# f4exb/sdrdaemon

Measured on AMD Instinct MI355X. Metric: IQ Msamples/s through decim+FEC-encode pipe; bit-exact vs CPU ref, higher is better.
Workload: dtype int32

## Files before the change

### sdrdaemon_amd/csrc/decim_body.h

```cpp
#pragma once
#include "sdrhip_internal.h"

namespace sdrhip {
namespace {

constexpr int NT = 256;
constexpr int P0 = DECIM_PASS;
constexpr int FULL = 512;
constexpr int HE = 32;

typedef short short2_t __attribute__((ext_vector_type(2)));
typedef int int2_t __attribute__((ext_vector_type(2)));
typedef int int4_t __attribute__((ext_vector_type(4)));
typedef unsigned uint4_t __attribute__((ext_vector_type(4)));

constexpr int C64[16] = {-7, 11, -20, 32, -49, 71, -101, 140, -190, 256, -345, 469, -656, 978, -1698, 5201};
__host__ __device__ constexpr int H32(int i) { return i < 16 ? C64[i] : C64[31 - i]; }
__host__ __device__ constexpr unsigned pack_taps(int lo, int hi) { return ((unsigned)lo & 0xffffu) | ((unsigned)hi << 16); }

constexpr int PK0_DW = 16 + 512 + 16;
constexpr int I0_DW = 32 + 1024;
constexpr int SN_DW = 32 + FULL;

template <int NS_, bool PK_> struct Geo {
    static constexpr int NS = NS_;
    static constexpr bool PK = PK_;
    static constexpr int stride(int s) { return s == 0 ? (PK ? PK0_DW : I0_DW) : SN_DW; }
    static constexpr int base(int s) { return s == 0 ? 0 : base(s - 1) + 4 * stride(s - 1); }
    static constexpr int ldsDw = base(NS);
    static constexpr int plane(int s, int parity, int comp) { return base(s) + (parity * 2 + comp) * stride(s); }
};

__device__ __forceinline__ int dot2(unsigned a, unsigned taps, int acc)
{
    return __builtin_amdgcn_sdot2(__builtin_bit_cast(short2_t, a), __builtin_bit_cast(short2_t, taps), acc, false);
}

__device__ __forceinline__ int dot2_link(unsigned a, unsigned taps, int acc) { return dot2(a, taps, acc); }

__device__ __forceinline__ int dot2_init(unsigned a, unsigned taps, int c)
{
    int d;
    asm("v_dot2_i32_i16 %0, %1, %2, %3" : "=v"(d) : "v"(a), "s"(taps), "v"(c));
    return d;
}

__device__ __forceinline__ int mad24(int a, int tap, int acc)
{
    int d;
    asm("v_mad_i32_i24 %0, %1, %2, %3" : "=v"(d) : "v"(a), "s"(tap), "v"(acc));
    return d;
}

struct OutCtx {
    unsigned *out;
    size_t out_pos;
    bool store;
    int norm, trunk;
    int frame_mode, frame_blocks;
    uint64_t frame_sample_base;
};

__device__ __forceinline__ unsigned final_pack(int i, int q, int norm, int trunk)
{
    int a = (int)((unsigned)i << norm) >> trunk;
    int b = (int)((unsigned)q << norm) >> trunk;
    return ((unsigned)a & 0xffffu) | ((unsigned)b << 16);
}

__device__ __forceinline__ void store_one(const OutCtx &oc, size_t k, unsigned v)
{
    if (!oc.frame_mode) {
        oc.out[k] = v;
    } else {
        uint64_t g = oc.frame_sample_base + k;
        uint64_t f = g / 16129u;
        unsigned w = (unsigned)(g - f * 16129u);
        unsigned b = w / 127u, i = w - b * 127u;
        oc.out[((size_t)f * oc.frame_blocks + 1 + b) * 128u + 1 + i] = v;
    }
}

template <class G, int S> __device__ __forceinline__ void run_stage(int *lds, int tid, int valid, int fill_next, int bias, const OutCtx &oc)
{
    constexpr bool PK = G::PK && S == 0;
    constexpr bool LAST = (S == G::NS - 1);
    constexpr int R = (S == 0) ? 8 : 4;
    const int j = tid >> 1, comp = tid & 1;
    const int k0 = j * R;
    if (k0 >= valid) return;
    const int *pe = lds + G::plane(S, 0, 0) + comp * G::stride(S);
    const int *po = lds + G::plane(S, 1, 0) + comp * G::stride(S);
    int res[R];
    if constexpr (PK) {
        constexpr int WO = (R + 32) / 2, WE = R / 2 + 4;
        unsigned wo[WO], we[WE];
#pragma unroll
        for (int d = 0; d < WO; d += 4) {
            uint4_t v = *reinterpret_cast<const uint4_t *>(po + k0 / 2 + d);
            wo[d] = v.x; wo[d + 1] = v.y; wo[d + 2] = v.z; wo[d + 3] = v.w;
        }
#pragma unroll
        for (int d = 0; d < WE; d += 4) {
            uint4_t v = *reinterpret_cast<const uint4_t *>(pe + k0 / 2 + 8 + d);
            we[d] = v.x; we[d + 1] = v.y; we[d + 2] = v.z; we[d + 3] = v.w;
        }
        const int bias13 = bias << 13;
        int acc[R];
#pragma unroll
        for (int r = 0; r < R; ++r)
            acc[r] = (r & 1) ? dot2_init(we[(r + 1) / 2], pack_taps(8192, 0), bias13) : dot2_init(we[r / 2], pack_taps(0, 8192), bias13);
#pragma unroll
        for (int t = 0; t < 17; ++t) {
#pragma unroll
            for (int r = 0; r < R; ++r) {
                if (r & 1) {
                    if (t < 16) acc[r] = dot2_link(wo[(r + 1) / 2 + t], pack_taps(H32(31 - 2 * t), H32(30 - 2 * t)), acc[r]);
                } else {
                    const unsigned taps = t == 0 ? pack_taps(0, H32(31)) : (t == 16 ? pack_taps(H32(0), 0) : pack_taps(H32(32 - 2 * t), H32(31 - 2 * t)));
                    acc[r] = dot2_link(wo[r / 2 + t], taps, acc[r]);
                }
            }
        }
#pragma unroll
        for (int r = 0; r < R; ++r) res[r] = acc[r] >> 13;
    } else {
        int wo[R + 32], we[R + 4];
#pragma unroll
        for (int x = 0; x < R + 32; x += 4) {
            int4_t v = *reinterpret_cast<const int4_t *>(po + k0 + x);
            wo[x] = v.x; wo[x + 1] = v.y; wo[x + 2] = v.z; wo[x + 3] = v.w;
        }
#pragma unroll
        for (int x = 0; x < R + 4; x += 4) {
            int4_t v = *reinterpret_cast<const int4_t *>(pe + k0 + 16 + x);
            we[x] = v.x; we[x + 1] = v.y; we[x + 2] = v.z; we[x + 3] = v.w;
        }
        int acc[R];
#pragma unroll
        for (int r = 0; r < R; ++r) acc[r] = (int)((unsigned)(we[r + 1] + bias) << 13);
#pragma unroll
        for (int i = 0; i < 16; ++i) {
#pragma unroll
            for (int r = 0; r < R; ++r) acc[r] = mad24(wo[r + 32 - i] + wo[r + 1 + i], C64[i], acc[r]);
        }
#pragma unroll
        for (int r = 0; r < R; ++r) res[r] = acc[r] >> 13;
    }

    if constexpr (LAST) {
        unsigned o[R];
#pragma unroll
        for (int r = 0; r < R; ++r) {
            int other = __builtin_amdgcn_update_dpp(0, res[r], 0xB1 , 0xf, 0xf, true);
            o[r] = final_pack(res[r], other, oc.norm, oc.trunk);
        }
        if (comp != 0 || !oc.store) return;
        const size_t k = oc.out_pos + k0;
        if (!oc.frame_mode && k0 + R <= valid) {
#pragma unroll
            for (int r = 0; r < R; r += 4) *reinterpret_cast<uint4_t *>(oc.out + k + r) = (uint4_t){o[r], o[r + 1], o[r + 2], o[r + 3]};
        } else if (!oc.frame_mode) {
#pragma unroll
            for (int r = 0; r < R; ++r)
                if (k0 + r < valid) oc.out[k + r] = o[r];
        } else {
            const uint64_t g = oc.frame_sample_base + k;
            const uint64_t f = g / 16129u;
            const unsigned w = (unsigned)(g - f * 16129u);
            unsigned b = w / 127u, i = w - b * 127u;
            size_t dw = ((size_t)f * oc.frame_blocks + 1 + b) * 128u + 1 + i;
#pragma unroll
            for (int r = 0; r < R; ++r) {
                if (k0 + r < valid) oc.out[dw] = o[r];
                ++i; ++dw;
                if (i == 127u) {
                    i = 0; ++b; dw += 1;
                    if (b == 127u) { b = 0; dw += ((size_t)oc.frame_blocks - 127u) * 128u; }
                }
            }
        }
    } else {
        int *ne = lds + G::plane(S + 1, 0, 0) + comp * G::stride(S + 1) + HE + fill_next + k0 / 2;
        int *no = lds + G::plane(S + 1, 1, 0) + comp * G::stride(S + 1) + HE + fill_next + k0 / 2;
        if constexpr (R == 8) {
            *reinterpret_cast<int4_t *>(ne) = (int4_t){res[0], res[2], res[4], res[6]};
            *reinterpret_cast<int4_t *>(no) = (int4_t){res[1], res[3], res[5], res[7]};
        } else {
            *reinterpret_cast<int2_t *>(ne) = (int2_t){res[0], res[2]};
            *reinterpret_cast<int2_t *>(no) = (int2_t){res[1], res[3]};
        }
    }
}

template <class G, int S> __device__ __forceinline__ void slide(int *lds, int tid, int consumed)
{
    if (tid >= 128) return;
    const int p = tid >> 5, e = tid & 31;
    int *pl = lds + G::base(S) + p * G::stride(S);
    if constexpr (G::PK && S == 0) {
        short *ps = reinterpret_cast<short *>(pl);
        const short v = ps[e + consumed];
        ps[e] = v;
    } else {
        const int v = pl[e + consumed];
        pl[e] = v;
    }
}

template <class G, int S> __device__ __forceinline__ void hist_put(int *lds, int p, int e, int v)
{
    int *pl = lds + G::base(S) + p * G::stride(S);
    if constexpr (G::PK && S == 0) reinterpret_cast<short *>(pl)[e] = (short)v;
    else pl[e] = v;
}
template <class G, int S> __device__ __forceinline__ int hist_get(const int *lds, int p, int e)
{
    const int *pl = lds + G::base(S) + p * G::stride(S);
    if constexpr (G::PK && S == 0) return reinterpret_cast<const short *>(pl)[e];
    else return pl[e];
}

template <class G, int S = 0> __device__ __forceinline__ void state_load(int *lds, int tid, const int32_t *st, bool zero)
{
    if (tid < 128) {
        const int sp = tid >> 5, e = tid & 31;
        const int kp = (sp & 1) * 2 + (sp >> 1);
        hist_put<G, S>(lds, kp, e, zero ? 0 : st[S * 4 * DEC_HIST + sp * DEC_HIST + e]);
    }
    if constexpr (S + 1 < G::NS) state_load<G, S + 1>(lds, tid, st, zero);
}
template <class G, int S = 0> __device__ __forceinline__ void state_store(const int *lds, int tid, int32_t *st)
{
    if (tid < 128) {
        const int sp = tid >> 5, e = tid & 31;
        const int kp = (sp & 1) * 2 + (sp >> 1);
        st[S * 4 * DEC_HIST + sp * DEC_HIST + e] = hist_get<G, S>(lds, kp, e);
    }
    if constexpr (S + 1 < G::NS) state_store<G, S + 1>(lds, tid, st);
}

template <class G, int S> __device__ __forceinline__ void later_stages(int *lds, int tid, int (&fill)[6], int consumed_prev, bool flush, int bias, OutCtx &oc)
{
    if constexpr (S < G::NS) {
        slide<G, S - 1>(lds, tid, consumed_prev);
        fill[S] += consumed_prev / 2;
        const int have = fill[S];
        const bool run = have > 0 && (have >= FULL || flush);
        if (run) {
            run_stage<G, S>(lds, tid, have, fill[S + 1 < 6 ? S + 1 : 5], bias, oc);
            if (S == G::NS - 1 && oc.store) oc.out_pos += have;
            fill[S] = 0;
        }
        __syncthreads();
        if (run) later_stages<G, S + 1>(lds, tid, fill, have, flush, bias, oc);
    } else {
        slide<G, G::NS - 1>(lds, tid, consumed_prev);
        __syncthreads();
    }
}

template <int L, int FC, bool PACK16, bool TAB = true>
__device__ __forceinline__ void decim_piece(const DecimArgs &a, int *lds, int stream, size_t seg_start, size_t seg_end, bool from_state,
                                            bool store_state, int meta_id, int meta_n)
{
    constexpr bool CEN = (FC == 2);
    constexpr int NS = CEN ? L : L - 2;
    constexpr int RAWSH = CEN ? 0 : 2;
    constexpr int PRAW = P0 << RAWSH;
    constexpr int NLD = PRAW / 4 / NT;
    constexpr int WRAW = 64 << L;
    using G = Geo<NS, PACK16>;
    const int tid = threadIdx.x;
    const unsigned *in = reinterpret_cast<const unsigned *>(a.in) + (size_t)stream * a.in_stride;

    const int32_t *stc = a.state_cur + (size_t)stream * DEC_STATE_WORDS;
    state_load<G>(lds, tid, stc, !from_state);

    OutCtx oc;
    oc.norm = a.norm; oc.trunk = a.trunk;
    oc.frame_mode = a.frame_mode; oc.frame_blocks = a.frame_blocks; oc.frame_sample_base = a.frame_sample_base;
    oc.out = reinterpret_cast<unsigned *>(a.out) + (size_t)stream * a.out_stride;
    oc.out_pos = seg_start >> L;

    if (a.frame_mode) {
        unsigned base[6], rate;
        stream_meta_base(a.meta_w, a.meta_rate, TAB ? a.meta_tab : nullptr, stream, base, rate);
        for (int fi = meta_id + tid * meta_n; fi < a.meta_count; fi += NT * meta_n) {
            unsigned w[6];
            frame_meta_words_thread(base, a.meta_idx0, rate, fi, w);
            unsigned *fr = oc.out + (size_t)(a.meta_first + fi) * a.frame_blocks * 128u;
            fr[0] = (a.meta_frame_count0 + (unsigned)fi) & 0xffffu;
#pragma unroll
            for (int k = 0; k < 6; ++k) fr[1 + k] = w[k];
        }
        if (tid < 128) {
            for (int fi = meta_id; fi < a.meta_count; fi += meta_n) {
                unsigned *fr = oc.out + (size_t)(a.meta_first + fi) * a.frame_blocks * 128u;
                const unsigned fidx = (a.meta_frame_count0 + (unsigned)fi) & 0xffffu;
                if (tid >= 7) fr[tid] = 0u;
                if (tid >= 1) fr[(size_t)tid * 128] = fidx | ((unsigned)tid << 16);
            }
        }
    }

    int fill[6] = {0, 0, 0, 0, 0, 0};
    bool warm = !from_state;
    size_t pos = warm ? seg_start - WRAW : 0;
    size_t region_end = warm ? seg_start : seg_end;

    uint4_t ld[NLD];
    auto issue = [&](size_t p, size_t rend) {
        const unsigned *src = in + p;
        const size_t left = rend - p;
        if (left >= (size_t)PRAW) {
#pragma unroll
            for (int n = 0; n < NLD; ++n) ld[n] = SDRHIP_STREAM_LOAD(reinterpret_cast<const uint4_t *>(src + 4 * (tid + n * NT)));
            return;
        }
        const unsigned rem = (unsigned)left;
#pragma unroll
        for (int n = 0; n < NLD; ++n) {
            const unsigned q = (unsigned)(tid + n * NT);
            uint4_t v = (uint4_t){0u, 0u, 0u, 0u};
            if (4 * q + 3 < rem) {
                v = SDRHIP_STREAM_LOAD(reinterpret_cast<const uint4_t *>(src + 4 * q));
            } else if (4 * q < rem) {
                v.x = src[4 * q];
                if (4 * q + 1 < rem) v.y = src[4 * q + 1];
                if (4 * q + 2 < rem) v.z = src[4 * q + 2];
            }
            ld[n] = v;
        }
    };
    issue(pos, region_end);
    __syncthreads();

    while (true) {
        const size_t left = region_end - pos;
        const int cnt_raw = left < (size_t)PRAW ? (int)left : PRAW;
        const int cnt0 = cnt_raw >> RAWSH;
#pragma unroll
        for (int n = 0; n < NLD; ++n) {
            const int q = tid + n * NT;
            const uint4_t v = ld[n];
            if constexpr (CEN && PACK16) {
                lds[G::plane(0, 0, 0) + 16 + q] = (int)__builtin_amdgcn_perm(v.z, v.x, 0x05040100u);
                lds[G::plane(0, 0, 1) + 16 + q] = (int)__builtin_amdgcn_perm(v.z, v.x, 0x07060302u);
                lds[G::plane(0, 1, 0) + 16 + q] = (int)__builtin_amdgcn_perm(v.w, v.y, 0x05040100u);
                lds[G::plane(0, 1, 1) + 16 + q] = (int)__builtin_amdgcn_perm(v.w, v.y, 0x07060302u);
            } else if constexpr (CEN) {
                *reinterpret_cast<int2_t *>(&lds[G::plane(0, 0, 0) + HE + 2 * q]) = (int2_t){(int)(short)(v.x & 0xffff), (int)(short)(v.z & 0xffff)};
                *reinterpret_cast<int2_t *>(&lds[G::plane(0, 0, 1) + HE + 2 * q]) = (int2_t){(int)v.x >> 16, (int)v.z >> 16};
                *reinterpret_cast<int2_t *>(&lds[G::plane(0, 1, 0) + HE + 2 * q]) = (int2_t){(int)(short)(v.y & 0xffff), (int)(short)(v.w & 0xffff)};
                *reinterpret_cast<int2_t *>(&lds[G::plane(0, 1, 1) + HE + 2 * q]) = (int2_t){(int)v.y >> 16, (int)v.w >> 16};
            } else {
                const int I0 = (short)(v.x & 0xffff), Q0 = (int)v.x >> 16, I1 = (short)(v.y & 0xffff), Q1 = (int)v.y >> 16;
                const int I2 = (short)(v.z & 0xffff), Q2 = (int)v.z >> 16, I3 = (short)(v.w & 0xffff), Q3 = (int)v.w >> 16;
                int x, y;
                if constexpr (FC == 0) {
                    x = I0 - Q1 + Q3 - I2; y = Q0 - Q2 + I1 - I3;
                } else {
                    x = Q0 - I1 - Q2 + I3; y = -I0 - Q1 + I2 + Q3;
                }
                lds[G::plane(0, q & 1, 0) + HE + (q >> 1)] = x;
                lds[G::plane(0, q & 1, 1) + HE + (q >> 1)] = y;
            }
        }
        const size_t next_pos = pos + cnt_raw;
        const bool flush = next_pos >= region_end;
        bool more = !flush;
        size_t n_pos = next_pos, n_end = region_end;
        if (flush && warm && seg_start < seg_end) { more = true; n_pos = seg_start; n_end = seg_end; }
        if (more) issue(n_pos, n_end);
        __syncthreads();

        oc.store = !warm;
        const int valid0 = cnt0 >> 1;
        run_stage<G, 0>(lds, tid, valid0, fill[1], a.bias, oc);
        if (NS == 1 && oc.store) oc.out_pos += valid0;
        __syncthreads();
        later_stages<G, 1>(lds, tid, fill, valid0, flush, a.bias, oc);

        if (!more) break;
        if (flush) { warm = false; region_end = seg_end; }
        pos = n_pos;
    }

    if (store_state) {
        int32_t *stn = a.state_next + (size_t)stream * DEC_STATE_WORDS;
        state_store<G>(lds, tid, stn);
        for (int i = NS * 4 * DEC_HIST + tid; i < DEC_STAGES * 4 * DEC_HIST; i += NT) stn[i] = stc[i];
    }
}


template <int L, int FC, bool PACK16> struct DecimLds {
    static constexpr int NS = (FC == 2) ? L : L - 2;
    static constexpr int dwords = Geo<NS, PACK16>::ldsDw;
    static_assert(dwords * 4 <= 64 * 1024, "LDS budget");
};

__device__ __forceinline__ void decim_simple_row(int log2decim, int fcpos, const int16_t *in, size_t in_stride, int16_t *out,
                                                 size_t out_stride, size_t n_in, int norm, int trunk, int stream)
{
    const unsigned *src = reinterpret_cast<const unsigned *>(in) + (size_t)stream * in_stride;
    unsigned *dst = reinterpret_cast<unsigned *>(out) + (size_t)stream * out_stride;
    const size_t g = (size_t)blockIdx.x * blockDim.x + threadIdx.x;
    if (log2decim == 0) {
        for (size_t i = g; i < n_in; i += (size_t)gridDim.x * blockDim.x) {
            unsigned v = SDRHIP_STREAM_LOAD(src + i);
            int a = (short)(v & 0xffff), b = (int)v >> 16;
            dst[i] = (((unsigned)a << norm) & 0xffffu) | (((unsigned)b << norm) << 16);
        }
        return;
    }
    const size_t n_resize = n_in >> log2decim;
    const size_t ngroups = n_in / 4;
    for (size_t q = g; q < (n_in + 3) / 4; q += (size_t)gridDim.x * blockDim.x) {
        if (q >= ngroups) {
            if (log2decim == 1 && 2 * q < n_resize) dst[2 * q] = 0;
            continue;
        }
        const unsigned v0 = SDRHIP_STREAM_LOAD(src + 4 * q), v1 = SDRHIP_STREAM_LOAD(src + 4 * q + 1), v2 = SDRHIP_STREAM_LOAD(src + 4 * q + 2), v3 = SDRHIP_STREAM_LOAD(src + 4 * q + 3);
        const int I0 = (short)(v0 & 0xffff), Q0 = (int)v0 >> 16, I1 = (short)(v1 & 0xffff), Q1 = (int)v1 >> 16;
        const int I2 = (short)(v2 & 0xffff), Q2 = (int)v2 >> 16, I3 = (short)(v3 & 0xffff), Q3 = (int)v3 >> 16;
        if (log2decim == 1) {
            int xa, ya, xb, yb;
            if (fcpos == 0) { xa = I0 - Q1; ya = Q0 + I1; xb = Q3 - I2; yb = -Q2 - I3; }
            else { xa = Q0 - I1; ya = -I0 - Q1; xb = I3 - Q2; yb = I2 + Q3; }
            dst[2 * q] = final_pack(xa, ya, norm, trunk);
            dst[2 * q + 1] = final_pack(xb, yb, norm, trunk);
        } else {
            int x, y;
            if (fcpos == 0) { x = I0 - Q1 + Q3 - I2; y = Q0 - Q2 + I1 - I3; }
            else { x = Q0 - I1 - Q2 + I3; y = -I0 - Q1 + I2 + Q3; }
            dst[q] = final_pack(x, y, norm, trunk);
        }
    }
}

}
}
```

### sdrdaemon_amd/csrc/decim_mfma.hip

```cpp
#include "decim_body.h"

#include <type_traits>
#include <utility>

#ifndef MF_WAVES
#define MF_WAVES 2
#endif
#ifndef MF_DMA_BURST
#define MF_DMA_BURST 1
#endif

namespace sdrhip {
namespace {

__host__ __device__ constexpr int mf_entry(int kq, int t) { return 8 * (t >> 1) + 2 * kq + (t & 1); }

struct MfATab {
    unsigned w[2][4][64][4];
};

constexpr MfATab mf_make_atab()
{
    MfATab T{};
    for (int m = 0; m < 2; ++m)
        for (int ph = 0; ph < 4; ++ph)
            for (int lane = 0; lane < 64; ++lane) {
                const int r = lane & 15, kq = lane >> 4;
                for (int j = 0; j < 4; ++j) {
                    const int beta = (ph - j) & 3;
                    unsigned word = 0;
                    for (int t = 0; t < 4; ++t) {
                        const int d = r - mf_entry(kq, t) + 16 * beta;
                        int v = 0;
                        if (beta == 3) {
                            const int e = mf_entry(kq, t);
                            const bool hit = (kq == 0 && t == 0) ? r == 15 : e == r + 1;
                            v = (m == 1 && hit) ? 32 : 0;
                        } else if (d >= 0 && d <= 31) {
                            const int h = H32(d);
                            const int h1 = (h + 128) >> 8, h0 = h - 256 * h1;
                            v = m == 0 ? h0 : h1;
                        }
                        word |= (unsigned)(v & 0xff) << (8 * t);
                    }
                    T.w[m][ph][lane][j] = word;
                }
            }
    return T;
}

__device__ const MfATab mf_atab = mf_make_atab();

constexpr int mf_tap_sum()
{
    int s = 0;
    for (int i = 0; i < 32; ++i) s += H32(i);
    return s;
}

template <class F, int... Is> __device__ __forceinline__ void mf_static_for_impl(F &&f, std::integer_sequence<int, Is...>)
{
    (f(std::integral_constant<int, Is>{}), ...);
}
template <int N, class F> __device__ __forceinline__ void mf_static_for(F &&f)
{
    mf_static_for_impl(f, std::make_integer_sequence<int, N>{});
}

__device__ __forceinline__ int4_t mfma(int4_t a, int4_t b, int4_t c)
{
    return __builtin_amdgcn_mfma_i32_16x16x64_i8(a, b, c, 0, 0, 0);
}
__device__ __forceinline__ unsigned perm(unsigned hi, unsigned lo, unsigned sel) { return __builtin_amdgcn_perm(hi, lo, sel); }

template <int NS> struct MfState {
    int4_t O[NS][3];
    unsigned pend[NS][2];
    unsigned evp[NS][2];
};

constexpr int MF_LIMB_BIAS = 128 + 32768 - 262144;

struct MfConst {
    int4_t A[2][4];
    int4_t c0;
    int cinN;
    unsigned selA;
    unsigned selB;
};

template <bool FR> struct MfOut {
    unsigned *p;
    unsigned *dump;
    int store;
    int norm, trunk;
    unsigned sel_pack;
    __amdgpu_buffer_rsrc_t rsrc;
    unsigned off, c, b, t0, t1;
    unsigned gap;
};

typedef unsigned uint2_t __attribute__((ext_vector_type(2)));
__device__ __forceinline__ int sbfe16(unsigned v, int off) { return (int)__builtin_amdgcn_sbfe((int)v, (unsigned)off, 16u); }

__device__ __forceinline__ unsigned lshl_add(unsigned a, int sh, unsigned b) { return (a << sh) + b; }
__device__ __forceinline__ unsigned opaque(unsigned v)
{
    asm("" : "+v"(v));
    return v;
}

__host__ __device__ constexpr int mf_nfixed(int ns) { return ns > 4 ? ns - 4 : 0; }
__host__ __device__ constexpr bool mf_fixed(int ns, int s) { return s >= ns - mf_nfixed(ns); }
template <int NS> constexpr int mf_period() { return 4 << (NS - 1 - mf_nfixed(NS)); }

template <int NS, int S, int I, class OC> __device__ __forceinline__ void mf_stage(MfState<NS> &st, const MfConst &k, OC &oc, int comp)
{
    constexpr int PH = mf_fixed(NS, S) ? 0 : (I & 3);
    const int4_t Ah0 = k.A[0][PH], Ah1 = k.A[1][PH];
    const int4_t z = {0, 0, 0, 0};
    unsigned acc[4];
    if constexpr (S == 0) {
        int4_t g0 = mfma(Ah0, st.O[0][0], k.c0);
        int4_t g1 = mfma(Ah0, st.O[0][1], z);
        int4_t g2 = mfma(Ah1, st.O[0][1], z);
        g1 = mfma(Ah1, st.O[0][0], g1);
#pragma unroll
        for (int r = 0; r < 4; ++r) acc[r] = lshl_add(opaque(lshl_add((unsigned)g2[r], 8, (unsigned)g1[r])), 8, (unsigned)g0[r]);
    } else {
        const int4_t cN = {k.cinN, k.cinN, k.cinN, k.cinN};
        int4_t g0 = mfma(Ah0, st.O[S][0], cN);
        int4_t g1 = mfma(Ah0, st.O[S][1], z);
        int4_t g2 = mfma(Ah0, st.O[S][2], z);
        int4_t g3 = mfma(Ah1, st.O[S][2], z);
        g1 = mfma(Ah1, st.O[S][0], g1);
        g2 = mfma(Ah1, st.O[S][1], g2);
#pragma unroll
        for (int r = 0; r < 4; ++r)
            acc[r] = lshl_add(opaque(lshl_add(opaque(lshl_add((unsigned)g3[r], 8, (unsigned)g2[r])), 8, (unsigned)g1[r])), 8, (unsigned)g0[r]);
    }

    if constexpr (S < NS - 1) {
        constexpr int SIG = I & 1, J = I >> 1;
        const unsigned X = 0x80808080u, X2 = 0x04040404u;
        const unsigned u0 = acc[0] >> 13, u1 = acc[1] >> 13, u2 = acc[2] >> 13, u3 = acc[3] >> 13;
        const unsigned po = perm(u3, u1, 0x05010400u), po2 = perm(u3, u1, 0x0c0c0602u);
        const unsigned pe = perm(u2, u0, 0x05010400u), pe2 = perm(u2, u0, 0x0c0c0602u);
        if constexpr (SIG == 0) {
            st.pend[S + 1][0] = po; st.pend[S + 1][1] = po2;
            constexpr int DJ = mf_fixed(NS, S + 1) ? 1 : ((J + 1) & 3);
            st.O[S + 1][0][DJ] = (int)(perm(pe, (unsigned)st.O[S + 1][0][DJ], k.selA) ^ X);
            st.O[S + 1][1][DJ] = (int)(perm(pe, (unsigned)st.O[S + 1][1][DJ], k.selB) ^ X);
            st.O[S + 1][2][DJ] = (int)(perm(pe2, (unsigned)st.O[S + 1][2][DJ], k.selA) ^ X2);
            st.evp[S + 1][0] = pe; st.evp[S + 1][1] = pe2;
        } else {
            constexpr bool FIX = mf_fixed(NS, S + 1);
            constexpr int NJ = FIX ? 0 : (J & 3), DN = FIX ? 1 : ((J + 2) & 3);
            if constexpr (FIX) {
#pragma unroll
                for (int l = 0; l < 3; ++l) { st.O[S + 1][l][2] = st.O[S + 1][l][3]; st.O[S + 1][l][3] = st.O[S + 1][l][0]; }
            }
            st.O[S + 1][0][NJ] = (int)(perm(po, st.pend[S + 1][0], 0x05040100u) ^ X);
            st.O[S + 1][1][NJ] = (int)(perm(po, st.pend[S + 1][0], 0x07060302u) ^ X);
            st.O[S + 1][2][NJ] = (int)(perm(po2, st.pend[S + 1][1], 0x05040100u) ^ X2);
            const unsigned e0 = perm(pe, st.evp[S + 1][0], 0x05040100u), e1 = perm(pe, st.evp[S + 1][0], 0x07060302u),
                           e2 = perm(pe2, st.evp[S + 1][1], 0x05040100u);
            mf_stage<NS, S + 1, J>(st, k, oc, comp);
            st.O[S + 1][0][DN] = (int)e0; st.O[S + 1][1][DN] = (int)e1; st.O[S + 1][2][DN] = (int)e2;
        }
    } else {
        const int o0 = (int)acc[0] >> 13, o1 = (int)acc[1] >> 13, o2 = (int)acc[2] >> 13, o3 = (int)acc[3] >> 13;
        const int g0 = comp ? o0 : o2, g1 = comp ? o1 : o3;
        const int m0 = comp ? o2 : o0, m1 = comp ? o3 : o1;
        const int r0 = __builtin_amdgcn_update_dpp(0, g0, 0xB1 , 0xf, 0xf, true);
        const int r1 = __builtin_amdgcn_update_dpp(0, g1, 0xB1, 0xf, 0xf, true);
        const unsigned pk0 = perm((unsigned)((int)((unsigned)r0 << oc.norm) >> oc.trunk), (unsigned)((int)((unsigned)m0 << oc.norm) >> oc.trunk), oc.sel_pack);
        const unsigned pk1 = perm((unsigned)((int)((unsigned)r1 << oc.norm) >> oc.trunk), (unsigned)((int)((unsigned)m1 << oc.norm) >> oc.trunk), oc.sel_pack);
        if constexpr (std::is_same<OC, MfOut<true>>::value) {
            const unsigned extra = oc.b == 126u ? oc.gap : 4u;
            const unsigned bias = oc.store ? 0u : 0x80000000u;
            const unsigned a0 = oc.off + (oc.c >= oc.t0 ? extra : 0u) + bias;
            const unsigned hi = a0 ^ 0x40000000u;
            const bool split = oc.c == oc.t1;
            const unsigned a8 = split ? hi : a0, a4 = split ? a0 : hi;
            __builtin_amdgcn_raw_buffer_store_b64((uint2_t){pk0, pk1}, oc.rsrc, a8, 0, 0);
            __builtin_amdgcn_raw_buffer_store_b32(pk0, oc.rsrc, a4, 0, 0);
            __builtin_amdgcn_raw_buffer_store_b32(pk1, oc.rsrc, a4 + extra, 4, 0);
            const unsigned inc = oc.store ? 16u : 0u;
            oc.c += inc;
            const bool wrap = oc.c >= 127u;
            oc.off += 4u * inc + (wrap ? extra : 0u);
            oc.c -= wrap ? 127u : 0u;
            oc.b += wrap ? 1u : 0u;
            oc.b = oc.b >= 127u ? 0u : oc.b;
        } else {
            unsigned *dst = oc.store ? oc.p : oc.dump;
            *reinterpret_cast<uint2_t *>(dst) = (uint2_t){pk0, pk1};
            oc.p += oc.store ? 16 : 0;
        }
    }
}

struct MfFront {
    unsigned sel_own, sel_oth, sel_lo, sel_hi;
    unsigned ev_lo, ev_hi;
};
template <int NS, int I> __device__ __forceinline__ void mf_front(MfState<NS> &st, const MfConst &k, MfFront &f, const uint4_t r)
{
    constexpr int i = I;
    const unsigned ao = perm(r.w, r.y, f.sel_own), ae = perm(r.z, r.x, f.sel_own);
    const unsigned xo = perm(r.w, r.y, f.sel_oth), xe = perm(r.z, r.x, f.sel_oth);
    const unsigned yo = (unsigned)__builtin_amdgcn_update_dpp(0, (int)xo, 0xB1 , 0xf, 0xf, true);
    const unsigned ye = (unsigned)__builtin_amdgcn_update_dpp(0, (int)xe, 0xB1, 0xf, 0xf, true);
    st.O[0][0][i & 3] = (int)(perm(ao, yo, f.sel_lo) ^ 0x80808080u);
    st.O[0][1][i & 3] = (int)perm(ao, yo, f.sel_hi);
    const unsigned cur_lo = perm(ae, ye, f.sel_lo) ^ 0x80808080u, cur_hi = perm(ae, ye, f.sel_hi);
    st.O[0][0][(i + 1) & 3] = (int)perm(cur_lo, f.ev_lo, k.selA);
    st.O[0][1][(i + 1) & 3] = (int)perm(cur_hi, f.ev_hi, k.selA);
    f.ev_lo = cur_lo; f.ev_hi = cur_hi;
}

template <int NS, int I> __device__ __forceinline__ void mf_front2(MfState<NS> &st, const MfConst &k, MfFront &f, const uint4_t rA, const uint4_t rB)
{
    constexpr int i = I;
    const unsigned aoA = perm(rA.w, rA.y, f.sel_own), aoB = perm(rB.w, rB.y, f.sel_own);
    const unsigned aeA = perm(rA.z, rA.x, f.sel_own), aeB = perm(rB.z, rB.x, f.sel_own);
    st.O[0][0][i & 3] = (int)(perm(aoA, aoB, 0x01000504u) ^ 0x80808080u);
    st.O[0][1][i & 3] = (int)perm(aoA, aoB, 0x03020706u);
    const unsigned cur_lo = perm(aeA, aeB, 0x01000504u) ^ 0x80808080u, cur_hi = perm(aeA, aeB, 0x03020706u);
    st.O[0][0][(i + 1) & 3] = (int)perm(cur_lo, f.ev_lo, k.selA);
    st.O[0][1][(i + 1) & 3] = (int)perm(cur_hi, f.ev_hi, k.selA);
    f.ev_lo = cur_lo; f.ev_hi = cur_hi;
}

constexpr int MF_GROUP_BYTES = 9216;
constexpr int mf_wave_ring(int ng) { return ng * MF_GROUP_BYTES; }
static_assert(MF_HEAD_MIN % P0 == 0 && MF_TAIL_SEG % P0 == 0, "K1m's head and tail pieces are whole passes of the VALU code");
__host__ __device__ constexpr int mf_block_units(int p) { return 72 * p + 2 * (p >> 2); }

template <int D> __device__ __forceinline__ void mf_dma_issue(unsigned slot, unsigned voff, unsigned long long span_base)
{
    constexpr int off = 16 * mf_block_units(D);
    asm volatile("s_add_u32 m0, %1, %2\n\ts_nop 0\n\tglobal_load_lds_dwordx4 %0, %3 nt" ::"v"(voff), "s"(slot), "n"(off), "s"(span_base) : "memory", "scc");
}
template <int N> __device__ __forceinline__ void mf_wait_vm()
{
    static_assert(N == 0 || N == 7 || N == 8 || N == 15 || N == 16, "vmcnt immediates of the ring");
    if constexpr (N == 0) asm volatile("s_waitcnt vmcnt(0)" ::: "memory");
    if constexpr (N == 7) asm volatile("s_waitcnt vmcnt(7)" ::: "memory");
    if constexpr (N == 8) asm volatile("s_waitcnt vmcnt(8)" ::: "memory");
    if constexpr (N == 15) asm volatile("s_waitcnt vmcnt(15)" ::: "memory");
    if constexpr (N == 16) asm volatile("s_waitcnt vmcnt(16)" ::: "memory");
}

#ifdef MF_STAMPS
__device__ unsigned long long g_mf_stamps[4096 * 10];
__device__ __forceinline__ void mf_stamp(int gw, int k)
{
    if ((threadIdx.x & 63) == 0 && gw < 4096) {
        unsigned long long t;
        asm volatile("s_memrealtime %0\n\ts_waitcnt lgkmcnt(0)" : "=s"(t)::"memory");
        g_mf_stamps[gw * 10 + k] = t;
        if (k == 0) {
            unsigned hw, xcc;
            asm volatile("s_getreg_b32 %0, hwreg(HW_REG_HW_ID)" : "=s"(hw));
            asm volatile("s_getreg_b32 %0, hwreg(HW_REG_XCC_ID)" : "=s"(xcc));
            g_mf_stamps[gw * 10 + 8] = ((unsigned long long)(xcc & 0xfu) << 32) | hw;
        }
    }
}
#define MF_STAMP(gw, k) mf_stamp(gw, k)
#else
#define MF_STAMP(gw, k) do { } while (0)
#endif

template <int NS, int NG, class OC>
__device__ __forceinline__ void mf_loop_dma(const DecimArgs &a, MfState<NS> &st, const MfConst &k, OC &oc, MfFront &fr, unsigned lds_addr,
                                            const char *wbase, size_t S, int nper, int WP, int lane, int p, int comp, int q, int gw)
{
    constexpr int P = mf_period<NS>();
    static_assert(P == 32, "four groups of 8 steps per period");
    static_assert(NG == 2 || NG == 3 || NG == 4, "ring depth");
    constexpr int LA = NG - 1;
    const int wv = __builtin_amdgcn_readfirstlane((int)(threadIdx.x >> 6));
    const unsigned ring = (unsigned)__builtin_amdgcn_readfirstlane((int)(lds_addr + (unsigned)wv * (unsigned)mf_wave_ring(NG)));
    unsigned long long sb[8];
#pragma unroll
    for (int d = 0; d < 8; ++d) {
        const unsigned long long v = (unsigned long long)(wbase + (size_t)d * S * 4);
        sb[d] = ((unsigned long long)(unsigned)__builtin_amdgcn_readfirstlane((int)(v >> 32)) << 32) | (unsigned)__builtin_amdgcn_readfirstlane((int)v);
    }
    unsigned rs[NG];
    const __attribute__((address_space(3))) char *lr[NG];
#pragma unroll
    for (int j = 0; j < NG; ++j) {
        rs[j] = ring + (unsigned)(j * MF_GROUP_BYTES);
        lr[j] = (const __attribute__((address_space(3))) char *)(size_t)(rs[j] + 16u * (unsigned)(mf_block_units(0) + 72 * p + 2 * (p >> 2) + 4 * comp + q));
    }
    unsigned voff[4];
    const unsigned vmax = 16u * (unsigned)lane + 1024u * (unsigned)(4 * nper - 1);
#pragma unroll
    for (int g = 0; g < 4; ++g) voff[g] = min(16u * (unsigned)lane + 1024u * (unsigned)(g + LA), vmax);
    {
        unsigned v0 = 16u * (unsigned)lane;
        mf_static_for<8 * LA>([&](auto ic) {
            constexpr int i = decltype(ic)::value;
            mf_dma_issue<i % 8>(rs[i / 8], v0 + 1024u * (unsigned)(i / 8), sb[i % 8]);
        });
    }
    MF_STAMP(gw, 1);
    mf_wait_vm<8 * (LA - 1)>();
    uint4_t r = *reinterpret_cast<const __attribute__((address_space(3))) uint4_t *>(lr[0]);
    MF_STAMP(gw, 2);
    for (int per = 0; per < nper; ++per) {
#ifdef MF_STAMPS
        if (per == 1) MF_STAMP(gw, 3);
        if (per == nper / 4) MF_STAMP(gw, 4);
        if (per == nper / 2) MF_STAMP(gw, 5);
        if (per == 3 * nper / 4) MF_STAMP(gw, 6);
#endif
        oc.store = per >= WP;
        mf_static_for<P>([&](auto ic) {
            constexpr int i = decltype(ic)::value;
            constexpr int i1 = i + 1;
            constexpr int B = NG == 2 ? 8 : MF_DMA_BURST;
            if constexpr (i1 % 8 == 0) mf_wait_vm<(B == 1 ? 8 * (LA - 2) + 7 : 8 * (LA - 1))>();
            const uint4_t rn = *reinterpret_cast<const __attribute__((address_space(3))) uint4_t *>(lr[(i1 / 8) % NG] + 128 * (i1 % 8));
            constexpr int g = i / 8, d = i % 8;
            if constexpr (d < 8 / B) {
                mf_static_for<B>([&](auto bc) {
                    constexpr int sp = B * d + decltype(bc)::value;
                    mf_dma_issue<sp>(rs[(g + LA) % NG], voff[g], sb[sp]);
                });
                if constexpr (d == 8 / B - 1) voff[g] = min(voff[g] + 4096u, vmax);
            }
            mf_front<NS, i>(st, k, fr, r);
            mf_stage<NS, 0, i>(st, k, oc, comp);
            r = rn;
        });
        if constexpr (4 % NG != 0) {
            const unsigned t = rs[0];
            const __attribute__((address_space(3))) char *u = lr[0];
#pragma unroll
            for (int j = 0; j + 1 < NG; ++j) { rs[j] = rs[j + 1]; lr[j] = lr[j + 1]; }
            rs[NG - 1] = t; lr[NG - 1] = u;
        }
    }
    mf_wait_vm<0>();
}

template <int NS, int NG = 0, bool FR = false> __device__ __forceinline__ void mf_wave(const DecimArgs &a, int gw, unsigned lds_addr)
{
    if (a.mf_prio) __builtin_amdgcn_s_setprio(3);
    constexpr int L = NS;
    constexpr int P = mf_period<NS>();
#ifndef MF_DEPTH
#define MF_DEPTH 8
#endif
#ifndef MF_BURST
#define MF_BURST 1
#endif
    constexpr int D = MF_DEPTH < P ? MF_DEPTH : P / 2;
    constexpr size_t W = (size_t)64 << L;
    constexpr int WP = (int)(W / (32 * (size_t)P));
    static_assert(P % D == 0, "prefetch ring");
    static_assert((size_t)D * 32 <= MF_READ_AHEAD, "the planner leaves the register ring's read-ahead behind a wave's last span (decim_plan.h)");
    const int lane = threadIdx.x & 63;
    const int n = lane & 15, q = lane >> 4, comp = n & 1, p = n >> 1;
    const int stream = gw / a.mf_wps, ws = gw - stream * a.mf_wps;
    const size_t S = a.mf_span;
    const size_t wave_start = a.mf_head + (size_t)ws * 8 * S;
    const char *wbase = reinterpret_cast<const char *>(a.in) + ((size_t)stream * a.in_stride + wave_start - W) * 4;
    const unsigned loff = (unsigned)((size_t)p * S * 4) + 16u * (unsigned)q + 64u * (unsigned)comp;
    const int T = (int)((W + S) / 32);
    const int nper = T / P;

    MfConst k;
#pragma unroll
    for (int m = 0; m < 2; ++m)
#pragma unroll
        for (int ph = 0; ph < 4; ++ph) k.A[m][ph] = *reinterpret_cast<const int4_t *>(&mf_atab.w[m][ph][lane][0]);
    const unsigned b13 = (unsigned)a.bias << 13;
    const unsigned gain = (unsigned)mf_tap_sum() + 8192u;
    {
        const int c = (int)(128u * gain + b13);
        k.c0 = (int4_t){c, c, c, c};
    }
    k.cinN = (int)((unsigned)MF_LIMB_BIAS * gain + b13);
    k.selA = q == 0 ? 0x03020104u : 0x03020100u;
    k.selB = q == 0 ? 0x03020106u : 0x03020100u;

    MfOut<FR> oc;
    oc.store = 0;
    oc.dump = a.mf_dump + 4 * lane;
    oc.norm = a.norm; oc.trunk = a.trunk;
    oc.sel_pack = comp ? 0x01000504u : 0x05040100u;
    {
        const size_t first = ((wave_start + (size_t)p * S) >> L) + 4u * (unsigned)q;
        if constexpr (FR) {
            unsigned *obase = reinterpret_cast<unsigned *>(a.out) + (size_t)stream * a.out_stride;
            oc.rsrc = __builtin_amdgcn_make_buffer_rsrc(obase, 0, 0x3fffffff, 0x00020000);
            const unsigned long long g = a.frame_sample_base + first;
            const unsigned long long f = g / 16129u;
            const unsigned w = (unsigned)(g - f * 16129u);
            oc.b = w / 127u; oc.c = w - oc.b * 127u;
            oc.off = 4u * (unsigned)(((size_t)f * (size_t)a.frame_blocks + 1u + oc.b) * 128u + 1u + oc.c + 2u * (unsigned)comp);
            oc.t0 = 127u - 2u * (unsigned)comp; oc.t1 = 126u - 2u * (unsigned)comp;
            oc.gap = 4u * ((unsigned)a.frame_blocks * 128u - 16255u);
            oc.p = nullptr;
        } else {
            unsigned *obase = reinterpret_cast<unsigned *>(a.out) + (size_t)stream * a.out_stride;
            oc.p = obase + first + 2 * comp;
            oc.off = oc.c = oc.b = oc.t0 = oc.t1 = oc.gap = 0u;
        }
    }

    MfState<NS> st;
#pragma unroll
    for (int s = 0; s < NS; ++s) {
#pragma unroll
        for (int b = 0; b < 3; ++b) st.O[s][b] = (int4_t){0, 0, 0, 0};
        st.pend[s][0] = st.pend[s][1] = 0u;
        st.evp[s][0] = st.evp[s][1] = 0u;
    }

    MfFront fr;
    fr.sel_own = comp ? 0x07030602u : 0x05010400u;
    fr.sel_oth = comp ? 0x05010400u : 0x07030602u;
    fr.sel_lo = comp ? 0x05040100u : 0x01000504u; fr.sel_hi = comp ? 0x07060302u : 0x03020706u;
    fr.ev_lo = 0u; fr.ev_hi = 0u;
    if constexpr (NG != 0 && mf_dma_applies(NS)) {
        mf_loop_dma<NS, NG>(a, st, k, oc, fr, lds_addr, wbase, S, nper, WP, lane, p, comp, q, gw);
        return;
    }
    uint4_t ld[D];
    const char *src = wbase + loff;
#define MF_LDSTRIDE 128
#pragma unroll
    for (int d = 0; d < D; ++d) ld[d] = SDRHIP_STREAM_LOAD(reinterpret_cast<const uint4_t *>(src + MF_LDSTRIDE * d));

    for (int per = 0; per < nper; ++per) {
        oc.store = per >= WP;
        mf_static_for<P>([&](auto ic) {
            constexpr int i = decltype(ic)::value;
            constexpr int slot = i % D;
            const uint4_t r = ld[slot];
            ld[slot] = SDRHIP_STREAM_LOAD(reinterpret_cast<const uint4_t *>(src + MF_LDSTRIDE * (i + D)));
            mf_front<NS, i>(st, k, fr, r);
            mf_stage<NS, 0, i>(st, k, oc, comp);
        });
        src += MF_LDSTRIDE * P;
    }
}

__host__ __device__ constexpr int mf_block_threads(int) { return NT; }

template <int L, bool PACK16, int NG, bool FR> __global__ __launch_bounds__(mf_block_threads(L), mf_dma_applies(L) && NG != 2 ? 1 : MF_WAVES) void decim_mfma_kernel(DecimArgs a)
{
    constexpr int LDSDW = mf_dma_applies(L) && mf_wave_ring(NG) > DecimLds<L, 2, PACK16>::dwords ? mf_wave_ring(NG) : DecimLds<L, 2, PACK16>::dwords;
    __shared__ __attribute__((aligned(16))) int lds[LDSDW];
    const int nmf = (a.nstreams * a.mf_wps + 3) / 4;
    const int bx = blockIdx.x;
    if (bx >= nmf) {
        const int nitems = a.nstreams * a.mf_npieces, j = bx - nmf, nearly = a.mf_piece_early * a.mf_piece_share;
        const int nmine = j < a.mf_piece_early ? a.mf_piece_share : 1;
        for (int k = 0; k < nmine; ++k) {
            const int lx = j < a.mf_piece_early ? j + k * a.mf_piece_early : nearly + (j - a.mf_piece_early);
            if (lx >= nitems || (j < a.mf_piece_early && lx >= nearly)) break;
            const int stream = lx / a.mf_npieces, piece = lx - stream * a.mf_npieces;
            if (piece == 0) {
                decim_piece<L, 2, PACK16>(a, lds, stream, 0, a.mf_head, true, false, piece, a.mf_npieces);
            } else {
                const size_t s0 = a.mf_tail_start + (size_t)(piece - 1) * a.mf_tail_seg;
                size_t s1 = s0 + a.mf_tail_seg;
                if (s1 > a.n_used || piece == a.mf_npieces - 1) s1 = a.n_used;
                decim_piece<L, 2, PACK16>(a, lds, stream, s0, s1, false, piece == a.mf_npieces - 1, piece, a.mf_npieces);
            }
            __syncthreads();
        }
        return;
    }
    const int gw = __builtin_amdgcn_readfirstlane(bx * 4 + (int)(threadIdx.x >> 6));
    if (gw >= a.nstreams * a.mf_wps) return;
    MF_STAMP(gw, 0);
    mf_wave<L, NG, FR>(a, gw, (unsigned)(size_t)(__attribute__((address_space(3))) char *)lds);
    MF_STAMP(gw, 7);
}
__device__ __forceinline__ int mf_ragged_find(const RaggedRow *rows, int nstreams, int x, bool waves)
{
    int lo = 0, hi = nstreams - 1;
    while (lo < hi) {
        const int mid = (lo + hi + 1) >> 1;
        if ((waves ? rows[mid].mf_w0 : rows[mid].mf_p0) <= x) lo = mid;
        else hi = mid - 1;
    }
    return __builtin_amdgcn_readfirstlane(lo);
}
__device__ __forceinline__ DecimArgs mf_ragged_args(const DecimArgs &a, const RaggedRow &r)
{
    DecimArgs b = a;
    b.n_used = (size_t)r.n_used;
    b.mf_wps = r.mf_wps;
    const unsigned sh = (unsigned)__builtin_amdgcn_readfirstlane((int)r.shifts);
    b.norm = (int)(sh & 0xffu); b.trunk = (int)(sh >> 8);
    if (a.frame_mode) {
        b.out = reinterpret_cast<int16_t *>(reinterpret_cast<unsigned *>(a.out) + r.out_off);
        b.frame_sample_base = r.frame_sample_base;
        b.meta_first = r.meta_first; b.meta_count = r.meta_count; b.meta_frame_count0 = r.frame_count0;
        b.meta_w[3] = r.tv_sec; b.meta_w[4] = r.tv_usec;
        b.meta_idx0 = r.meta_idx0;
    }
    return b;
}

template <int L, bool PACK16, int NG, bool FR> __global__ __launch_bounds__(mf_block_threads(L), mf_dma_applies(L) && NG != 2 ? 1 : MF_WAVES) void decim_mfma_ragged_kernel(DecimArgs a, const RaggedRow *rows)
{
    constexpr int LDSDW = mf_dma_applies(L) && mf_wave_ring(NG) > DecimLds<L, 2, PACK16>::dwords ? mf_wave_ring(NG) : DecimLds<L, 2, PACK16>::dwords;
    __shared__ __attribute__((aligned(16))) int lds[LDSDW];
    const int nmf = (a.mf_wps + 3) / 4;
    const int bx = blockIdx.x;
    if (bx >= nmf) {
        const int nitems = a.mf_npieces, j = bx - nmf, nearly = a.mf_piece_early * a.mf_piece_share;
        const int nmine = j < a.mf_piece_early ? a.mf_piece_share : 1;
        for (int k = 0; k < nmine; ++k) {
            const int lx = j < a.mf_piece_early ? j + k * a.mf_piece_early : nearly + (j - a.mf_piece_early);
            if (lx >= nitems || (j < a.mf_piece_early && lx >= nearly)) break;
            const int stream = mf_ragged_find(rows, a.nstreams, lx, false);
            const RaggedRow &r = rows[stream];
            const DecimArgs b = mf_ragged_args(a, r);
            const int piece = lx - r.mf_p0;
            const size_t n_used = (size_t)r.n_used;
            if (piece == 0) {
                decim_piece<L, 2, PACK16, false>(b, lds, stream, 0, (size_t)r.mf_head, true, r.mf_np == 1, piece, r.mf_np);
            } else {
                const size_t s0 = (size_t)r.mf_tail_start + (size_t)(piece - 1) * a.mf_tail_seg;
                size_t s1 = s0 + a.mf_tail_seg;
                if (s1 > n_used || piece == r.mf_np - 1) s1 = n_used;
                decim_piece<L, 2, PACK16, false>(b, lds, stream, s0, s1, false, piece == r.mf_np - 1, piece, r.mf_np);
            }
            __syncthreads();
        }
        return;
    }
    const int gw = __builtin_amdgcn_readfirstlane(bx * 4 + (int)(threadIdx.x >> 6));
    if (gw >= a.mf_wps) return;
    const int stream = mf_ragged_find(rows, a.nstreams, gw, true);
    const RaggedRow &r = rows[stream];
    const DecimArgs b = mf_ragged_args(a, r);
    mf_wave<L, NG, FR>(b, stream * r.mf_wps + (gw - r.mf_w0), (unsigned)(size_t)(__attribute__((address_space(3))) char *)lds);
}

#ifdef MF_STAMPS
}
extern "C" int sdrhip_debug_mf_stamps(unsigned long long *dst) { return (int)hipMemcpyFromSymbol(dst, HIP_SYMBOL(g_mf_stamps), sizeof(g_mf_stamps)); }
namespace {
#endif

#include "gf_encode128_body.h"
#ifndef MF_FUSED_WPE
#define MF_FUSED_WPE 3
#endif
struct FusedRoles {
    unsigned *tab;
    unsigned tag;
};

template <int L, bool PACK16> __global__ __launch_bounds__(NT, MF_FUSED_WPE) void rx_fused_kernel(DecimArgs a, Enc128Args e, FusedRoles fr)
{
    constexpr int LDSDW = ENC128_LDS_BYTES / 4 > DecimLds<L, 2, PACK16>::dwords ? ENC128_LDS_BYTES / 4 : DecimLds<L, 2, PACK16>::dwords;
    __shared__ __attribute__((aligned(16))) int lds[LDSDW];
    __shared__ int s_unit;
    const int nmf = (a.nstreams * a.mf_wps + 3) / 4;
    const int npiece = a.nstreams * a.mf_npieces;
    const int nenc = 2 * e.nlist;
    if (threadIdx.x == 0) {
        unsigned hw, xcc;
        asm volatile("s_getreg_b32 %0, hwreg(HW_REG_HW_ID)" : "=s"(hw));
        asm volatile("s_getreg_b32 %0, hwreg(HW_REG_XCC_ID)" : "=s"(xcc));
        const unsigned key = ((xcc & 0xfu) << 8) | ((hw >> 8) & 0xffu);
        unsigned *cnt = fr.tab + 4096 + 4 * (fr.tag & 1u);
        if (blockIdx.x == 0) { unsigned *nxt = fr.tab + 4096 + 4 * ((fr.tag + 1u) & 1u); nxt[0] = 0u; nxt[1] = 0u; nxt[2] = 0u; }
        const bool first = atomicMax(fr.tab + key, fr.tag) < fr.tag;
        int unit = -1;
        if (first) { const unsigned u = atomicAdd(cnt + 0, 1u); if (u < (unsigned)nmf) unit = (int)u; }
        if (unit < 0) { const unsigned u = atomicAdd(cnt + 1, 1u); if (u < (unsigned)npiece) unit = nmf + (int)u; }
        if (unit < 0) { const unsigned u = atomicAdd(cnt + 2, 1u); if (u < (unsigned)nenc) unit = nmf + npiece + (int)u; }
        if (unit < 0) { const unsigned u = atomicAdd(cnt + 0, 1u); if (u < (unsigned)nmf) unit = (int)u; }
        s_unit = unit;
    }
    __syncthreads();
    const int bx = s_unit;
    if (bx < 0) return;
    const int ndec = nmf + npiece;
    if (bx >= ndec) {
        gf_encode128_wg(e, bx - ndec, reinterpret_cast<unsigned char *>(lds));
        return;
    }
    if (bx >= nmf) {
        const int lx = bx - nmf;
        const int stream = lx / a.mf_npieces, piece = lx - stream * a.mf_npieces;
        if (piece == 0) {
            decim_piece<L, 2, PACK16>(a, lds, stream, 0, a.mf_head, true, false, piece, a.mf_npieces);
        } else {
            const size_t s0 = a.mf_tail_start + (size_t)(piece - 1) * a.mf_tail_seg;
            size_t s1 = s0 + a.mf_tail_seg;
            if (s1 > a.n_used || piece == a.mf_npieces - 1) s1 = a.n_used;
            decim_piece<L, 2, PACK16>(a, lds, stream, s0, s1, false, piece == a.mf_npieces - 1, piece, a.mf_npieces);
        }
        return;
    }
    const int gw = __builtin_amdgcn_readfirstlane(bx * 4 + (int)(threadIdx.x >> 6));
    if (gw >= a.nstreams * a.mf_wps) return;
    mf_wave<L, 0>(a, gw, 0u);
}

template <int L> hipError_t launch_fused(bool pack16, const DecimArgs &a, const Enc128Args &e, unsigned *roles, unsigned tag, hipStream_t stream)
{
    const int ndec = (a.nstreams * a.mf_wps + 3) / 4 + a.nstreams * a.mf_npieces;
    const dim3 grid(ndec + 2 * e.nlist), block(NT);
    FusedRoles fr;
    fr.tab = roles; fr.tag = tag;
    if (pack16) hipLaunchKernelGGL((rx_fused_kernel<L, true>), grid, block, 0, stream, a, e, fr);
    else hipLaunchKernelGGL((rx_fused_kernel<L, false>), grid, block, 0, stream, a, e, fr);
    return hipGetLastError();
}

template <int L, int NG, bool FR> void launch_mf2(bool pack16, const DecimArgs &a, dim3 grid, dim3 block, hipStream_t stream)
{
    if (pack16) hipLaunchKernelGGL((decim_mfma_kernel<L, true, NG, FR>), grid, block, 0, stream, a);
    else hipLaunchKernelGGL((decim_mfma_kernel<L, false, NG, FR>), grid, block, 0, stream, a);
}

template <int L> hipError_t launch_mf(bool pack16, const DecimArgs &a, hipStream_t stream)
{
    const int nleg = a.mf_piece_wgs > 0 ? a.mf_piece_wgs : a.nstreams * a.mf_npieces;
    const int nmf = (a.nstreams * a.mf_wps + 3) / 4;
    const dim3 grid(nleg + nmf), block(mf_block_threads(L));
    if constexpr (mf_dma_applies(L)) {
// ... 76 lines not shown
```

### sdrdaemon_amd/csrc/rx_frame_area.h

```cpp
#pragma once
#include <cstddef>
#include <cstdint>
#include <vector>

namespace sdrhip {
constexpr uint64_t RX_FRAME_SAMPLES = 127 * 127;
constexpr size_t RX_NO_LATE = ~(size_t)0;

struct RxAdvance {
    size_t done;
    uint64_t rest;
    int first_new;
    int started;
    uint64_t idx0;
    unsigned frame_count0;
};

struct RxAreaPlan {
    size_t new_cap = 0;
    bool keep_old = false;
    std::vector<uint8_t> to_slot0;
    bool moves() const
    {
        for (size_t s = 0; s < to_slot0.size(); ++s)
            if (to_slot0[s]) return true;
        return false;
    }
};

class RxFrameArea {
public:
    void init(size_t nstreams)
    {
        cap_ = 0;
        base_.assign(nstreams, 0); pending_.assign(nstreams, 0); open_.assign(nstreams, 0); count_.assign(nstreams, 0);
    }
    size_t streams() const { return base_.size(); }
    size_t cap() const { return cap_; }
    size_t slot(size_t s) const { return base_[s]; }
    const size_t *slots() const { return base_.data(); }
    uint64_t pending(size_t s) const { return pending_[s]; }
    bool open(size_t s) const { return open_[s] != 0; }
    uint16_t count(size_t s) const { return count_[s]; }
    size_t index(size_t s, size_t f = 0) const { return s * cap_ + base_[s] + f; }

    bool aligned() const
    {
        for (size_t s = 1; s < base_.size(); ++s)
            if (base_[s] != base_[0] || pending_[s] != pending_[0] || open_[s] != open_[0] || count_[s] != count_[0]) return false;
        return true;
    }

    RxAdvance advance(size_t s, size_t n_dec) const
    {
        RxAdvance a;
        const uint64_t total = pending_[s] + n_dec;
        a.done = (size_t)(total / RX_FRAME_SAMPLES);
        a.rest = total - (uint64_t)a.done * RX_FRAME_SAMPLES;
        a.first_new = open_[s] ? 1 : 0;
        a.started = (int)(a.done + (a.rest > 0 ? 1 : 0)) - a.first_new;
        a.idx0 = a.first_new ? RX_FRAME_SAMPLES - pending_[s] : 0;
        a.frame_count0 = (unsigned)count_[s] + (unsigned)a.first_new;
        return a;
    }

    RxAreaPlan plan(const size_t *done, size_t late_slot0, size_t window_multiple) const
    {
        RxAreaPlan p;
        const size_t S = base_.size();
        size_t need_max = 0;
        for (size_t s = 0; s < S; ++s) need_max = done[s] + 1 > need_max ? done[s] + 1 : need_max;
        bool hits_late = false;
        p.to_slot0.assign(S, 0);
        if (need_max > cap_) p.new_cap = window_multiple * need_max;
        else
            for (size_t s = 0; s < S; ++s) {
                if (base_[s] + done[s] + 1 <= cap_) continue;
                p.to_slot0[s] = 1;
                hits_late = hits_late || (late_slot0 != RX_NO_LATE && done[s] + 1 > late_slot0);
            }
        if (hits_late) p.new_cap = cap_;
        if (p.new_cap) {
            p.to_slot0.assign(S, 1);
            p.keep_old = late_slot0 != RX_NO_LATE;
        }
        return p;
    }
    RxAreaPlan replan() const
    {
        RxAreaPlan p;
        p.new_cap = cap_;
        p.to_slot0.assign(base_.size(), cap_ ? 1 : 0);
        return p;
    }
    void moved(const RxAreaPlan &p)
    {
        if (p.new_cap) cap_ = p.new_cap;
        for (size_t s = 0; s < base_.size(); ++s)
            if (p.to_slot0[s]) base_[s] = 0;
    }
    void commit(const size_t *done, const uint64_t *rest)
    {
        for (size_t s = 0; s < base_.size(); ++s) {
            base_[s] += done[s];
            pending_[s] = rest[s];
            open_[s] = rest[s] > 0 ? 1 : 0;
            count_[s] = (uint16_t)(count_[s] + done[s]);
        }
    }

    void reset(const uint8_t *mask)
    {
        for (size_t s = 0; s < base_.size(); ++s) {
            if (mask && !mask[s]) continue;
            pending_[s] = 0; open_[s] = 0; count_[s] = 0;
            if (!mask) base_[s] = 0;
        }
    }
    static bool importable(uint64_t pending, uint32_t open, uint32_t count)
    {
        return open <= 1 && pending < RX_FRAME_SAMPLES && (open || !pending) && count <= 0xffffu;
    }
    void import_stream(size_t s, uint64_t pending, uint32_t open, uint32_t count)
    {
        pending_[s] = pending; open_[s] = (uint8_t)open; count_[s] = (uint16_t)count;
    }

private:
    size_t cap_ = 0;
    std::vector<size_t> base_;
    std::vector<uint64_t> pending_;
    std::vector<uint8_t> open_;
    std::vector<uint16_t> count_;
};

class RxView {
public:
    const uint8_t *base() const { return base_; }
    size_t stride() const { return stride_; }
    size_t first(size_t s) const { return first_[s]; }
    size_t frames(size_t s) const { return frames_[s]; }
    void init(size_t nstreams) { set(nullptr, 0, nstreams, 0, 0); }
    void clear() { base_ = nullptr; stride_ = 0; first_.assign(first_.size(), 0); frames_.assign(frames_.size(), 0); }
    bool uniform() const
    {
        for (size_t s = 1; s < first_.size(); ++s)
            if (first_[s] != first_[0] || frames_[s] != frames_[0]) return false;
        return true;
    }
    void set(const uint8_t *area, size_t stream_stride, size_t nstreams, size_t first_slot, size_t n)
    {
        base_ = area; stride_ = stream_stride; first_.assign(nstreams, first_slot); frames_.assign(nstreams, n);
    }
    void set_each(const uint8_t *area, size_t stream_stride, size_t nstreams, const size_t *first_slot, const size_t *n)
    {
        base_ = area; stride_ = stream_stride; first_.assign(first_slot, first_slot + nstreams); frames_.assign(n, n + nstreams);
    }
    size_t offset(size_t s, size_t frame_bytes) const { return s * stride_ + first_[s] * frame_bytes; }
    const uint8_t *window(size_t s, size_t frame_bytes) const { return base_ ? base_ + offset(s, frame_bytes) : nullptr; }

private:
    const uint8_t *base_ = nullptr;
    size_t stride_ = 0;
    std::vector<size_t> first_, frames_;
};
}
```

### sdrdaemon_amd/csrc/sdrhip.cpp

```cpp
#include "sdrhip_host.h"
#include "gf256.h"

#include <cstdarg>
#include <cstdio>
#include <cstdlib>
#include <cstring>
#include <new>
#include <string>
#include <vector>

using namespace sdrhip;

namespace {
thread_local std::string g_err;
}

namespace sdrhip {

int fail(int code, const char *fmt, ...)
{
    char buf[512];
    va_list ap;
    va_start(ap, fmt);
    vsnprintf(buf, sizeof(buf), fmt, ap);
    va_end(ap);
    g_err = buf;
    return code;
}

}

extern "C" const char *sdrhip_last_error(void) { return g_err.c_str(); }

extern "C" int sdrhip_device_count(void)
{
    int n = 0;
    if (hipGetDeviceCount(&n) != hipSuccess) return 0;
    return n;
}

namespace sdrhip {
static void ctx_free(sdrhip_ctx *c);
static void drop_kernel_events(sdrhip_ctx *c)
{
    (void)hipStreamSynchronize(c->stream);
    if (c->stream2) (void)hipStreamSynchronize(c->stream2);
    for (int k = 0; k < SDRHIP_KCLASSES; ++k) {
        for (auto &pr : c->kev[k]) { (void)hipEventDestroy(pr.first); (void)hipEventDestroy(pr.second); }
        c->kev[k].clear();
    }
}
}

extern "C" int sdrhip_ctx_create(int device, void *hip_stream, sdrhip_ctx **out)
{
    if (!out) return fail(SDRHIP_EINVAL, "ctx_create: out is NULL");
    *out = nullptr;
    int n = sdrhip_device_count();
    if (n <= 0) return fail(SDRHIP_EDEVICE, "no HIP device available (this library has no CPU fallback)");
    if (device < 0 || device >= n) return fail(SDRHIP_EINVAL, "device %d out of range (have %d)", device, n);
    HIP_TRY(hipSetDevice(device));
    sdrhip_ctx *c = new (std::nothrow) sdrhip_ctx();
    if (!c) return fail(SDRHIP_ENOMEM, "out of host memory");
    c->device = device;
    c->stream = static_cast<hipStream_t>(hip_stream);
    {
        hipDeviceProp_t prop;
        if (hipGetDeviceProperties(&prop, device) == hipSuccess && prop.multiProcessorCount > 0) c->n_cu = prop.multiProcessorCount;
        static const char *const keys[][2] = {{"SDRHIP_DECIM_PATH", "decim_path"}, {"SDRHIP_MFMA_SPAN", "mfma_span"}, {"SDRHIP_MFMA_MIN", "mfma_min"},
                                              {"SDRHIP_INTERP_PATH", "interp_path"}, {"SDRHIP_INTERP_SPAN", "interp_span"}, {"SDRHIP_RX_FUSED", "rx_fused"}, {"SDRHIP_RX_DIRECT", "rx_direct"},
                                              {"SDRHIP_DEC_PATH", "dec_path"}, {"SDRHIP_ENC_PATH", "enc_path"}, {"SDRHIP_ENC_MIN_ROWS", "enc_min_rows"}, {"SDRHIP_MFMA_RING", "mfma_ring"}, {"SDRHIP_TX_OVERLAP", "tx_overlap"}, {"SDRHIP_RX_WINDOW", "rx_window"}, {"SDRHIP_FEC_STAGGER", "fec_stagger"}, {"SDRHIP_FEC_STAGGER_MOD", "fec_stagger_mod"}, {"SDRHIP_DEC_PLAN", "dec_plan"}, {"SDRHIP_TX_GATHER", "tx_gather"}, {"SDRHIP_ENC_UNITS", "enc_units"}, {"SDRHIP_ENC_FORM", "enc_form"}};
        for (size_t i = 0; i < sizeof(keys) / sizeof(keys[0]); ++i)
            if (const char *v = getenv(keys[i][0])) (void)sdrhip_ctx_set_option(c, keys[i][1], v);
    }
    std::vector<uint8_t> tab(256 * 32);
    gf_build_tables(tab.data());
    if (hipMalloc(reinterpret_cast<void **>(&c->gf_tab), tab.size()) != hipSuccess) { c->gf_tab = nullptr; ctx_free(c); return fail(SDRHIP_ENOMEM, "hipMalloc gf tables"); }
    if (hipMemcpy(c->gf_tab, tab.data(), tab.size(), hipMemcpyHostToDevice) != hipSuccess) { ctx_free(c); return fail(SDRHIP_EDEVICE, "upload gf tables"); }
    std::vector<uint8_t> em(128 * 128);
    cm256_encode_matrix(128, 128, em.data());
    if (hipMalloc(reinterpret_cast<void **>(&c->enc_matrix), em.size()) != hipSuccess ||
        hipMemcpy(c->enc_matrix, em.data(), em.size(), hipMemcpyHostToDevice) != hipSuccess) { ctx_free(c); return fail(SDRHIP_ENOMEM, "upload encode matrix"); }
    std::vector<uint8_t> kl(8 * 81 * 32);
    cm256_karatsuba_leaf_tables(kl.data());
    if (hipMalloc(reinterpret_cast<void **>(&c->enc_leaves), kl.size()) != hipSuccess ||
        hipMemcpy(c->enc_leaves, kl.data(), kl.size(), hipMemcpyHostToDevice) != hipSuccess) { ctx_free(c); return fail(SDRHIP_ENOMEM, "upload encoder constants"); }
    {
        std::vector<uint8_t> ft((size_t)CM256_FFT_TABLES * 32);
        cm256_fft_tables(ft.data());
        if (hipMalloc(reinterpret_cast<void **>(&c->enc_fft), ft.size()) != hipSuccess ||
            hipMemcpy(c->enc_fft, ft.data(), ft.size(), hipMemcpyHostToDevice) != hipSuccess) { ctx_free(c); return fail(SDRHIP_ENOMEM, "upload encoder FFT constants"); }
    }
    {
        const GF256 &g = gf();
        uint8_t el[1024];
        memcpy(el, g.exp, 512);
        memcpy(el + 512, g.log, 512);
        if (hipMalloc(reinterpret_cast<void **>(&c->gf_explog), sizeof(el)) != hipSuccess ||
            hipMemcpy(c->gf_explog, el, sizeof(el), hipMemcpyHostToDevice) != hipSuccess) { ctx_free(c); return fail(SDRHIP_ENOMEM, "upload GF(256) exp/log tables"); }
    }
    if (hipMalloc(reinterpret_cast<void **>(&c->dec_stats), 64) != hipSuccess ||
        hipMemset(c->dec_stats, 0, 64) != hipSuccess) { ctx_free(c); return fail(SDRHIP_ENOMEM, "hipMalloc decoder counters"); }
    if (hipMalloc(reinterpret_cast<void **>(&c->decim_dump), 4096) != hipSuccess) { c->decim_dump = nullptr; ctx_free(c); return fail(SDRHIP_ENOMEM, "hipMalloc decimator scratch"); }
    if (hipMalloc(reinterpret_cast<void **>(&c->fused_roles), SDRHIP_FUSED_ROLE_WORDS * 4) != hipSuccess ||
        hipMemset(c->fused_roles, 0, SDRHIP_FUSED_ROLE_WORDS * 4) != hipSuccess) { ctx_free(c); return fail(SDRHIP_ENOMEM, "hipMalloc role table"); }
    if (hipEventCreate(&c->ev0) != hipSuccess || hipEventCreate(&c->ev1) != hipSuccess) { ctx_free(c); return fail(SDRHIP_EDEVICE, "hipEventCreate"); }
    *out = c;
    return SDRHIP_OK;
}

namespace sdrhip {
int ctx_stream2(sdrhip_ctx *c, hipStream_t *out)
{
    if (!c->stream2) {
        int lo = 0, hi = 0;
        if (hipDeviceGetStreamPriorityRange(&lo, &hi) != hipSuccess) lo = 0;
        if (hipStreamCreateWithPriority(&c->stream2, hipStreamNonBlocking, lo) != hipSuccess) {
            c->stream2 = nullptr;
            return fail(SDRHIP_EDEVICE, "hipStreamCreate (second stream)");
        }
    }
    *out = c->stream2;
    return SDRHIP_OK;
}
void ctx_retain(sdrhip_ctx *c) { c->refs.fetch_add(1); }
void ctx_release(sdrhip_ctx *c)
{
    if (c->refs.fetch_sub(1) == 1 && c->dying) ctx_free(c);
}
}

extern "C" void sdrhip_ctx_destroy(sdrhip_ctx *c)
{
    if (!c || c->dying.exchange(true)) return;
    if (c->refs.load() == 0) ctx_free(c);
}

extern "C" int sdrhip_ctx_set_option(sdrhip_ctx *c, const char *key, const char *value)
{
    if (!c || !key || !value) return fail(SDRHIP_EINVAL, "ctx_set_option: NULL argument");
    sdrhip::CtxLock lock_(c);
    const std::string k(key), v(value);
    char *end = nullptr;
    const unsigned long long num = strtoull(value, &end, 10);
    const bool isnum = *value && end && !*end;
    if (k == "decim_path") {
        if (v == "auto") c->opt.decim_path = DECIM_PATH_AUTO;
        else if (v == "valu") c->opt.decim_path = DECIM_PATH_VALU;
        else if (v == "mfma") c->opt.decim_path = DECIM_PATH_MFMA;
        else return fail(SDRHIP_EINVAL, "ctx_set_option: decim_path must be auto, valu or mfma");
    } else if (k == "interp_path") {
        if (v == "auto") c->opt.interp_wave = CtxOptions().interp_wave;
        else if (v == "valu") c->opt.interp_wave = 0;
        else if (v == "wave") c->opt.interp_wave = 1;
        else return fail(SDRHIP_EINVAL, "ctx_set_option: interp_path must be auto, valu or wave");
    } else if (k == "mfma_span" && isnum) c->opt.mfma_span = (size_t)num;
    else if (k == "mfma_min" && isnum) c->opt.mfma_min = (size_t)num;
    else if (k == "interp_span" && isnum) c->opt.interp_span = (size_t)num;
    else if (k == "rx_fused" && isnum && num <= 3) c->opt.rx_fused = (int)num;
    else if (k == "rx_fused" && v == "overlap") c->opt.rx_fused = 3;
    else if (k == "rx_direct" && isnum && num <= 1) c->opt.rx_direct = (int)num;
    else if (k == "rx_window" && isnum && num <= 8) c->opt.rx_window = (int)num;
    else if (k == "mfma_ring" && isnum && num >= 2 && num <= 4) c->opt.mfma_ring = (int)num;
    else if (k == "tx_overlap" && isnum && num <= 1) c->opt.tx_overlap = (int)num;
    else if (k == "fec_stagger" && isnum && num <= 64) c->opt.fec_stagger = (int)num;
    else if (k == "fec_stagger_mod" && isnum && num <= 116) c->opt.fec_stagger_mod = (int)num;
    else if (k == "tx_gather" && isnum && num <= 1) c->opt.tx_gather = (int)num;
    else if (k == "dec_plan") {
        if (v == "fused") c->opt.dec_fused_plan = 1;
        else if (v == "kernel") c->opt.dec_fused_plan = 0;
        else return fail(SDRHIP_EINVAL, "ctx_set_option: dec_plan must be fused or kernel");
    }
    else if (k == "enc_min_rows" && isnum && num >= 1 && num <= 32) c->opt.enc_min_rows = (int)num;
    else if (k == "enc_units" && (v == "frame" || v == "half")) c->opt.enc_half = v == "half";
    else if (k == "enc_form" && (v == "bitslice" || v == "table")) c->opt.enc_bitslice = v == "bitslice";
    else if (k == "enc_path") {
        if (v == "fft") c->opt.enc_fft = 1;
        else if (v == "karatsuba") c->opt.enc_fft = 0;
        else return fail(SDRHIP_EINVAL, "ctx_set_option: enc_path must be fft or karatsuba");
    } else if (k == "dec_path") {
        if (v == "syndrome") c->opt.dec_syndrome = 1;
        else if (v == "dense") c->opt.dec_syndrome = 0;
        else return fail(SDRHIP_EINVAL, "ctx_set_option: dec_path must be syndrome or dense");
    } else if (k == "dec_max_rows" && isnum && num >= 1 && num <= 128) { c->opt.dec_max_rows = (int)num; c->opt.dec_auto = 0; }
    else if (k == "dec_max_rows" && v == "auto") { c->opt.dec_max_rows = 128; c->opt.dec_auto = 1; }
    else if (k == "dec_strict" && isnum && num <= 1) c->opt.dec_strict = (int)num;
    else if (k == "ktime_stride" && isnum && num >= 1 && num <= 1024) { c->ktime_stride = (int)num; for (int i = 0; i < SDRHIP_KCLASSES; ++i) c->ktime_stride_cls[i] = 0; }
    else if (k == "ktime_stride_class") {
        int cls = -1, st = 0;
        if (sscanf(value, "%d:%d", &cls, &st) != 2 || cls < 0 || cls >= SDRHIP_KCLASSES || st < 1 || st > 1024) return fail(SDRHIP_EINVAL, "ctx_set_option: ktime_stride_class takes <class 0..4>:<stride 1..1024>");
        c->ktime_stride_cls[cls] = st;
    }
    else return fail(SDRHIP_EINVAL, "ctx_set_option: unknown key or malformed value: %s=%s", key, value);
    return SDRHIP_OK;
}

extern "C" int sdrhip_ctx_get_counter(sdrhip_ctx *c, const char *key, uint64_t *value)
{
    if (!c || !key || !value) return fail(SDRHIP_EINVAL, "ctx_get_counter: NULL argument");
    sdrhip::CtxLock lock_(c);
    if (std::string(key) == "h2d_bytes") { *value = c->h2d_bytes; return SDRHIP_OK; }
    if (std::string(key) == "d2h_bytes") { *value = c->d2h_bytes; return SDRHIP_OK; }
    const bool shadow = std::string(key) == "fecbuf_shadow_mismatch";
    const bool deferred = std::string(key) == "dec_deferred";
    if (std::string(key) != "dec_rows_exceeded" && !shadow && !deferred) return fail(SDRHIP_EINVAL, "ctx_get_counter: unknown key: %s", key);
    HIP_TRY(hipSetDevice(c->device));
    unsigned v = 0;
    HIP_TRY(link_copy(c, &v, c->dec_stats + (shadow ? DEC_STATS_SHADOW_MISMATCH : deferred ? DEC_STATS_DEFERRED : 0), sizeof(v), hipMemcpyDeviceToHost, c->stream));
    HIP_TRY(hipStreamSynchronize(c->stream));
    *value = v;
    return SDRHIP_OK;
}

int sdrhip::enc128_min_rows(const sdrhip_ctx *c) { return c->opt.enc_fft ? c->opt.enc_min_rows : ENC128_MIN_ROWS; }

static void sdrhip::ctx_free(sdrhip_ctx *c)
{
    (void)hipSetDevice(c->device);
    (void)hipStreamSynchronize(c->stream);
    drop_kernel_events(c);
    c->in.release(); c->out.release(); c->aux.release(); c->aux3.release();
    if (c->gf_tab) (void)hipFree(c->gf_tab);
    if (c->enc_matrix) (void)hipFree(c->enc_matrix);
    if (c->enc_leaves) (void)hipFree(c->enc_leaves);
    if (c->enc_fft) (void)hipFree(c->enc_fft);
    if (c->decim_dump) (void)hipFree(c->decim_dump);
    if (c->fused_roles) (void)hipFree(c->fused_roles);
    if (c->gf_explog) (void)hipFree(c->gf_explog);
    if (c->dec_stats) (void)hipFree(c->dec_stats);
    c->dec_plan.release();
    c->pin.release();
    c->zin.release(); c->zout.release();
    if (c->stream2) { (void)hipStreamSynchronize(c->stream2); (void)hipStreamDestroy(c->stream2); }
    if (c->ev0) (void)hipEventDestroy(c->ev0);
    if (c->ev1) (void)hipEventDestroy(c->ev1);
    delete c;
}

extern "C" int sdrhip_ctx_synchronize(sdrhip_ctx *c)
{
    if (!c) return fail(SDRHIP_EINVAL, "ctx is NULL");
    sdrhip::CtxLock lock_(c);
    HIP_TRY(hipStreamSynchronize(c->stream));
    if (c->stream2) HIP_TRY(hipStreamSynchronize(c->stream2));
    return SDRHIP_OK;
}

extern "C" int sdrhip_ctx_timing_begin(sdrhip_ctx *c)
{
    if (!c) return fail(SDRHIP_EINVAL, "ctx is NULL");
    HIP_TRY(hipEventRecord(c->ev0, c->stream));
    return SDRHIP_OK;
}

extern "C" int sdrhip_ctx_timing_end(sdrhip_ctx *c, float *ms)
{
    if (!c || !ms) return fail(SDRHIP_EINVAL, "ctx/ms is NULL");
    HIP_TRY(hipEventRecord(c->ev1, c->stream));
    HIP_TRY(hipEventSynchronize(c->ev1));
    HIP_TRY(hipEventElapsedTime(ms, c->ev0, c->ev1));
    return SDRHIP_OK;
}

extern "C" int sdrhip_ctx_kernel_timing(sdrhip_ctx *c, int enable)
{
    if (!c) return fail(SDRHIP_EINVAL, "ctx is NULL");
    sdrhip::CtxLock lock_(c);
    c->ktime_on = enable != 0;
    for (int i = 0; i < SDRHIP_KCLASSES; ++i) c->ktime_seen[i] = 0;
    if (!enable) drop_kernel_events(c);
    return SDRHIP_OK;
}

extern "C" int sdrhip_ctx_kernel_timing_read(sdrhip_ctx *c, int cls, double *total_ms, unsigned *launches)
{
    if (!c || cls < 0 || cls >= SDRHIP_KCLASSES || !total_ms || !launches) return fail(SDRHIP_EINVAL, "kernel_timing_read: bad argument");
    sdrhip::CtxLock lock_(c);
    HIP_TRY(hipStreamSynchronize(c->stream));
    if (c->stream2) HIP_TRY(hipStreamSynchronize(c->stream2));
    double sum = 0;
    unsigned n = 0;
    for (auto &pr : c->kev[cls]) {
        float ms = 0;
        if (hipEventElapsedTime(&ms, pr.first, pr.second) == hipSuccess) { sum += ms; ++n; }
        (void)hipEventDestroy(pr.first);
        (void)hipEventDestroy(pr.second);
    }
    c->kev[cls].clear();
    *total_ms = sum;
    *launches = n;
    return SDRHIP_OK;
}

namespace {
struct HostRange { const char *p; size_t n; };
std::mutex g_host_mtx;
std::vector<HostRange> g_host_ranges;
}
namespace sdrhip {
bool host_is_pinned(const void *p, size_t n)
{
    std::lock_guard<std::mutex> g(g_host_mtx);
    const char *c = static_cast<const char *>(p);
    for (const HostRange &r : g_host_ranges)
        if (c >= r.p && c + n <= r.p + r.n) return true;
    return false;
}
}

extern "C" void *sdrhip_host_alloc(sdrhip_ctx *c, size_t bytes)
{
    if (!c || bytes == 0) return nullptr;
    if (hipSetDevice(c->device) != hipSuccess) return nullptr;
    void *p = nullptr;
    if (hipHostMalloc(&p, bytes, hipHostMallocDefault) != hipSuccess) { (void)fail(SDRHIP_ENOMEM, "hipHostMalloc(%zu) failed", bytes); return nullptr; }
    std::lock_guard<std::mutex> g(g_host_mtx);
    g_host_ranges.push_back(HostRange{static_cast<const char *>(p), bytes});
    return p;
}

extern "C" void sdrhip_host_free(sdrhip_ctx *c, void *p)
{
    if (!p) return;
    (void)c;
    {
        std::lock_guard<std::mutex> g(g_host_mtx);
        for (size_t i = 0; i < g_host_ranges.size(); ++i)
            if (g_host_ranges[i].p == p) { g_host_ranges.erase(g_host_ranges.begin() + (long)i); break; }
    }
    (void)hipHostFree(p);
}
```

### sdrdaemon_amd/csrc/sdrhip_decim.cpp

```cpp
#include "sdrhip_host.h"

#include <cstring>
#include <new>
#include <vector>

using namespace sdrhip;

struct sdrhip_decimators {
    sdrhip::CtxRef ctx;
    int nstreams;
    int bias;
    sdrhip::DevBuf state[2];
    int cur;
    bool stage0_int16;
    sdrhip::DecimPlanInfo last;
    sdrhip::PinnedBuf rows_pin, stage_pin, out_pin;
    sdrhip::DevBuf rows_dev;
    sdrhip::StreamMask reset_mask;
    explicit sdrhip_decimators(sdrhip_ctx *c) : ctx(c) {}
};

extern "C" int sdrhip_decimators_last_plan(const sdrhip_decimators *d, sdrhip_decim_plan *out)
{
    if (!d || !out) return fail(SDRHIP_EINVAL, "decimators_last_plan: NULL argument");
    sdrhip::CtxLock lock_(d->ctx);
    out->path = d->last.path; out->wps = d->last.wps; out->npieces = d->last.npieces; out->nseg = d->last.nseg;
    out->span = d->last.span; out->head = d->last.head; out->tail_start = d->last.tail_start;
    return SDRHIP_OK;
}

extern "C" int sdrhip_decimators_create(sdrhip_ctx *ctx, int nstreams, int hb_variant, sdrhip_decimators **out)
{
    if (!ctx || !out || nstreams <= 0 || nstreams > 65535) return fail(SDRHIP_EINVAL, "decimators_create: bad argument");
    if (hb_variant != SDRHIP_HB_EO1 && hb_variant != SDRHIP_HB_DB) return fail(SDRHIP_EINVAL, "hb_variant must be SDRHIP_HB_EO1 or SDRHIP_HB_DB");
    HIP_TRY(hipSetDevice(ctx->device));
    sdrhip_decimators *d = new (std::nothrow) sdrhip_decimators(ctx);
    if (!d) return fail(SDRHIP_ENOMEM, "out of host memory");
    d->nstreams = nstreams; d->bias = hb_variant; d->cur = 0; d->stage0_int16 = true;
    size_t bytes = (size_t)nstreams * DEC_STATE_WORDS * sizeof(int32_t);
    if (d->state[0].alloc_exact(bytes) || d->state[1].alloc_exact(bytes)) {
        delete d;
        return fail(SDRHIP_ENOMEM, "hipMalloc decimator state");
    }
    *out = d;
    return sdrhip_decimators_reset(d);
}

extern "C" void sdrhip_decimators_destroy(sdrhip_decimators *d)
{
    if (!d) return;
    (void)hipSetDevice(d->ctx->device);
    (void)hipStreamSynchronize(d->ctx->stream);
    delete d;
}

extern "C" int sdrhip_decimators_reset(sdrhip_decimators *d)
{
    if (!d) return fail(SDRHIP_EINVAL, "decimators is NULL");
    sdrhip::CtxLock lock_(d->ctx);
    size_t bytes = (size_t)d->nstreams * DEC_STATE_WORDS * sizeof(int32_t);
    HIP_TRY(hipMemsetAsync(d->state[0].p, 0, bytes, d->ctx->stream));
    HIP_TRY(hipMemsetAsync(d->state[1].p, 0, bytes, d->ctx->stream));
    d->cur = 0;
    d->stage0_int16 = true;
    return SDRHIP_OK;
}

namespace sdrhip {
void decimators_reset_part(sdrhip_decimators *d, StreamResetArgs *a)
{
    a->rows[0] = d->state[0].as<int32_t>(); a->rows[1] = d->state[1].as<int32_t>();
    a->row_words = DEC_STATE_WORDS;
}
void decimators_reset_done(sdrhip_decimators *d, bool all)
{
    if (all) d->stage0_int16 = true;
}
int32_t *decimators_row(sdrhip_decimators *d, int s, int half) { return d->state[d->cur ^ (half & 1)].as<int32_t>() + (size_t)s * DEC_STATE_WORDS; }
bool decimators_stage0_int16(const sdrhip_decimators *d) { return d->stage0_int16; }
void decimators_clear_stage0_int16(sdrhip_decimators *d) { d->stage0_int16 = false; }
}

extern "C" int sdrhip_decimators_reset_streams(sdrhip_decimators *d, const uint8_t *mask)
{
    if (!d) return fail(SDRHIP_EINVAL, "decimators is NULL");
    sdrhip::CtxLock lock_(d->ctx);
    return stream_reset_bank(d->ctx, d->reset_mask, mask, d->nstreams,
                             [d](StreamResetArgs *a) { decimators_reset_part(d, a); },
                             [d](const uint8_t *m) { decimators_reset_done(d, m == nullptr); });
}

namespace {
void set_mf_args(DecimArgs &a, const MfPlan &p)
{
    a.mf_head = p.head; a.mf_span = p.span; a.mf_tail_start = p.tail_start; a.mf_tail_seg = p.tail_seg;
    a.mf_wps = p.wps; a.mf_npieces = p.npieces;
    a.mf_piece_wgs = p.piece_wgs; a.mf_piece_early = p.piece_early; a.mf_piece_share = p.piece_share;
}

struct DecimCall {
    const int16_t *in;
    size_t in_stride;
    int16_t *out;
    size_t out_stride;
    int frame_mode, frame_blocks;
    size_t n_raw, n_dec;
    size_t min_used;
};

template <class Simple, class Plan, class Launch>
int decimate_core(sdrhip_decimators *d, unsigned L, int fcpos, const DecimCall &k, Simple simple, Plan plan, Launch launch)
{
    sdrhip_ctx *c = d->ctx;
    d->last = DecimPlanInfo();
    if ((L == 0 ? k.n_raw : k.n_dec) == 0) return SDRHIP_OK;
    const bool cen = fcpos == SDRHIP_FC_CEN;
    if (L == 0 || (!cen && L <= 2)) {
        if (k.frame_mode) return fail(SDRHIP_EINVAL, L == 0 ? "internal: frame mode needs log2decim >= 1" : "internal: frame mode unsupported for filter-less decimation");
        hipError_t e = simple();
        if (e != hipSuccess) return fail(SDRHIP_EDEVICE, "decimate%u launch: %s", 1u << L, hipGetErrorString(e));
        return SDRHIP_OK;
    }

    DecimArgs a;
    memset(&a, 0, sizeof(a));
    a.in = k.in; a.out = k.out; a.in_stride = k.in_stride; a.out_stride = k.out_stride;
    a.state_cur = d->state[d->cur].as<int32_t>(); a.state_next = d->state[d->cur ^ 1].as<int32_t>();
    a.nstreams = d->nstreams;
    a.bias = d->bias;
    a.frame_mode = k.frame_mode; a.frame_blocks = k.frame_blocks;
    a.mf_dump = c->decim_dump;
    bool mfma = false;
    if (int rc = plan(a, &mfma)) return rc;
    const bool pack16 = cen && d->stage0_int16;
    hipError_t e;
    {
        KTimer kt(c, SDRHIP_K_DECIMATE);
        e = launch(a, pack16, mfma);
    }
    if (e != hipSuccess) return fail(SDRHIP_EDEVICE, "decimate launch: %s", hipGetErrorString(e));
    d->last.path = mfma ? DECIM_PATH_MFMA : DECIM_PATH_VALU;
    if (mfma) {
        d->last.span = a.mf_span; d->last.head = a.mf_head; d->last.tail_start = a.mf_tail_start;
        d->last.wps = a.mf_wps; d->last.npieces = a.mf_npieces;
    } else {
        d->last.nseg = a.nseg;
    }
    d->cur ^= 1;
    d->stage0_int16 = cen && (d->stage0_int16 || k.min_used >= (size_t)2 * DEC_HIST);
    return SDRHIP_OK;
}
}

namespace sdrhip {
int decimate_device(sdrhip_decimators *d, int log2decim, int fcpos, unsigned *sampleSize, const int16_t *in, size_t n_in,
                    size_t in_stride, int16_t *out, size_t out_stride, size_t *n_out, int frame_mode, int frame_blocks,
                    uint64_t frame_sample_base, const RxMeta *meta, const Enc128Args *fuse, bool *fused, bool coresident)
{
    if (fused) *fused = false;
    sdrhip_ctx *c = d->ctx;
    const int S = d->nstreams;
    const unsigned L = (unsigned)log2decim;
    const DecimShifts sh = decimated_shifts(L, *sampleSize);
    const size_t n_dec = n_in >> L;
    const size_t n_used = n_dec << L;
    *sampleSize = decimated_sample_size(L, *sampleSize);
    if (n_out) *n_out = n_dec;
    const DecimCall k = {in, in_stride, out, out_stride, frame_mode, frame_blocks, n_in, n_dec, n_used};
    return decimate_core(
        d, L, fcpos, k,
        [&]() { return launch_decimate_simple(log2decim, fcpos, in, in_stride, out, out_stride, n_in, S, (int)sh.norm, (int)sh.trunk, c->stream); },
        [&](DecimArgs &a, bool *mfma) -> int {
            a.n_used = n_used;
            a.norm = (int)sh.norm; a.trunk = (int)sh.trunk;
            a.frame_sample_base = frame_sample_base;
            if (meta) set_meta_args(a, *meta);
            plan_decimate(log2decim, fcpos, n_used, S, &a.nsub_per_seg, &a.nseg);
            const CtxOptions &env = c->opt;
            const bool mfma_frames = env.rx_direct && out_stride * 4 < 0x3fffffffu;
            a.mf_ring = coresident ? 3 : env.mfma_ring;
            a.mf_prio = coresident ? 1 : 0;
            MfPlan p;
            *mfma = (!frame_mode || mfma_frames) && mfma_admitted(env.decim_path, env.mfma_min, log2decim, n_used * (size_t)S) &&
                    plan_decimate_mfma(log2decim, fcpos, n_used, S, env.mfma_span, c->n_cu, a.mf_ring, &p);
            if (*mfma) set_mf_args(a, p);
            return SDRHIP_OK;
        },
        [&](const DecimArgs &a, bool pack16, bool mfma) -> hipError_t {
            if (!(mfma && fuse && L <= 4))
                return mfma ? launch_decimate_mfma(log2decim, pack16, a, c->stream) : launch_decimate(log2decim, fcpos, pack16, a, c->stream);
            hipError_t e;
            if (++c->fused_tag == 0xffffffffu) {
                (void)hipMemsetAsync(c->fused_roles, 0, SDRHIP_FUSED_ROLE_WORDS * 4, c->stream);
                c->fused_tag = 1;
            }
            if (c->opt.rx_fused == 2) {
                Enc128Args none = *fuse;
                none.nlist = 0;
                e = launch_rx_fused(log2decim, pack16, a, none, c->fused_roles, c->fused_tag, c->stream);
                if (e == hipSuccess) e = launch_gf_encode128(*fuse, c->stream);
            } else
                e = launch_rx_fused(log2decim, pack16, a, *fuse, c->fused_roles, c->fused_tag, c->stream);
            if (e != hipSuccess) {
                (void)hipMemsetAsync(c->fused_roles, 0, SDRHIP_FUSED_ROLE_WORDS * 4, c->stream);
                c->fused_tag = 0;
            }
            if (fused) *fused = true;
            return e;
        });
}

bool decimate_mfma_applies(const sdrhip_decimators *d, int log2decim, int fcpos, size_t n_in)
{
    const CtxOptions &env = d->ctx->opt;
    const size_t n_used = (n_in >> log2decim) << log2decim;
    MfPlan p;
    return mfma_admitted(env.decim_path, env.mfma_min, log2decim, n_used * (size_t)d->nstreams) &&
           plan_decimate_mfma(log2decim, fcpos, n_used, d->nstreams, env.mfma_span, d->ctx->n_cu, env.mfma_ring, &p);
}
}

extern "C" int sdrhip_decimate(sdrhip_decimators *d, int log2decim, int fcpos, unsigned *sampleSize, const int16_t *iq_in,
                               size_t n_in, size_t in_stride, int16_t *iq_out, size_t out_stride, size_t *n_out, int mem)
{
    if (!d || !sampleSize) return fail(SDRHIP_EINVAL, "decimate: NULL handle or sampleSize");
    sdrhip::CtxLock lock_(d->ctx);
    if (log2decim < 0 || log2decim > 6) return fail(SDRHIP_EINVAL, "Invalid log2 decimation factor");
    if (fcpos < SDRHIP_FC_INF || fcpos > SDRHIP_FC_CEN) return fail(SDRHIP_EINVAL, "Invalid Fc position index");
    if (*sampleSize < 1 || *sampleSize > 16) return fail(SDRHIP_EINVAL, "sampleSize must be 1..16");
    if (n_in && (!iq_in || (!iq_out && (n_in >> log2decim)))) return fail(SDRHIP_EINVAL, "decimate: NULL buffer");
    sdrhip_ctx *c = d->ctx;
    HIP_TRY(hipSetDevice(c->device));
    const int S = d->nstreams;
    const size_t n_res = n_in >> log2decim;
    if (S == 1) { in_stride = n_in; out_stride = n_res; }
    if (S > 1 && (in_stride < n_in || out_stride < n_res)) return fail(SDRHIP_EINVAL, "decimate: stride smaller than the per-stream length");

    if (mem == SDRHIP_MEM_DEVICE) {
        if (n_in && (!aligned16(iq_in) || !aligned16(iq_out) || (S > 1 && ((in_stride & 3) || (out_stride & 3)))))
            return fail(SDRHIP_EALIGN, "decimate: device pointers must be 16-byte aligned and strides multiples of 4 samples");
        return decimate_device(d, log2decim, fcpos, sampleSize, iq_in, n_in, in_stride, iq_out, out_stride, n_out, 0, 0, 0);
    }
    if (int e = check_mem(mem)) return e;

    const size_t dis = (n_in + 3) & ~(size_t)3, dos = (n_res + 3) & ~(size_t)3;
    if (n_in == 0)
        return decimate_device(d, log2decim, fcpos, sampleSize, nullptr, 0, 0, nullptr, 0, n_out, 0, 0, 0);
    int rc;
    if ((size_t)S * dis * 4 <= SDRHIP_ZEROCOPY_MAX) {
        if ((rc = c->zin.reserve((size_t)S * dis * 4 + 16))) return rc;
        if ((rc = c->zout.reserve((size_t)S * dos * 4 + 16))) return rc;
        for (int s = 0; s < S; ++s) memcpy(c->zin.as<int16_t>() + (size_t)s * dis * 2, iq_in + (size_t)s * in_stride * 2, n_in * 4);
        link_bytes(c, hipMemcpyHostToDevice, (size_t)S * n_in * 4);
        link_bytes(c, hipMemcpyDeviceToHost, (size_t)S * n_res * 4);
        rc = decimate_device(d, log2decim, fcpos, sampleSize, c->zin.as<int16_t>(), n_in, dis, c->zout.as<int16_t>(), dos, n_out, 0, 0, 0);
        if (rc) return rc;
        HIP_TRY(hipStreamSynchronize(c->stream));
        for (int s = 0; s < S && n_res; ++s) memcpy(iq_out + (size_t)s * out_stride * 2, c->zout.as<int16_t>() + (size_t)s * dos * 2, n_res * 4);
        return SDRHIP_OK;
    }
    if ((rc = c->in.reserve((size_t)S * dis * 4 + 16))) return rc;
    if ((rc = c->out.reserve((size_t)S * dos * 4 + 16))) return rc;
    HIP_TRY(link_copy2d(c, c->in.p, dis * 4, iq_in, in_stride * 4, n_in * 4, S, hipMemcpyHostToDevice, c->stream));
    rc = decimate_device(d, log2decim, fcpos, sampleSize, static_cast<const int16_t *>(c->in.p), n_in, dis,
                         static_cast<int16_t *>(c->out.p), dos, n_out, 0, 0, 0);
    if (rc) return rc;
    if (n_res) HIP_TRY(link_copy2d(c, iq_out, out_stride * 4, c->out.p, dos * 4, n_res * 4, S, hipMemcpyDeviceToHost, c->stream));
    HIP_TRY(hipStreamSynchronize(c->stream));
    return SDRHIP_OK;
}

namespace sdrhip {
int ragged_prepare(sdrhip_decimators *d, int log2decim, int fcpos, const size_t *n_in, RaggedRow *rows, const RaggedRow **rows_dev,
                   RaggedPlan *plan, PinnedBuf *pin)
{
    sdrhip_ctx *c = d->ctx;
    const int S = d->nstreams;
    size_t total = 0;
    for (int s = 0; s < S; ++s) {
        rows[s].n_raw = n_in[s];
        rows[s].n_dec = n_in[s] >> log2decim;
        rows[s].n_used = (uint64_t)(n_in[s] >> log2decim) << log2decim;
        total += (size_t)rows[s].n_used;
    }
    if (!plan_decimate_ragged(log2decim, fcpos, rows, S, total, &plan->nsub, &plan->grid)) return fail(SDRHIP_EINVAL, "ragged call: too many segments");
    const CtxOptions &env = c->opt;
    plan->ring = env.mfma_ring == 3 ? 3 : 4;
    plan->mfma = mfma_admitted(env.decim_path, env.mfma_min, log2decim, total) &&
                 plan_decimate_mfma_ragged(log2decim, fcpos, rows, S, env.mfma_span, c->n_cu, plan->ring, &plan->mf);
    const size_t bytes = (size_t)S * sizeof(RaggedRow);
    int rc;
    PinnedBuf &tab = pin ? *pin : d->rows_pin;
    if ((rc = tab.reserve(bytes))) return rc;
    if ((rc = d->rows_dev.reserve(bytes))) return rc;
    memcpy(tab.p, rows, bytes);
    HIP_TRY(hipMemcpyAsync(d->rows_dev.p, tab.p, bytes, hipMemcpyHostToDevice, c->stream));
    tab.mark(c->stream);
    *rows_dev = d->rows_dev.as<RaggedRow>();
    return SDRHIP_OK;
}

int ragged_reserve(sdrhip_decimators *d, PinnedBuf *pin)
{
    const size_t bytes = (size_t)d->nstreams * sizeof(RaggedRow);
    if (int rc = (pin ? *pin : d->rows_pin).reserve(bytes)) return rc;
    return d->rows_dev.reserve(bytes);
}

int decimate_ragged_device(sdrhip_decimators *d, int log2decim, int fcpos, unsigned *sampleSize, const int16_t *in, size_t in_stride,
                           int16_t *out, size_t out_stride, const RaggedRow *rows, const RaggedRow *rows_dev, const RaggedPlan &plan,
                           int frame_mode, int frame_blocks, const unsigned *meta_w, unsigned meta_rate)
{
    sdrhip_ctx *c = d->ctx;
    const int S = d->nstreams;
    const unsigned L = (unsigned)log2decim;
    size_t max_raw = 0, max_dec = 0, min_used = SIZE_MAX;
    for (int s = 0; s < S; ++s) {
        if (rows[s].n_raw > max_raw) max_raw = (size_t)rows[s].n_raw;
        if (rows[s].n_dec > max_dec) max_dec = (size_t)rows[s].n_dec;
        if (rows[s].n_used < min_used) min_used = (size_t)rows[s].n_used;
    }
    for (int s = 0; s < S; ++s) sampleSize[s] = decimated_sample_size(L, sampleSize[s]);
    const DecimCall k = {in, in_stride, out, out_stride, frame_mode, frame_blocks, max_raw, max_dec, min_used};
    return decimate_core(
        d, L, fcpos, k,
        [&]() { return launch_decimate_simple_ragged(log2decim, fcpos, in, in_stride, out, out_stride, max_raw, S, 0, 0, rows_dev, c->stream); },
        [&](DecimArgs &a, bool *mfma) -> int {
            if (frame_mode && !plan.mfma) return fail(SDRHIP_EINVAL, "internal: ragged frame mode needs the matrix-core launch");
            a.nsub_per_seg = plan.nsub; a.nseg = plan.grid;
            a.meta_rate = meta_rate;
            if (meta_w) memcpy(a.meta_w, meta_w, sizeof(a.meta_w));
            if (plan.mfma) {
                set_mf_args(a, plan.mf);
                a.mf_ring = plan.ring;
            }
            *mfma = plan.mfma;
            return SDRHIP_OK;
        },
// ... 102 lines not shown
```

### sdrdaemon_amd/csrc/sdrhip_host.h

```cpp
#pragma once
#include "../../include/sdrhip.h"
#include "dev_buffers.h"
#include "rx_stream_settings.h"
#include "sdrhip_internal.h"

#include <cstdint>
#include <cstring>
#include <atomic>
#include <map>
#include <mutex>
#include <string>
#include <utility>
#include <vector>

namespace sdrhip {

#define HIP_TRY(expr)                                                                                           \
    do {                                                                                                        \
        hipError_t e_ = (expr);                                                                                 \
        if (e_ != hipSuccess) return ::sdrhip::fail(SDRHIP_EDEVICE, "%s: %s", #expr, hipGetErrorString(e_));    \
    } while (0)

constexpr size_t SDRHIP_ZEROCOPY_MAX = (size_t)384 << 10;

inline bool aligned16(const void *p) { return (reinterpret_cast<uintptr_t>(p) & 15u) == 0; }
inline int check_mem(int mem)
{
    return mem == SDRHIP_MEM_HOST || mem == SDRHIP_MEM_DEVICE ? SDRHIP_OK : fail(SDRHIP_EINVAL, "mem must be SDRHIP_MEM_HOST or SDRHIP_MEM_DEVICE");
}

struct RxMeta {
    int first, count;
    unsigned frame_count0;
    unsigned w[6];
    uint64_t idx0;
    unsigned rate;
    const unsigned *tab;
};

int decimate_device(sdrhip_decimators *d, int log2decim, int fcpos, unsigned *sampleSize, const int16_t *in, size_t n_in,
                    size_t in_stride, int16_t *out, size_t out_stride, size_t *n_out, int frame_mode, int frame_blocks,
                    uint64_t frame_sample_base, const RxMeta *meta = nullptr, const Enc128Args *fuse = nullptr, bool *fused = nullptr,
                    bool coresident = false);
int ragged_prepare(sdrhip_decimators *d, int log2decim, int fcpos, const size_t *n_in, RaggedRow *rows, const RaggedRow **rows_dev,
                   RaggedPlan *plan, PinnedBuf *pin = nullptr);
int ragged_reserve(sdrhip_decimators *d, PinnedBuf *pin);
int decimate_ragged_device(sdrhip_decimators *d, int log2decim, int fcpos, unsigned *sampleSize, const int16_t *in, size_t in_stride,
                           int16_t *out, size_t out_stride, const RaggedRow *rows, const RaggedRow *rows_dev, const RaggedPlan &plan,
                           int frame_mode = 0, int frame_blocks = 0, const unsigned *meta_w = nullptr, unsigned meta_rate = 0);
int ragged_stage_in(sdrhip_ctx *c, PinnedBuf &pin, DevBuf &dev, const void *src, size_t in_stride, const size_t *n_in, int S, size_t esz,
                    size_t dstride, const void **out);
int ctx_stream2(sdrhip_ctx *c, hipStream_t *out);
bool decimate_mfma_applies(const sdrhip_decimators *d, int log2decim, int fcpos, size_t n_in);
struct InterpGather {
    const unsigned *map;
    const uint8_t *rx, *restored;
    int frames;
};
bool interpolate_gather_ok(const sdrhip_ctx *c, int log2interp);
struct InterpCount {
    const int *count;
    int stride, unit;
};
int interpolate_device(sdrhip_interpolators *p, int log2interp, const int16_t *in, size_t n_in, size_t in_stride, int16_t *out,
                       size_t out_stride, size_t *n_out, const InterpGather *gather = nullptr, const InterpCount *count = nullptr,
                       int out_fmt = IQF_S16,
                       const int *fmt_dev = nullptr);
int fecbuf_check_dgrams(const sdrhip_fecbuf *b, const uint8_t *dgrams, const size_t *n_dgrams, size_t dgram_stride_bytes, int mem, const char *who);
struct FecBufJoin {
    const unsigned *row_off;
    int (*admit)(void *arg, const size_t *n_frames);
    void *arg;
};
int fecbuf_collect(sdrhip_fecbuf *b, const uint8_t *dgrams, const size_t *n_dgrams, size_t dgram_stride_bytes, int mem, uint8_t *data_out,
                   size_t data_stride_bytes, uint8_t *block0_out, size_t max_frames, sdrhip_fecbuf_frame *info_out, size_t *n_frames,
                   const int **counts, const FecBufJoin *join = nullptr, const uint8_t *staged = nullptr);
int fecbuf_join_carry(sdrhip_fecbuf *b, unsigned **dev, std::vector<size_t> **host);
const FecBufState *fecbuf_committed_state(const sdrhip_fecbuf *b);
struct FecBufShadow {
    int head, count, recov, maxrow, dup;
    unsigned pres[4];
};
int fecbuf_shadow(sdrhip_fecbuf *b, std::vector<FecBufShadow> *out);
void fecbuf_shadow_run(FecBufShadow &h, const uint8_t *dg, size_t n, int res[4]);
void fecbuf_shadow_step(FecBufShadow &h, uint32_t hd, int res[4]);
int fecbuf_packed(sdrhip_fecbuf *b, const uint8_t *dg, const size_t *n_dgrams, const int *res, const std::vector<FecBufShadow> &next,
                  PinnedBuf &tab, uint8_t *data_out, size_t data_stride, uint8_t *block0_out, size_t max_frames, unsigned *mismatch,
                  bool *committed, const int **counts, const FecBufPub **pub, const FecBufJoin *join = nullptr);
struct FecBufBatch {
    int S;
    const uint8_t *dgrams;
    const size_t *n_dgrams;
    size_t stride;
    bool packed, inplace;
    size_t sum, nmax, bytes_in;
    size_t dev_bytes;
    const uint16_t *tags = nullptr;
    size_t n_total = 0;
    std::vector<size_t> counts;
    uint32_t *dest = nullptr;
};
int fecbuf_batch_check(FecBufBatch *in, int S, const uint8_t *dgrams, const size_t *n_dgrams, size_t dgram_stride_bytes, const char *who);
int fecbuf_batch_check_tagged(FecBufBatch *in, int S, const uint8_t *dgrams, const uint16_t *stream_of, size_t n_total, const char *who);
int fecbuf_batch_stage(FecBufBatch *in, PinnedBuf &arena, PinnedBuf &tab, std::vector<FecBufShadow> &sh, int *res);
int fecbuf_batch_upload(sdrhip_ctx *c, const FecBufBatch &in, PinnedBuf &arena, uint8_t *pk);
int fecbuf_tag_counts(int S, const uint8_t *dgrams, const uint16_t *stream_of, size_t n_total, const char *who, size_t *counts, size_t *sum,
                      size_t *nmax);
int fecbuf_batch_lost(const char *who, int rc);
constexpr size_t DG_REC = sizeof(sdrhip_fecbuf_frame);
static_assert(sizeof(sdrhip_fecbuf_frame) == sizeof(FecBufPub), "public record layout");
inline int reserve_settled(sdrhip_ctx *c, DevBuf &b, size_t n);
constexpr int DEC_STATS_SHADOW_MISMATCH = 1;
void fecbuf_set_async_busy(sdrhip_fecbuf *b, bool busy);
struct EncodeLin {
    const unsigned *lin;
    size_t stride;
    int cap, first, pending;
};
int enc128_min_rows(const sdrhip_ctx *c);
inline bool fec_encode_fuses_framing(const sdrhip_ctx *c, int nb_fec) { return nb_fec >= enc128_min_rows(c); }
int fec_encode_device(sdrhip_ctx *ctx, const uint8_t *frames, size_t frame_bytes, size_t nframes, int nb_fec, uint8_t *rec,
                      size_t rec_frame_bytes, const int32_t *frame_list_dev = nullptr, int ngroups = 0, const EncodeLin *lin = nullptr);
int fec_encode128_launch(sdrhip_ctx *ctx, const Enc128Args &k, hipStream_t on = nullptr);
struct DecodeSide {
    hipStream_t stream;
    DevBuf *plan, *idx;
    PinnedBuf *pin;
};
struct DecodeGather {
    unsigned *srcmap;
    uint8_t *restored;
    int rows;
};
bool fec_decode_gather_ok(const sdrhip_ctx *c);
int fec_decode_device(sdrhip_ctx *ctx, const uint8_t *rx, size_t rx_frame_bytes, const uint8_t *indices, size_t nframes,
                      uint8_t *payload_out, size_t payload_frame_bytes, uint8_t *block0_out, const DecodeSide *side = nullptr,
                      const DecodeGather *gather = nullptr, int max_rows = 0);
bool host_is_pinned(const void *p, size_t n);

typedef TableVersions StreamMask;
int stream_mask_upload(sdrhip_ctx *c, StreamMask &m, const uint8_t *mask, int S, const uint8_t **dev, int *n_set);
void decimators_reset_part(sdrhip_decimators *d, StreamResetArgs *a);
void decimators_reset_done(sdrhip_decimators *d, bool all);
void interpolators_reset_part(sdrhip_interpolators *p, StreamResetArgs *a);
void fecbuf_reset_part(sdrhip_fecbuf *b, StreamResetArgs *a);
void fecbuf_reset_done(sdrhip_fecbuf *b, const uint8_t *mask);
void fecbuf_fresh_state(FecBufState *x);
int stream_reset_launch(sdrhip_ctx *c, const StreamResetArgs &a);
int32_t *decimators_row(sdrhip_decimators *d, int s, int half);
int32_t *interpolators_row(sdrhip_interpolators *p, int s, int half);
bool decimators_stage0_int16(const sdrhip_decimators *d);
void decimators_clear_stage0_int16(sdrhip_decimators *d);
struct FecBufStreamRef {
    FecBufState *st[2];
    uint8_t *carry;
    size_t carry_half;
};
void fecbuf_stream_ref(sdrhip_fecbuf *b, int s, FecBufStreamRef *out);
void fecbuf_import_host(sdrhip_fecbuf *b, int s, const FecBufState &st, size_t carry);

}

#define SDRHIP_KCLASSES 5
namespace sdrhip {
struct CtxOptions {
    int decim_path = DECIM_PATH_AUTO;
    size_t mfma_span = 0;
    size_t mfma_min = (size_t)1 << 22;
    int interp_wave = 1;
    size_t interp_span = 0;
    int mfma_ring = 4;
    int rx_fused = 1;
    int rx_direct = 1;
    int rx_window = 0;
    int tx_overlap = 1;
    int enc_fft = 1;
    int enc_half = 0;
    int enc_bitslice = 1;
    int enc_min_rows = 1;
    int fec_stagger_mod = 0;
    int fec_stagger = 0;
    int tx_gather = 0;
    int dec_fused_plan = 1;
    int dec_syndrome = 1;
    int dec_strict = 0;
    int dec_max_rows = 128;
    int dec_auto = 0;
};
struct DecimPlanInfo {
    int path = 0;
    size_t span = 0, head = 0, tail_start = 0;
    int wps = 0, npieces = 0, nseg = 0;
};
}

struct sdrhip_ctx {
    std::recursive_mutex mtx;
    int device = 0;
    int n_cu = 256;
    sdrhip::CtxOptions opt;
    hipStream_t stream = nullptr;
    hipStream_t stream2 = nullptr;
    std::atomic<int> refs{0};
    std::atomic<bool> dying{false};
    sdrhip::DevBuf in, out, aux, aux3;
    uint8_t *gf_tab = nullptr;
    uint8_t *enc_matrix = nullptr;
    uint8_t *enc_leaves = nullptr;
    uint8_t *enc_fft = nullptr;
    unsigned *decim_dump = nullptr;
    unsigned *fused_roles = nullptr;
    unsigned fused_tag = 0;
    hipEvent_t ev0 = nullptr, ev1 = nullptr;
    uint8_t *gf_explog = nullptr;
    sdrhip::DevBuf dec_plan;
    unsigned *dec_stats = nullptr;
    sdrhip::PinnedBuf pin;
    sdrhip::PinnedBuf zin, zout;
    bool ktime_on = false;
    int ktime_stride = 1;
    int ktime_stride_cls[SDRHIP_KCLASSES] = {0, 0, 0, 0, 0};
    unsigned ktime_seen[SDRHIP_KCLASSES] = {0, 0, 0, 0, 0};
    std::vector<std::pair<hipEvent_t, hipEvent_t>> kev[SDRHIP_KCLASSES];
    uint64_t h2d_bytes = 0, d2h_bytes = 0;
};

namespace sdrhip {
struct CtxLock {
    std::lock_guard<std::recursive_mutex> g;
    explicit CtxLock(sdrhip_ctx *c) : g(c->mtx) {}
};
struct KTimer {
    sdrhip_ctx *c;
    int cls;
    hipEvent_t e1 = nullptr;
    hipStream_t st;
    KTimer(sdrhip_ctx *ctx, int kernel_class, hipStream_t on = nullptr) : c(ctx), cls(kernel_class), st(on ? on : ctx->stream)
    {
        if (!c->ktime_on) return;
        if (cls >= 0 && cls < SDRHIP_KCLASSES) {
            const int stride = c->ktime_stride_cls[cls] > 0 ? c->ktime_stride_cls[cls] : c->ktime_stride;
            if (stride > 1 && (c->ktime_seen[cls]++ % (unsigned)stride) != 0) return;
        }
        hipEvent_t e0 = nullptr;
        if (hipEventCreate(&e0) != hipSuccess) return;
        if (hipEventCreate(&e1) != hipSuccess) { (void)hipEventDestroy(e0); e1 = nullptr; return; }
        (void)hipEventRecord(e0, st);
        c->kev[cls].push_back(std::make_pair(e0, e1));
    }
    ~KTimer()
    {
        if (e1) (void)hipEventRecord(e1, st);
    }
};
inline int reserve_settled(sdrhip_ctx *c, DevBuf &b, size_t n)
{
    if (n > b.cap && b.p && hipStreamSynchronize(c->stream) != hipSuccess) return fail(SDRHIP_EDEVICE, "hipStreamSynchronize");
    return b.reserve(n);
}
inline void link_bytes(sdrhip_ctx *c, hipMemcpyKind kind, size_t bytes)
{
    if (kind == hipMemcpyHostToDevice) c->h2d_bytes += bytes;
    else if (kind == hipMemcpyDeviceToHost) c->d2h_bytes += bytes;
}
inline hipError_t link_copy(sdrhip_ctx *c, void *dst, const void *src, size_t bytes, hipMemcpyKind kind, hipStream_t stream)
{
    const hipError_t e = hipMemcpyAsync(dst, src, bytes, kind, stream);
    if (e == hipSuccess) link_bytes(c, kind, bytes);
    return e;
}
inline hipError_t link_copy2d(sdrhip_ctx *c, void *dst, size_t dpitch, const void *src, size_t spitch, size_t width, size_t height,
                              hipMemcpyKind kind, hipStream_t stream)
{
    const hipError_t e = hipMemcpy2DAsync(dst, dpitch, src, spitch, width, height, kind, stream);
    if (e == hipSuccess) link_bytes(c, kind, width * height);
    return e;
}
template <class F, class D> int stream_reset_bank(sdrhip_ctx *c, StreamMask &m, const uint8_t *mask, int S, F fill, D done)
{
    HIP_TRY(hipSetDevice(c->device));
    StreamResetArgs a;
    memset(&a, 0, sizeof(a));
    int n_set = 0;
    if (int rc = stream_mask_upload(c, m, mask, S, &a.mask, &n_set)) return rc;
    if (n_set == 0) return SDRHIP_OK;
    a.nstreams = S;
    fill(&a);
    if (int rc = stream_reset_launch(c, a)) return rc;
    done(n_set == S ? nullptr : mask);
    return SDRHIP_OK;
}
}
```

### sdrdaemon_amd/csrc/sdrhip_internal.h

```cpp
#pragma once
#include <hip/hip_runtime.h>
#include <stddef.h>
#include <stdint.h>

#include "decim_plan.h"
#include "interp_pick.h"
#include "rx_depart_order.h"
#include "rx_egress_order.h"
#include "rx_unpack_plan.h"

#ifndef SDRHIP_NT
#define SDRHIP_NT 1
#endif
#if SDRHIP_NT
#define SDRHIP_STREAM_LOAD(ptr) __builtin_nontemporal_load(ptr)
#else
#define SDRHIP_STREAM_LOAD(ptr) (*(ptr))
#endif

namespace sdrhip {

constexpr int DEC_STAGES = 6;
constexpr int DEC_HIST = 32;
constexpr int DEC_STATE_WORDS = DEC_STAGES * 4 * DEC_HIST;

constexpr int INT_STAGES = 6;
constexpr int INT_HIST = 32;
constexpr int INT_STATE_WORDS = INT_STAGES * 2 * INT_HIST;

struct DecimArgs {
    const int16_t *in;
    int16_t *out;
    size_t in_stride;
    size_t out_stride;
    size_t n_used;
    const int32_t *state_cur;
    int32_t *state_next;
    int nstreams;
    int nsub_per_seg;
    int nseg;
    int bias;
    int norm, trunk;
    int frame_mode;
    int frame_blocks;
    uint64_t frame_sample_base;
    int meta_first, meta_count;
    unsigned meta_frame_count0;
    unsigned meta_w[6];
    uint64_t meta_idx0;
    unsigned meta_rate;
    size_t mf_head, mf_span, mf_tail_start, mf_tail_seg;
    int mf_wps, mf_npieces;
    int mf_piece_wgs, mf_piece_early, mf_piece_share;
    unsigned *mf_dump;
    int mf_ring;
    int mf_prio;
    const unsigned *meta_tab;
};
template <class Args, class Meta> inline void set_meta_args(Args &a, const Meta &m)
{
    a.meta_first = m.first; a.meta_count = m.count; a.meta_frame_count0 = m.frame_count0;
    for (int i = 0; i < 6; ++i) a.meta_w[i] = m.w[i];
    a.meta_idx0 = m.idx0; a.meta_rate = m.rate; a.meta_tab = m.tab;
}

constexpr int STREAM_META_WORDS = 3;
#if defined(__HIPCC__) && __cplusplus >= 201703L
struct CrcBitTable { unsigned c[64]; };
constexpr CrcBitTable make_crc_bit_table()
{
    CrcBitTable T{};
    for (int k = 0; k < 64; ++k) {
        unsigned crc = 0u;
        for (int byte = 0; byte < 20; ++byte) {
            unsigned v = 0u;
            if (byte >= 12 && byte == 12 + k / 8) v = 1u << (k % 8);
            crc ^= v;
            for (int b = 0; b < 8; ++b) crc = (crc >> 1) ^ (0xEDB88320u & (0u - (crc & 1u)));
        }
        T.c[k] = crc;
    }
    return T;
}
__device__ const CrcBitTable CRC_BIT = make_crc_bit_table();

__device__ __forceinline__ void frame_meta_words(const unsigned (&base)[6], uint64_t idx0, unsigned rate, int fi, unsigned (&w)[6])
{
    unsigned sec = base[3], usec = base[4];
    if (rate) {
        const uint64_t idx = idx0 + (uint64_t)fi * 16129u;
        const uint64_t dus = idx * 1000000ull / rate;
        const uint64_t ds = dus / 1000000ull;
        usec += (unsigned)(dus - ds * 1000000ull);
        sec += (unsigned)ds;
        if (usec >= 1000000u) { usec -= 1000000u; sec += 1u; }
    }
    w[0] = base[0]; w[1] = base[1]; w[2] = base[2]; w[3] = sec; w[4] = usec;
    const int lane = (int)(threadIdx.x & 63u);
    const unsigned word = lane < 32 ? sec : usec;
    unsigned x = ((word >> (lane & 31)) & 1u) ? CRC_BIT.c[lane] : 0u;
#pragma unroll
    for (int m = 32; m >= 1; m >>= 1) x ^= (unsigned)__shfl_xor((int)x, m, 64);
    w[5] = base[5] ^ x;
}
__device__ __forceinline__ void frame_meta_words_thread(const unsigned (&base)[6], uint64_t idx0, unsigned rate, int fi, unsigned (&w)[6])
{
    unsigned sec = base[3], usec = base[4];
    if (rate) {
        const uint64_t idx = idx0 + (uint64_t)fi * 16129u;
        const uint64_t dus = idx * 1000000ull / rate;
        const uint64_t ds = dus / 1000000ull;
        usec += (unsigned)(dus - ds * 1000000ull);
        sec += (unsigned)ds;
        if (usec >= 1000000u) { usec -= 1000000u; sec += 1u; }
    }
    w[0] = base[0]; w[1] = base[1]; w[2] = base[2]; w[3] = sec; w[4] = usec;
    unsigned x = 0u;
#pragma unroll 8
    for (int k = 0; k < 32; ++k) {
        x ^= (0u - ((sec >> k) & 1u)) & CRC_BIT.c[k];
        x ^= (0u - ((usec >> k) & 1u)) & CRC_BIT.c[32 + k];
    }
    w[5] = base[5] ^ x;
}
template <bool ROW = false>
__device__ __forceinline__ void stream_meta_base(const unsigned (&shared)[6], unsigned shared_rate, const unsigned *p, int stream,
                                                 unsigned (&base)[6], unsigned &rate)
{
#pragma unroll
    for (int k = 0; k < 6; ++k) base[k] = shared[k];
    rate = shared_rate;
    if (ROW || p) {
        const unsigned *t = ROW ? p : p + (size_t)STREAM_META_WORDS * (size_t)__builtin_amdgcn_readfirstlane(stream);
        base[0] = t[0]; base[1] = t[1]; base[5] = t[2];
        if (ROW) base[2] = t[3];
        rate = t[1];
    }
}
#endif

hipError_t launch_decimate(int log2decim, int fcpos, bool pack16, const DecimArgs &a, hipStream_t stream);
hipError_t launch_decimate_mfma(int log2decim, bool pack16, const DecimArgs &a, hipStream_t stream);
struct Enc128Args;
constexpr int SDRHIP_FUSED_ROLE_WORDS = 4096 + 8;
hipError_t launch_rx_fused(int log2decim, bool pack16, const DecimArgs &a, const Enc128Args &e, unsigned *roles, unsigned tag, hipStream_t stream);

hipError_t launch_decimate_simple(int log2decim, int fcpos, const int16_t *in, size_t in_stride, int16_t *out,
                                  size_t out_stride, size_t n_in, int nstreams, int norm, int trunk,
                                  hipStream_t stream);

struct RaggedRow {
    uint64_t n_raw;
    uint64_t n_used;
    uint64_t n_dec;
    uint64_t out_off;
    uint64_t frame_sample_base;
    uint64_t meta_idx0;
    int seg0;
    int meta_first, meta_count;
    unsigned frame_count0;
    unsigned tv_sec, tv_usec;
    int mf_w0, mf_wps, mf_p0, mf_np;
    uint64_t mf_head, mf_tail_start;
    unsigned fc, rate, crc0;
    unsigned w2;
    unsigned shifts;
};
static_assert(sizeof(RaggedRow) == 128, "RaggedRow: one 128-byte row per stream");
hipError_t launch_decimate_mfma_ragged(int log2decim, bool pack16, const DecimArgs &a, const RaggedRow *rows, hipStream_t stream);
hipError_t launch_decimate_ragged(int log2decim, int fcpos, bool pack16, const DecimArgs &a, const RaggedRow *rows, hipStream_t stream);
hipError_t launch_decimate_simple_ragged(int log2decim, int fcpos, const int16_t *in, size_t in_stride, int16_t *out,
                                         size_t out_stride, size_t n_in, int nstreams, int norm, int trunk, const RaggedRow *rows,
                                         hipStream_t stream);

struct TestSourceParams {
    unsigned phase0;
    unsigned inc;
    int amp;
};
hipError_t launch_testsource(const int *table, const TestSourceParams *par, int16_t *out, size_t out_stride, size_t n, int nstreams,
                             hipStream_t stream);

struct FrameArgs {
    const unsigned *in;
    unsigned *out;
    size_t in_stride, out_stride;
    size_t n;
    size_t skip_from, skip_to;
    uint64_t frame_sample_base;
    int frame_blocks;
    int meta_first, meta_count;
    unsigned meta_frame_count0;
    unsigned meta_w[6];
    uint64_t meta_idx0;
    unsigned meta_rate;
    const unsigned *meta_tab;
};
hipError_t launch_frame_pack(const FrameArgs &a, int nstreams, hipStream_t stream);
hipError_t launch_frame_pack_ragged(const FrameArgs &a, const RaggedRow *rows, int nstreams, hipStream_t stream);
hipError_t launch_frame_meta_ragged(const FrameArgs &a, const RaggedRow *rows, int max_started, int nstreams, hipStream_t stream);

struct InterpArgs {
    const int16_t *in;
    int16_t *out;
    size_t in_stride, out_stride;
    size_t n_in;
    const int32_t *state_cur;
    int32_t *state_next;
    int nstreams;
    int nsub_per_seg, nseg;
// ... 273 lines not shown
```

### sdrdaemon_amd/csrc/sdrhip_rx.cpp

```cpp
#include "sdrhip_pipes.h"

using namespace sdrhip;

static int rx_check_config(const sdrhip_rx_config *cfg);

extern "C" int sdrhip_rx_create(sdrhip_ctx *ctx, int nstreams, const sdrhip_rx_config *cfg, sdrhip_rx **out)
{
    if (!ctx || !cfg || !out || nstreams <= 0) return fail(SDRHIP_EINVAL, "rx_create: bad argument");
    {
        const int rcc = rx_check_config(cfg);
        if (rcc) return rcc;
    }
    sdrhip_rx *rx = new (std::nothrow) sdrhip_rx(ctx);
    if (!rx) return fail(SDRHIP_ENOMEM, "out of host memory");
    rx->nstreams = nstreams; rx->cfg = *cfg;
    rx->area.init((size_t)nstreams);
    rx->view.init((size_t)nstreams);
    rx->streams.init((size_t)nstreams);
    int rc = sdrhip_decimators_create(ctx, nstreams, cfg->hb_variant, &rx->dec);
    if (rc) { delete rx; return rc; }
    *out = rx;
    return SDRHIP_OK;
}

static int rx_check_config(const sdrhip_rx_config *cfg)
{
    if (cfg->log2decim < 0 || cfg->log2decim > 6) return fail(SDRHIP_EINVAL, "Invalid log2 decimation factor");
    if (cfg->fcpos < 0 || cfg->fcpos > 2) return fail(SDRHIP_EINVAL, "Invalid Fc position index");
    if (cfg->nb_fec < 0 || cfg->nb_fec > 128) return fail(SDRHIP_EINVAL, "nb_fec must be 0..128");
    if (cfg->sample_bits < 1 || cfg->sample_bits > 16) return fail(SDRHIP_EINVAL, "sample_bits must be 1..16");
    return SDRHIP_OK;
}

static int rx_settle(sdrhip_rx *rx)
{
    if (!rx->late.encode) return SDRHIP_OK;
    rx->late.encode = false;
    sdrhip_ctx *c = rx->ctx;
    if (c->opt.rx_fused != 3 || !rx->ev_framed) return fec_encode128_launch(c, rx->late.k);
    hipStream_t s2 = nullptr;
    int rc = ctx_stream2(c, &s2);
    if (rc) return rc;
    if ((rc = rx->ev_enc.ensure())) return rc;
    HIP_TRY(hipStreamWaitEvent(s2, rx->ev_framed, 0));
    if ((rc = fec_encode128_launch(c, rx->late.k, s2))) return rc;
    HIP_TRY(hipEventRecord(rx->ev_enc, s2));
    HIP_TRY(hipStreamWaitEvent(c->stream, rx->ev_enc, 0));
    return SDRHIP_OK;
}

extern "C" int sdrhip_rx_set_pipelined(sdrhip_rx *rx, int on)
{
    if (!rx) return fail(SDRHIP_EINVAL, "rx is NULL");
    sdrhip::CtxLock lock_(rx->ctx);
    if (!on && rx->late.have) return fail(SDRHIP_EINVAL, "rx_set_pipelined: sdrhip_rx_flush the waiting frames first");
    if (on && rx_refuse_uniform("rx_set_pipelined", nullptr, rx->streams.forces_ragged())) return SDRHIP_EINVAL;
    if (on && rx_dgrams_in_flight(rx)) return fail(SDRHIP_EINVAL, "rx_set_pipelined: asynchronous datagram batches are in flight: collect them first");
    if (on && !rx->area.aligned()) return fail(SDRHIP_EINVAL, "rx_set_pipelined: ragged calls left the streams at different frame positions");
    rx->pipelined = on ? 1 : 0;
    return SDRHIP_OK;
}

extern "C" int sdrhip_rx_set_input_format(sdrhip_rx *rx, int fmt)
{
    if (!rx) return fail(SDRHIP_EINVAL, "rx is NULL");
    sdrhip::CtxLock lock_(rx->ctx);
    if (fmt != SDRHIP_IQ_S16 && fmt != SDRHIP_IQ_U8 && fmt != SDRHIP_IQ_S8) return fail(SDRHIP_EINVAL, "rx_set_input_format: unknown format %d", fmt);
    if (rx->ring.busy()) return fail(SDRHIP_EINVAL, "rx_set_input_format: asynchronous batches are being filled or in flight: collect them first");
    if (rx->late.have) return fail(SDRHIP_EINVAL, "rx_set_input_format: frames of the previous call wait for delivery (pipelined mode): sdrhip_rx_flush them first");
    rx->in_fmt = fmt;
    return SDRHIP_OK;
}

static int rx_widen(sdrhip_rx *rx, const uint8_t *in, size_t in_stride, size_t n_in, size_t dstride, const int16_t **din)
{
    sdrhip_ctx *c = rx->ctx;
    int rc = rx->wide.reserve((size_t)rx->nstreams * dstride * 4 + 16);
    if (rc) return rc;
    hipError_t e;
    {
        KTimer kt(c, SDRHIP_K_CONVERT);
        e = launch_iq8_widen(rx->in_fmt, in, in_stride, rx->wide.as<int16_t>(), dstride, n_in, rx->nstreams, c->stream);
    }
    if (e != hipSuccess) return fail(SDRHIP_EDEVICE, "widen launch: %s", hipGetErrorString(e));
    *din = rx->wide.as<int16_t>();
    return SDRHIP_OK;
}

static int rx_release_old(sdrhip_rx *rx)
{
    if (rx->old_work.p && !(rx->late.have && rx->late.in_old)) {
        HIP_TRY(hipStreamSynchronize(rx->ctx->stream));
        rx->old_work.release();
    }
    return SDRHIP_OK;
}

static int rx_run_plan(sdrhip_rx *rx, const RxAreaPlan &p, DevBuf *fresh, size_t src_pitch, size_t dst_pitch, size_t bytes, const char *who)
{
    sdrhip_ctx *c = rx->ctx;
    const RxFrameArea &A = rx->area;
    const size_t S = A.streams(), dcap = fresh ? p.new_cap : A.cap();
    const uint8_t *src = rx->work.as<uint8_t>();
    uint8_t *dst = fresh ? fresh->as<uint8_t>() : rx->work.as<uint8_t>();
    bool together = true;
    for (size_t s = 0; s < S; ++s) together = together && p.to_slot0[s] && A.open(s) && A.slot(s) == A.slot(0);
    hipError_t e = hipSuccess;
    if (together)
        e = hipMemcpy2DAsync(dst, dcap * dst_pitch, src + A.slot(0) * src_pitch, A.cap() * src_pitch, bytes, S, hipMemcpyDeviceToDevice, c->stream);
    else
        for (size_t s = 0; s < S && e == hipSuccess; ++s)
            if (p.to_slot0[s] && A.open(s))
                e = hipMemcpyAsync(dst + s * dcap * dst_pitch, src + A.index(s) * src_pitch, bytes, hipMemcpyDeviceToDevice, c->stream);
    if (e == hipSuccess && fresh) e = hipStreamSynchronize(c->stream);
    if (e != hipSuccess) {
        if (fresh) { (void)hipStreamSynchronize(c->stream); fresh->release(); }
        return fail(SDRHIP_EDEVICE, "%s: moving the open frames: %s", who, hipGetErrorString(e));
    }
    if (fresh) {
        if (p.keep_old) { rx->old_work = std::move(rx->work); rx->late.in_old = true; }
        rx->work = std::move(*fresh);
        rx->view.clear();
    }
    rx->area.moved(p);
    return SDRHIP_OK;
}

static int rx_make_room(sdrhip_rx *rx, const size_t *done, bool pipelined, const char *who, bool grow_only = false)
{
    sdrhip_ctx *c = rx->ctx;
    const size_t wmul = c->opt.rx_window ? (size_t)c->opt.rx_window : pipelined ? 4 : 2;
    const RxAreaPlan p = rx->area.plan(done, rx->late.have && !rx->late.in_old ? rx->late.first : RX_NO_LATE, wmul);
    if (!p.new_cap && (grow_only || !p.moves())) return SDRHIP_OK;
    const size_t fb = rx_frame_bytes(rx);
    DevBuf fresh;
    if (p.new_cap)
        if (int rc = fresh.reserve(rx->area.streams() * p.new_cap * fb)) return rc;
    return rx_run_plan(rx, p, p.new_cap ? &fresh : nullptr, fb, fb, fb, who);
}

static int rx_repitch(sdrhip_rx *rx, size_t new_fb, const char *who)
{
    if (!rx->area.cap() || new_fb == rx_frame_bytes(rx)) return SDRHIP_OK;
    int rc;
    if ((rc = rx_settle(rx))) return rc;
    DevBuf fresh;
    if ((rc = fresh.reserve(rx->area.streams() * rx->area.cap() * new_fb))) return rc;
    if ((rc = rx_run_plan(rx, rx->area.replan(), &fresh, rx_frame_bytes(rx), new_fb, (size_t)SDRHIP_NB_ORIGINAL * SDRHIP_UDPSIZE, who))) return rc;
    rx->old_work.release();
    return SDRHIP_OK;
}

extern "C" int sdrhip_rx_reconfigure(sdrhip_rx *rx, const sdrhip_rx_config *cfg)
{
    if (!rx || !cfg) return fail(SDRHIP_EINVAL, "rx_reconfigure: NULL argument");
    sdrhip::CtxLock lock_(rx->ctx);
    int rc = rx_check_config(cfg);
    if (rc) return rc;
    if (cfg->hb_variant != rx->cfg.hb_variant) return fail(SDRHIP_EINVAL, "rx_reconfigure: hb_variant is fixed at creation");
    sdrhip_ctx *c = rx->ctx;
    HIP_TRY(hipSetDevice(c->device));
    const bool fec_changes = rx->streams.forces_ragged() != RX_SET_FEC && cfg->nb_fec != rx->cfg.nb_fec;
    if (fec_changes && rx->late.have)
        return fail(SDRHIP_EINVAL, "rx_reconfigure: frames of the previous call wait for delivery (pipelined mode): sdrhip_rx_flush them "
                                   "before changing fecblk (they carry the old frame size)");
    if (fec_changes && (rc = rx_repitch(rx, (size_t)(SDRHIP_NB_ORIGINAL + cfg->nb_fec) * SDRHIP_UDPSIZE, "rx_reconfigure"))) return rc;
    rx->cfg = *cfg;
    return SDRHIP_OK;
}

extern "C" void sdrhip_rx_destroy(sdrhip_rx *rx)
{
    if (!rx) return;
    sdrhip_ctx *c = rx->ctx;
    (void)hipSetDevice(c->device);
    (void)hipStreamSynchronize(c->stream);
    if (c->stream2) (void)hipStreamSynchronize(c->stream2);
    rx->ring.wait_all();
    sdrhip_decimators_destroy(rx->dec);
    sdrhip_fecbuf_destroy(rx->fb);
    delete rx;
}

extern "C" int sdrhip_rx_frames_view(const sdrhip_rx *rx, const uint8_t **base, size_t *stream_stride_bytes, size_t *n_frames)
{
    if (!rx || !base || !stream_stride_bytes || !n_frames) return fail(SDRHIP_EINVAL, "rx_frames_view: NULL argument");
    sdrhip::CtxLock lock_(rx->ctx);
    if (!rx->view.uniform()) return fail(SDRHIP_EINVAL, "rx_frames_view: the last call's windows differ between streams: use sdrhip_rx_frames_view_ragged");
    *base = rx->view.window(0, rx_frame_bytes(rx));
    *stream_stride_bytes = rx->view.stride();
    *n_frames = rx->view.frames(0);
    return SDRHIP_OK;
}

extern "C" int sdrhip_rx_frames_view_ragged(const sdrhip_rx *rx, const uint8_t **base, size_t *stream_stride_bytes, size_t *first_slot,
                                            size_t *n_frames)
{
    if (!rx || !base || !stream_stride_bytes || !first_slot || !n_frames) return fail(SDRHIP_EINVAL, "rx_frames_view_ragged: NULL argument");
    sdrhip::CtxLock lock_(rx->ctx);
    *base = rx->view.base();
    *stream_stride_bytes = rx->view.stride();
    for (size_t s = 0; s < (size_t)rx->nstreams; ++s) { first_slot[s] = rx->view.first(s); n_frames[s] = rx->view.frames(s); }
    return SDRHIP_OK;
}

extern "C" int sdrhip_rx_last_plan(const sdrhip_rx *rx, sdrhip_decim_plan *out)
{
    if (!rx) return fail(SDRHIP_EINVAL, "rx is NULL");
    return sdrhip_decimators_last_plan(rx->dec, out);
}

extern "C" size_t sdrhip_rx_max_frames(const sdrhip_rx *rx, size_t n_in)
{
    if (!rx) return 0;
    sdrhip::CtxLock lock_(rx->ctx);
    size_t now = 0;
    for (size_t s = 0; s < (size_t)rx->nstreams; ++s) {
        const size_t f = rx->area.advance(s, n_in >> rx->cfg.log2decim).done;
        if (f > now) now = f;
    }
    if (!rx->pipelined) return now;
    return rx->late.have && rx->late.frames > now ? rx->late.frames : now;
}

static int rx_deliver(sdrhip_rx *rx, const uint8_t *area, size_t first, size_t stride, size_t frames, size_t frame_bytes, uint8_t *frames_out,
                      size_t frame_stride_bytes, size_t *n_frames, int mem)
{
    sdrhip_ctx *c = rx->ctx;
    const int S = rx->nstreams;
    const uint8_t *base = area + first * frame_bytes;
    if (frames && frames_out) {
        if (S > 1 && frame_stride_bytes < frames * frame_bytes) return fail(SDRHIP_EINVAL, "rx_process: frame stride too small");
        HIP_TRY(link_copy2d(c, frames_out, S > 1 ? frame_stride_bytes : frames * frame_bytes, base, stride, frames * frame_bytes, S,
                            mem == SDRHIP_MEM_HOST ? hipMemcpyDeviceToHost : hipMemcpyDeviceToDevice, c->stream));
    } else if (frames && mem != SDRHIP_MEM_DEVICE) {
        return fail(SDRHIP_EINVAL, "rx_process: NULL frames_out");
    }
    rx->view.set(area, stride, (size_t)S, first, frames);
    if (n_frames) *n_frames = frames;
    return SDRHIP_OK;
}

extern "C" int sdrhip_rx_flush(sdrhip_rx *rx, uint8_t *frames_out, size_t frame_stride_bytes, size_t *n_frames, int mem)
{
    if (!rx) return fail(SDRHIP_EINVAL, "rx is NULL");
    sdrhip::CtxLock lock_(rx->ctx);
    if (n_frames) *n_frames = 0;
    if (int e = check_mem(mem)) return e;
    if (!rx->late.have) { rx->view.clear(); return SDRHIP_OK; }
    HIP_TRY(hipSetDevice(rx->ctx->device));
    int rc;
    if ((rc = rx_settle(rx))) return rc;
    if ((rc = rx_deliver(rx, rx->late.area, rx->late.first, rx->late.stride, rx->late.frames, rx->late.frame_bytes, frames_out, frame_stride_bytes, n_frames, mem))) return rc;
    rx->late.have = false;
    if (mem == SDRHIP_MEM_HOST) HIP_TRY(hipStreamSynchronize(rx->ctx->stream));
    return SDRHIP_OK;
}

static void rx_meta_base(const sdrhip_rx_config &cfg, unsigned ssd, unsigned w[6])
{
    rx_meta_record(cfg.center_frequency_khz, cfg.sample_rate, cfg.nb_fec, ssd, w);
}

static int rx_set_done(const RxSetResult &r, const char *who, const char *what, const char *range)
{
    if (r.kind == RxSetResult::RANGE) return fail(SDRHIP_EINVAL, "%s: %s[%zu] = %ld, must be %s", who, what, r.index, r.value, range);
    return r.kind == RxSetResult::NO_MEMORY ? fail(SDRHIP_ENOMEM, "out of host memory") : SDRHIP_OK;
}
static int rx_check_stream(const sdrhip_rx *rx, int stream, const char *who)
{
    return stream < 0 || stream >= rx->nstreams ? fail(SDRHIP_EINVAL, "%s: stream %d of %d", who, stream, rx->nstreams) : SDRHIP_OK;
}

extern "C" int sdrhip_rx_set_stream_meta(sdrhip_rx *rx, const uint32_t *center_frequency_khz, const uint32_t *sample_rate)
{
    if (!rx) return fail(SDRHIP_EINVAL, "rx is NULL");
    sdrhip::CtxLock lock_(rx->ctx);
    return rx_set_done(rx->streams.set_meta(center_frequency_khz, sample_rate), "rx_set_stream_meta", "", "");
}

extern "C" int sdrhip_rx_set_follow_meta(sdrhip_rx *rx, int on)
{
    if (!rx) return fail(SDRHIP_EINVAL, "rx is NULL");
    sdrhip::CtxLock lock_(rx->ctx);
    rx->follow_meta = on ? 1 : 0;
// ... 22 lines not shown
{
    if (!rx) return fail(SDRHIP_EINVAL, "rx is NULL");
    sdrhip::CtxLock lock_(rx->ctx);
    if (rx->pipelined || rx->late.have) return fail(SDRHIP_EINVAL, "rx_set_stream_fec: not available in pipelined mode");
    if (rx_batches_active(rx)) return fail(SDRHIP_EINVAL, "rx_set_stream_fec: asynchronous batches are being filled or in flight: collect them first");
    if (rx->ring.busy()) return fail(SDRHIP_EINVAL, "rx_set_stream_fec: a batch is lent (sdrhip_rx_collect_egress): sdrhip_rx_release_egress it first");
    if (int rc = rx_set_done(rx->streams.admit_fec(nb_fec), "rx_set_stream_fec", "nb_fec", "0..128")) return rc;
    HIP_TRY(hipSetDevice(rx->ctx->device));
    if (int rc = rx_repitch(rx, rx->streams.slot_blocks_of(nb_fec, rx_bank(rx)) * SDRHIP_UDPSIZE, "rx_set_stream_fec")) return rc;
    return rx_set_done(rx->streams.set_fec(nb_fec), "rx_set_stream_fec", "nb_fec", "0..128");
}

extern "C" int sdrhip_rx_get_stream_fec(const sdrhip_rx *rx, int stream, int *nb_fec, int *slot_blocks)
{
    if (!rx) return fail(SDRHIP_EINVAL, "rx is NULL");
    sdrhip::CtxLock lock_(rx->ctx);
    if (int e = rx_check_stream(rx, stream, "rx_get_stream_fec")) return e;
    if (nb_fec) *nb_fec = rx_fec_of(rx, (size_t)stream);
    if (slot_blocks) *slot_blocks = (int)(rx_frame_bytes(rx) / SDRHIP_UDPSIZE);
    return SDRHIP_OK;
}

extern "C" int sdrhip_rx_set_stream_bits(sdrhip_rx *rx, const unsigned *sample_bits)
{
    if (!rx) return fail(SDRHIP_EINVAL, "rx is NULL");
    sdrhip::CtxLock lock_(rx->ctx);
    if (rx->pipelined || rx->late.have) return fail(SDRHIP_EINVAL, "rx_set_stream_bits: not available in pipelined mode");
    return rx_set_done(rx->streams.set_bits(sample_bits), "rx_set_stream_bits", "sample_bits", "1..16");
}

extern "C" int sdrhip_rx_get_stream_bits(const sdrhip_rx *rx, int stream, unsigned *sample_bits, unsigned *frame_bits)
{
    if (!rx) return fail(SDRHIP_EINVAL, "rx is NULL");
    sdrhip::CtxLock lock_(rx->ctx);
    if (int e = rx_check_stream(rx, stream, "rx_get_stream_bits")) return e;
    const unsigned b = rx_bits_of(rx, (size_t)stream);
    if (sample_bits) *sample_bits = b;
    if (frame_bits) *frame_bits = decimated_sample_size((unsigned)rx->cfg.log2decim, b);
    return SDRHIP_OK;
}

extern "C" int sdrhip_rx_set_stream_format(sdrhip_rx *rx, const int *fmt)
{
    if (!rx) return fail(SDRHIP_EINVAL, "rx is NULL");
    sdrhip::CtxLock lock_(rx->ctx);
    if (rx->pipelined || rx->late.have) return fail(SDRHIP_EINVAL, "rx_set_stream_format: not available in pipelined mode");
    if (rx->ring.busy()) return fail(SDRHIP_EINVAL, "rx_set_stream_format: asynchronous batches are being filled or in flight: collect them first");
    return rx_set_done(rx->streams.set_format(fmt), "rx_set_stream_format", "fmt", "SDRHIP_IQ_S16, SDRHIP_IQ_U8 or SDRHIP_IQ_S8");
}

extern "C" int sdrhip_rx_get_stream_format(const sdrhip_rx *rx, int stream, int *fmt)
{
    if (!rx) return fail(SDRHIP_EINVAL, "rx is NULL");
    sdrhip::CtxLock lock_(rx->ctx);
    if (int e = rx_check_stream(rx, stream, "rx_get_stream_format")) return e;
    if (fmt) *fmt = rx->streams.format(rx->in_fmt, (size_t)stream);
    return SDRHIP_OK;
}

static int rx_stream_table(sdrhip_rx *rx, const unsigned **dev)
{
    *dev = nullptr;
    const RxStreamRecords *r = rx->streams.records(rx_bank(rx));
    if (!r) return SDRHIP_OK;
    if (rx->streams.changed()) {
        const void *tab = nullptr;
        if (int rc = rx->sm_tab.upload(rx->ctx->stream, r->words.data(), r->words.size() * sizeof(unsigned), &tab)) return rc;
        rx->streams.taken();
    }
    *dev = static_cast<const unsigned *>(rx->sm_tab.current());
    return SDRHIP_OK;
}

static int rx_stage_in(sdrhip_ctx *c, const void *src, size_t in_stride, size_t n_in, int S, size_t esz, size_t dstride, const void **out)
{
    int rc;
    if ((size_t)S * dstride * esz <= SDRHIP_ZEROCOPY_MAX) {
        if ((rc = c->zin.reserve((size_t)S * dstride * esz + 16))) return rc;
        for (int s = 0; s < S; ++s) memcpy(c->zin.as<char>() + (size_t)s * dstride * esz, static_cast<const char *>(src) + (size_t)s * in_stride * esz, n_in * esz);
        link_bytes(c, hipMemcpyHostToDevice, (size_t)S * n_in * esz);
        *out = c->zin.p;
    } else {
        if ((rc = c->in.reserve((size_t)S * dstride * esz + 16))) return rc;
        HIP_TRY(link_copy2d(c, c->in.p, dstride * esz, src, in_stride * esz, n_in * esz, S, hipMemcpyHostToDevice, c->stream));
        *out = c->in.p;
    }
    return SDRHIP_OK;
}

extern "C" int sdrhip_rx_process(sdrhip_rx *rx, const int16_t *iq_in, size_t n_in, size_t in_stride, uint32_t tv_sec, uint32_t tv_usec,
                                 uint8_t *frames_out, size_t frame_stride_bytes, size_t *n_frames, int mem)
{
    if (!rx) return fail(SDRHIP_EINVAL, "rx is NULL");
    sdrhip::CtxLock lock_(rx->ctx);
    if (n_frames) *n_frames = 0;
    if (int e = rx_refuse_uniform("rx_process", "sdrhip_rx_process_ragged", rx->streams.forces_ragged())) return e;
    if (rx_has_batches(rx, true)) return fail(SDRHIP_EINVAL, "rx_process: ragged batches are being filled or in flight: collect them first");
    if (rx_dgrams_in_flight(rx)) return fail(SDRHIP_EINVAL, "rx_process: asynchronous datagram batches are in flight: collect them first");
    if (n_in && !rx->area.aligned()) {
        const size_t S = (size_t)rx->nstreams;
        std::vector<size_t> cnt(S, n_in), nf(S, 0);
        std::vector<uint32_t> sec(S, tv_sec), usec(S, tv_usec);
        const int rc = rx_ragged(rx, iq_in, rx_counts(rx, cnt.data()), in_stride, sec.data(), usec.data(), frames_out, frame_stride_bytes, nf.data(), mem);
        if (rc) return rc;
        size_t most = 0;
        for (size_t s = 0; s < S; ++s) if (nf[s] > most) most = nf[s];
        if (n_frames) *n_frames = most;
        return SDRHIP_OK;
    }
    if (n_in == 0) {
        if (rx->pipelined && rx->late.have) return sdrhip_rx_flush(rx, frames_out, frame_stride_bytes, n_frames, mem);
        rx->view.clear();
        return SDRHIP_OK;
    }
    if (!iq_in) return fail(SDRHIP_EINVAL, "rx_process: NULL input");
    sdrhip_ctx *c = rx->ctx;
    rx->consumed = false;
    HIP_TRY(hipSetDevice(c->device));
    const int S = rx->nstreams, L = rx->cfg.log2decim, R = rx->cfg.nb_fec;
    const int FB = SDRHIP_NB_ORIGINAL + R;
    const size_t frame_bytes = (size_t)FB * SDRHIP_UDPSIZE;
    const size_t n_dec = n_in >> L;
    const uint64_t pending = rx->area.pending(0);
    const RxAdvance adv = rx->area.advance(0, n_dec);
    const size_t done = adv.done;
    if (S == 1) in_stride = n_in;
    const size_t deliver_now = rx->pipelined ? (rx->late.have ? rx->late.frames : 0) : done;
    const size_t deliver_fb = rx->pipelined && rx->late.have ? rx->late.frame_bytes : frame_bytes;
    if (deliver_now && !frames_out && mem != SDRHIP_MEM_DEVICE) return fail(SDRHIP_EINVAL, "rx_process: NULL frames_out");
    if (frames_out && S > 1 && deliver_now && frame_stride_bytes < deliver_now * deliver_fb) return fail(SDRHIP_EINVAL, "rx_process: frame stride too small");

    const int16_t *din = iq_in;
    size_t dstride = in_stride;
    int rc;
    const bool wide8 = rx->in_fmt != IQF_S16;
    const void *src = iq_in;
    if ((rc = check_mem(mem))) return rc;
    if (mem == SDRHIP_MEM_HOST) {
        dstride = wide8 ? (n_in + 7) & ~(size_t)7 : (n_in + 3) & ~(size_t)3;
        if ((rc = rx_stage_in(c, iq_in, in_stride, n_in, S, wide8 ? 2 : 4, dstride, &src))) return rc;
    } else if (!aligned16(iq_in) || (S > 1 && (in_stride & (wide8 ? 7 : 3)))) {
        return wide8 ? fail(SDRHIP_EALIGN, "rx_process: 8-bit device input must be 16-byte aligned, its stride a multiple of 8 samples")
                     : fail(SDRHIP_EALIGN, "rx_process: device input must be 16-byte aligned");
    }
    din = static_cast<const int16_t *>(src);
    if (wide8) {
        const size_t sstride = dstride;
        dstride = (n_in + 3) & ~(size_t)3;
        if ((rc = rx_widen(rx, static_cast<const uint8_t *>(src), sstride, n_in, dstride, &din))) return rc;
    }

    const std::vector<size_t> dones((size_t)S, done);
    if ((rc = rx_release_old(rx))) return rc;
    if ((rc = rx_make_room(rx, dones.data(), rx->pipelined != 0, "rx_process"))) return rc;
    const size_t cap = rx->area.cap(), slot0 = rx->area.slot(0);
    const size_t stream_bytes = cap * frame_bytes;
    uint8_t *work = rx->work.as<uint8_t>() + slot0 * frame_bytes;

    unsigned ss = rx->cfg.sample_bits;
    RxMeta meta;
    memset(&meta, 0, sizeof(meta));
    if (adv.started > 0) {
        rx_meta_base(rx->cfg, decimated_sample_size((unsigned)L, ss), meta.w);
        if ((rc = rx_stream_table(rx, &meta.tab))) return rc;
        meta.w[3] = tv_sec; meta.w[4] = tv_usec;
        meta.first = adv.first_new; meta.count = adv.started; meta.frame_count0 = adv.frame_count0;
        meta.idx0 = adv.idx0;
        meta.rate = rx->cfg.sample_rate;
    }

    size_t n_out = 0;
    EncodeLin elin;
    bool use_lin = false, pack_with_encoder = false;
    FrameArgs fa;
    memset(&fa, 0, sizeof(fa));
    const bool structured = R >= enc128_min_rows(c) && frame_bytes % 4 == 0;
    const bool filterless = L == 0 || (rx->cfg.fcpos != SDRHIP_FC_CEN && L <= 2);
    const Enc128Args *fuse = rx->late.encode && (c->opt.rx_fused == 1 || c->opt.rx_fused == 2) ? &rx->late.k : nullptr;
    const bool coresident = rx->late.encode && c->opt.rx_fused == 3 && rx->ev_framed;
    bool fused = false;
    const bool direct = c->opt.rx_direct && !rx->pipelined && stream_bytes < 0x3fffffffu;
    if (filterless || (!direct && decimate_mfma_applies(rx->dec, L, rx->cfg.fcpos, n_in))) {
        const size_t lstride = (n_dec + 3) & ~(size_t)3;
        if (rx->pipelined) rx->lin_sel ^= 1;
        DevBuf &lin = rx->lin[rx->lin_sel];
        if (lin.cap < (size_t)S * lstride * 4 + 16 && rx->late.encode) { if ((rc = rx_settle(rx))) return rc; fuse = nullptr; HIP_TRY(hipStreamSynchronize(c->stream)); }
        if ((rc = lin.reserve((size_t)S * lstride * 4 + 16))) return rc;
        rc = decimate_device(rx->dec, L, rx->cfg.fcpos, &ss, din, n_in, dstride, lin.as<int16_t>(), lstride, &n_out, 0, 0, 0, nullptr, fuse, &fused, coresident);
        if (rc) return rc;
        rx->consumed = true;
        if (fused) rx->late.encode = false;
        if (fec_encode_fuses_framing(c, R)) {
            const size_t first = pending ? 1 : 0;
            if (done > first && frame_bytes % 4 == 0) {
                elin.lin = lin.as<unsigned>(); elin.stride = lstride; elin.cap = (int)cap;
                elin.first = (int)first; elin.pending = (int)pending;
                use_lin = true;
            }
        }
        if (use_lin) {
            fa.skip_from = (size_t)elin.first * SDRHIP_SAMPLES_PER_FRAME - (size_t)elin.pending;
            fa.skip_to = done * SDRHIP_SAMPLES_PER_FRAME - (size_t)elin.pending;
        }
        fa.in = lin.as<unsigned>(); fa.out = reinterpret_cast<unsigned *>(work);
        fa.in_stride = lstride; fa.out_stride = stream_bytes / 4;
        fa.n = n_dec; fa.frame_sample_base = pending; fa.frame_blocks = FB;
        set_meta_args(fa, meta);
        pack_with_encoder = !rx->pipelined && c->opt.rx_fused && structured && R > 0 && use_lin;
        if (!pack_with_encoder) {
            hipError_t e = launch_frame_pack(fa, S, c->stream);
            if (e != hipSuccess) return fail(SDRHIP_EDEVICE, "frame pack launch: %s", hipGetErrorString(e));
        }
    } else {
        rc = decimate_device(rx->dec, L, rx->cfg.fcpos, &ss, din, n_in, dstride, reinterpret_cast<int16_t *>(work), stream_bytes / 4, &n_out, 1,
                             FB, pending, &meta);
        if (rc) return rc;
        rx->consumed = true;
    }
    if ((rc = rx_settle(rx))) return rc;

    bool encode_later = false;
    Enc128Args k;
    memset(&k, 0, sizeof(k));
    if (done && R > 0) {
        if (structured) {
            k.in = work; k.out = work + (size_t)SDRHIP_NB_ORIGINAL * SDRHIP_UDPSIZE; k.tab = c->gf_tab; k.leaf_tables = c->enc_leaves; k.fft_tables = c->enc_fft; k.use_fft = c->opt.enc_fft;
            k.bitslice = c->opt.enc_bitslice;
            k.in_frame_bytes = frame_bytes; k.out_frame_bytes = frame_bytes;
            k.rows = R; k.nframes = (int)((size_t)S * cap);
            k.nlist = (int)((size_t)S * done); k.gen_done = (int)done; k.gen_cap = (int)cap;
            if (use_lin) { k.lin = elin.lin; k.lin_stride = elin.stride; k.lin_cap = elin.cap; k.lin_first = elin.first; k.lin_pending = elin.pending; }
            if (rx->pipelined) {
                encode_later = true;
            } else if (pack_with_encoder) {
                set_meta_args(k, meta);
                if (elin.first == 1) { k.lin_straddle = 1; fa.skip_from = 0; }
                hipError_t e;
                {
                    KTimer kt(c, SDRHIP_K_FEC_ENCODE);
                    e = launch_gf_encode128_pack(k, fa, S, c->stream);
                }
                if (e != hipSuccess) return fail(SDRHIP_EDEVICE, "encode + frame pack launch: %s", hipGetErrorString(e));
            } else if ((rc = fec_encode128_launch(c, k))) return rc;
        } else {
            if (rx->flist_done != done || rx->flist_cap != cap) {
                HIP_TRY(hipStreamSynchronize(c->stream));
                rx->flist_host.clear();
                for (int s = 0; s < S; ++s)
                    for (size_t f = 0; f < done; ++f) rx->flist_host.push_back((int32_t)(s * cap + f));
                while (rx->flist_host.size() % GF_FRAMES_PER_GROUP) rx->flist_host.push_back(-1);
                if ((rc = rx->flist.reserve(rx->flist_host.size() * 4))) return rc;
                HIP_TRY(link_copy(c, rx->flist.p, rx->flist_host.data(), rx->flist_host.size() * 4, hipMemcpyHostToDevice, c->stream));
                rx->flist_done = done; rx->flist_cap = cap;
            }
            if ((rc = fec_encode_device(c, work, frame_bytes, (size_t)S * cap, R, work + (size_t)SDRHIP_NB_ORIGINAL * SDRHIP_UDPSIZE,
                                        frame_bytes, rx->flist.as<int32_t>(), (int)(rx->flist_host.size() / GF_FRAMES_PER_GROUP), nullptr)))
                return rc;
        }
    }
    if (rx->pipelined) {
        if (rx->late.have) {
            if ((rc = rx_deliver(rx, rx->late.area, rx->late.first, rx->late.stride, rx->late.frames, rx->late.frame_bytes, frames_out, frame_stride_bytes, n_frames, mem))) return rc;
        } else {
            rx->view.clear();
        }
        rx->late.have = done > 0;
        rx->late.encode = encode_later;
        if (encode_later && c->opt.rx_fused == 3) {
            if ((rc = rx->ev_framed.ensure())) return rc;
            HIP_TRY(hipEventRecord(rx->ev_framed, c->stream));
        }
        rx->late.k = k;
        rx->late.area = rx->work.as<uint8_t>(); rx->late.first = slot0; rx->late.in_old = false;
        rx->late.stride = stream_bytes; rx->late.frames = done; rx->late.frame_bytes = frame_bytes;
    } else {
        if ((rc = rx_deliver(rx, rx->work.as<uint8_t>(), slot0, stream_bytes, done, frame_bytes, frames_out, frame_stride_bytes, n_frames, mem))) return rc;
    }
    rx->area.commit(dones.data(), std::vector<uint64_t>((size_t)S, adv.rest).data());
    if (mem == SDRHIP_MEM_HOST) HIP_TRY(hipStreamSynchronize(c->stream));
    return SDRHIP_OK;
}

int sdrhip::rx_area_room(sdrhip_rx *rx, const size_t *done)
{
    return rx_make_room(rx, done ? done : std::vector<size_t>(rx->area.streams(), 0).data(), false, "rx_process_ragged", true);
}

static size_t rx_flist_entries(size_t sum_done) { return (sum_done / GF_FRAMES_PER_GROUP + 3) * GF_FRAMES_PER_GROUP; }
static int rx_encode_form(const sdrhip_ctx *c, int rows) { return rows < enc128_min_rows(c) ? 0 : rows <= 32 ? 1 : 2; }

int sdrhip::rx_ragged_room(sdrhip_rx *rx, const RxRaggedCounts &n, RxTabs *tabs)
{
    const int S = rx->nstreams, L = rx->cfg.log2decim;
    int rc;
    if ((rc = rx_area_room(rx, n.done.data()))) return rc;
    if ((rc = ragged_reserve(rx->dec, tabs ? &tabs->rows : nullptr))) return rc;
    const bool may_direct = rx->cfg.fcpos == SDRHIP_FC_CEN && L >= 2 && rx->ctx->opt.rx_direct;
    if (!may_direct && (rc = rx->lin[0].reserve((size_t)S * ((n.max_dec + 3) & ~(size_t)3) * 4 + 16))) return rc;
    if (n.sum_done && rx_fec_max(rx) > 0) {
        const size_t nl = rx_flist_entries(n.sum_done);
        if ((rc = (tabs ? tabs->flist : rx->r_flist_pin).reserve(nl * 4))) return rc;
        if ((rc = rx->r_flist.reserve(nl * 4))) return rc;
    }
    return SDRHIP_OK;
}

void sdrhip::rx_pack_rows(char *dst, const void *src, size_t pitch, const size_t *n_in, const int *fmts, int bank_fmt, size_t S)
{
    const char *rows = static_cast<const char *>(src), *packed = rows;
    for (size_t s = 0; s < S; ++s) {
        const size_t bytes = n_in[s] * unpackx_sample_bytes(fmts ? fmts[s] : bank_fmt);
        if (bytes) memcpy(dst, pitch ? rows + s * pitch : packed, bytes);
        dst += bytes;
        packed += bytes;
    }
}

int sdrhip::rx_unpack_launch(sdrhip_rx *rx, PinnedBuf &pin, DevBuf &dev, size_t tab_bytes, const int *fmts, const void *src, int16_t *out,
                             size_t dstride, unsigned grid)
{
    sdrhip_ctx *c = rx->ctx;
    const int S = rx->nstreams;
    HIP_TRY(hipMemcpyAsync(dev.p, pin.p, tab_bytes, hipMemcpyHostToDevice, c->stream));
    pin.mark(c->stream);
    const UnpackXRow *rows = dev.as<UnpackXRow>();
    const UnpackXSeg *segs = reinterpret_cast<const UnpackXSeg *>(rows + S + 1);
    hipError_t e;
    {
        KTimer kt(c, SDRHIP_K_CONVERT);
        e = fmts ? launch_unpack_mixed(src, out, dstride, rows, segs, S, grid, c->stream)
                 : launch_unpack_packed(rx->in_fmt, static_cast<const uint8_t *>(src), out, dstride, rows, segs, S, grid, c->stream);
    }
    if (e != hipSuccess) return fail(SDRHIP_EDEVICE, "unpack launch: %s", hipGetErrorString(e));
    return SDRHIP_OK;
}

static int rx_unpack_rows(sdrhip_rx *rx, const int16_t *iq_in, size_t in_stride, const size_t *n_in, const int *fmts, bool in_dev,
                          const int16_t **din, size_t *dstride)
{
    sdrhip_ctx *c = rx->ctx;
    const size_t S = (size_t)rx->nstreams;
    const UnpackXPlan m = unpackx_measure(n_in, 1, S, fmts);
    size_t max_in = 0;
    for (size_t s = 0; s < S; ++s) if (n_in[s] > max_in) max_in = n_in[s];
    const size_t rows_bytes = (S + 1) * sizeof(UnpackXRow), tab_bytes = rows_bytes + (size_t)m.nseg * sizeof(UnpackXSeg);
    const size_t ds = (max_in + 7) & ~(size_t)7;
    int rc;
    if ((rc = rx->f_tab_pin.reserve(tab_bytes))) return rc;
    if ((rc = reserve_settled(c, rx->f_tab, tab_bytes))) return rc;
    if ((rc = rx->wide.reserve(S * ds * 4 + 16))) return rc;
    const void *src = iq_in;
    if (!in_dev) {
        if ((rc = rx->f_pin.reserve((size_t)m.bytes))) return rc;
        if ((rc = reserve_settled(c, rx->f_pk, (size_t)m.bytes + 64))) return rc;
        rx_pack_rows(rx->f_pin.as<char>(), iq_in, in_stride * 4, n_in, fmts, 0, S);
        HIP_TRY(link_copy(c, rx->f_pk.p, rx->f_pin.p, (size_t)m.bytes, hipMemcpyHostToDevice, c->stream));
        rx->f_pin.mark(c->stream);
        src = rx->f_pk.p;
    }
    if (!unpackx_fill(n_in, 1, S, fmts, in_dev ? 2 * (uint64_t)in_stride : 0, rx->f_tab_pin.as<UnpackXRow>(),
                      reinterpret_cast<UnpackXSeg *>(rx->f_tab_pin.as<char>() + rows_bytes)).fits)
        return fail(SDRHIP_EINVAL, "rx_process_ragged: too many samples for one launch");
    if ((rc = rx_unpack_launch(rx, rx->f_tab_pin, rx->f_tab, tab_bytes, fmts, src, rx->wide.as<int16_t>(), ds, (unsigned)m.grid))) return rc;
    *din = rx->wide.as<int16_t>();
    *dstride = ds;
    return SDRHIP_OK;
}

int sdrhip::rx_ragged(sdrhip_rx *rx, const int16_t *iq_in, const RxRaggedCounts &n, size_t in_stride, const uint32_t *tv_sec, const uint32_t *tv_usec,
                      uint8_t *frames_out, size_t frame_stride_bytes, size_t *n_frames, int mem, bool batch, bool dev_rows, RxTabs *tabs,
                      const FecBufState *follow, const FecBufState *follow_bits)
{
    sdrhip_ctx *c = rx->ctx;
    const int S = rx->nstreams, L = rx->cfg.log2decim, R = rx_fec_max(rx);
    const size_t FB = (size_t)SDRHIP_NB_ORIGINAL + (size_t)R;
    const size_t frame_bytes = FB * SDRHIP_UDPSIZE;
    const bool mixed = rx_fec_mixed(rx);
    const size_t *n_in = n.n_in, max_in = n.max_in, max_dec = n.max_dec, max_done = n.max_done, sum_done = n.sum_done;
    const std::vector<size_t> &done = n.done;
    for (int s = 0; s < S; ++s) n_frames[s] = 0;
    if (int e = check_mem(mem)) return e;
    if (rx->pipelined) return fail(SDRHIP_EINVAL, "rx_process_ragged: not available in pipelined mode");
    if (!batch && rx_batches_active(rx)) return fail(SDRHIP_EINVAL, "rx_process_ragged: asynchronous batches are being filled or in flight: collect them first");
    if (S == 1) in_stride = max_in;
    if (S > 1 && in_stride < max_in) return fail(SDRHIP_EINVAL, "rx_process_ragged: in_stride smaller than the largest count");
    if (max_in && !iq_in) return fail(SDRHIP_EINVAL, "rx_process_ragged: NULL input");
    const int *fmts = !batch && !dev_rows ? rx->streams.formats() : nullptr;
    const bool wide8 = rx->in_fmt != IQF_S16 && !batch && !dev_rows && !fmts;
    const bool in_dev = mem == SDRHIP_MEM_DEVICE || dev_rows;
    if (fmts && !unpackx_measure(n_in, 1, (size_t)S, fmts).fits) return fail(SDRHIP_EINVAL, "rx_process_ragged: too many samples for one launch");
    if (max_in && in_dev && (!aligned16(iq_in) || (S > 1 && (in_stride & (wide8 ? 7 : 3)))))
        return fail(SDRHIP_EALIGN, "rx_process_ragged: device input must be 16-byte aligned, its stride a multiple of %d samples", wide8 ? 8 : 4);
    if (int e = rx_refuse_delivery("rx_process_ragged", n, frames_out, frame_stride_bytes, mem, false)) return e;
    HIP_TRY(hipSetDevice(c->device));
    rx->consumed = false;
    if (max_in == 0) {
        rx->view.clear();
        return SDRHIP_OK;
    }
    int rc;
    if ((rc = rx_release_old(rx))) return rc;
    if ((rc = rx_make_room(rx, done.data(), false, "rx_process_ragged"))) return rc;
    const RxFrameArea &A = rx->area;
    const size_t stream_bytes = A.cap() * frame_bytes;
    uint8_t *area = rx->work.as<uint8_t>();

    std::vector<unsigned> ss((size_t)S);
    for (int s = 0; s < S; ++s) ss[(size_t)s] = rx_bits_of(rx, (size_t)s);
    unsigned mw[6];
    rx_meta_base(rx->cfg, decimated_sample_size((unsigned)L, rx->cfg.sample_bits), mw);
    const RxStreamRecords *sw = rx->streams.records(rx_bank(rx));
    std::vector<RaggedRow> rows((size_t)S);
    memset(rows.data(), 0, rows.size() * sizeof(RaggedRow));
    for (int s = 0; s < S; ++s) {
        RaggedRow &r = rows[(size_t)s];
        const RxAdvance &a = n.adv[(size_t)s];
        r.out_off = A.slot((size_t)s) * frame_bytes / 4;
        r.frame_sample_base = A.pending((size_t)s);
        const unsigned *t = sw ? &sw->words[(size_t)s * STREAM_META_WORDS] : nullptr;
        r.fc = t ? t[0] : mw[0]; r.rate = t ? t[1] : mw[1];
        r.crc0 = t ? t[2] : mw[5];
        r.w2 = sw ? sw->w2[(size_t)s] : mw[2];
        r.shifts = sw ? sw->shifts[(size_t)s] : ragged_shift_word((unsigned)L, ss[(size_t)s]);
        if (a.started > 0 && (n_in[s] >> L)) {
            r.meta_first = a.first_new; r.meta_count = a.started;
            r.frame_count0 = a.frame_count0;
            r.meta_idx0 = a.idx0;
            r.tv_sec = tv_sec[s]; r.tv_usec = tv_usec[s];
        }
    }
    const RaggedRow *rdev = nullptr;
// ... 131 lines not shown
```

Before: 1.015 million.

## Slide frame area window and fold open frame ahead to avoid device copies

Adds a sliding frame-area plan in which the window base moves forward instead of resetting to slot 0. The matrix-core decimator can then write the frame that straddles the window edge into a slot folded in front of the window, through a cursor with a wrap threshold. The goal is to remove the device-to-device memcpy of the open partial frame on each rx_process call. It adds address arithmetic to the store cursor, a more complex buffer-resource range, and a new slide plan that can grow the area differently.

```diff
diff --git a/sdrdaemon_amd/csrc/decim_body.h b/sdrdaemon_amd/csrc/decim_body.h
--- a/sdrdaemon_amd/csrc/decim_body.h
+++ b/sdrdaemon_amd/csrc/decim_body.h
@@ -52,14 +52,23 @@
     return d;
 }
 
-struct OutCtx {
+template <bool FOLD> struct OutCtxT {
+    static constexpr bool can_fold = FOLD;
     unsigned *out;
     size_t out_pos;
     bool store;
     int norm, trunk;
     int frame_mode, frame_blocks;
     uint64_t frame_sample_base;
+    unsigned fold;
 };
+using OutCtx = OutCtxT<false>;
+
+template <class OC> __device__ __forceinline__ ptrdiff_t frame_slot_dw(const OC &oc, uint64_t f)
+{
+    if constexpr (OC::can_fold) return (f == oc.fold ? (ptrdiff_t)-1 : (ptrdiff_t)f) * oc.frame_blocks * 128;
+    else return (ptrdiff_t)((size_t)f * oc.frame_blocks * 128u);
+}
 
 __device__ __forceinline__ unsigned final_pack(int i, int q, int norm, int trunk)
 {
@@ -68,7 +77,7 @@
     return ((unsigned)a & 0xffffu) | ((unsigned)b << 16);
 }
 
-__device__ __forceinline__ void store_one(const OutCtx &oc, size_t k, unsigned v)
+template <class OC> __device__ __forceinline__ void store_one(const OC &oc, size_t k, unsigned v)
 {
     if (!oc.frame_mode) {
         oc.out[k] = v;
@@ -77,11 +86,11 @@
         uint64_t f = g / 16129u;
         unsigned w = (unsigned)(g - f * 16129u);
         unsigned b = w / 127u, i = w - b * 127u;
-        oc.out[((size_t)f * oc.frame_blocks + 1 + b) * 128u + 1 + i] = v;
-    }
-}
-
-template <class G, int S> __device__ __forceinline__ void run_stage(int *lds, int tid, int valid, int fill_next, int bias, const OutCtx &oc)
+        oc.out[frame_slot_dw(oc, f) + (ptrdiff_t)((1 + b) * 128u + 1 + i)] = v;
+    }
+}
+
+template <class G, int S, class OC> __device__ __forceinline__ void run_stage(int *lds, int tid, int valid, int fill_next, int bias, const OC &oc)
 {
     constexpr bool PK = G::PK && S == 0;
     constexpr bool LAST = (S == G::NS - 1);
@@ -169,14 +178,19 @@
             const uint64_t f = g / 16129u;
             const unsigned w = (unsigned)(g - f * 16129u);
             unsigned b = w / 127u, i = w - b * 127u;
-            size_t dw = ((size_t)f * oc.frame_blocks + 1 + b) * 128u + 1 + i;
+            ptrdiff_t dw = frame_slot_dw(oc, f) + (ptrdiff_t)((1 + b) * 128u + 1 + i);
+            [[maybe_unused]] unsigned fn = (unsigned)f;
 #pragma unroll
             for (int r = 0; r < R; ++r) {
                 if (k0 + r < valid) oc.out[dw] = o[r];
                 ++i; ++dw;
                 if (i == 127u) {
                     i = 0; ++b; dw += 1;
-                    if (b == 127u) { b = 0; dw += ((size_t)oc.frame_blocks - 127u) * 128u; }
+                    if (b == 127u) {
+                        b = 0; dw += ((ptrdiff_t)oc.frame_blocks - 127) * 128;
+                        if constexpr (OC::can_fold)
+                            if (++fn == oc.fold) dw -= (ptrdiff_t)(oc.fold + 1u) * oc.frame_blocks * 128;
+                    }
                 }
             }
         }
@@ -240,7 +254,7 @@
     if constexpr (S + 1 < G::NS) state_store<G, S + 1>(lds, tid, st);
 }
 
-template <class G, int S> __device__ __forceinline__ void later_stages(int *lds, int tid, int (&fill)[6], int consumed_prev, bool flush, int bias, OutCtx &oc)
+template <class G, int S, class OC> __device__ __forceinline__ void later_stages(int *lds, int tid, int (&fill)[6], int consumed_prev, bool flush, int bias, OC &oc)
 {
     if constexpr (S < G::NS) {
         slide<G, S - 1>(lds, tid, consumed_prev);
@@ -260,7 +274,7 @@
     }
 }
 
-template <int L, int FC, bool PACK16, bool TAB = true>
+template <int L, int FC, bool PACK16, bool TAB = true, bool FOLD = false>
 __device__ __forceinline__ void decim_piece(const DecimArgs &a, int *lds, int stream, size_t seg_start, size_t seg_end, bool from_state,
                                             bool store_state, int meta_id, int meta_n)
 {
@@ -277,11 +291,12 @@
     const int32_t *stc = a.state_cur + (size_t)stream * DEC_STATE_WORDS;
     state_load<G>(lds, tid, stc, !from_state);
 
-    OutCtx oc;
+    OutCtxT<FOLD> oc;
     oc.norm = a.norm; oc.trunk = a.trunk;
     oc.frame_mode = a.frame_mode; oc.frame_blocks = a.frame_blocks; oc.frame_sample_base = a.frame_sample_base;
     oc.out = reinterpret_cast<unsigned *>(a.out) + (size_t)stream * a.out_stride;
     oc.out_pos = seg_start >> L;
+    oc.fold = FOLD && a.frame_fold ? a.frame_fold : ~0u;
 
     if (a.frame_mode) {
         unsigned base[6], rate;
@@ -289,14 +304,14 @@
         for (int fi = meta_id + tid * meta_n; fi < a.meta_count; fi += NT * meta_n) {
             unsigned w[6];
             frame_meta_words_thread(base, a.meta_idx0, rate, fi, w);
-            unsigned *fr = oc.out + (size_t)(a.meta_first + fi) * a.frame_blocks * 128u;
+            unsigned *fr = oc.out + frame_slot_dw(oc, (uint64_t)(a.meta_first + fi));
             fr[0] = (a.meta_frame_count0 + (unsigned)fi) & 0xffffu;
 #pragma unroll
             for (int k = 0; k < 6; ++k) fr[1 + k] = w[k];
         }
         if (tid < 128) {
             for (int fi = meta_id; fi < a.meta_count; fi += meta_n) {
-                unsigned *fr = oc.out + (size_t)(a.meta_first + fi) * a.frame_blocks * 128u;
+                unsigned *fr = oc.out + frame_slot_dw(oc, (uint64_t)(a.meta_first + fi));
                 const unsigned fidx = (a.meta_frame_count0 + (unsigned)fi) & 0xffffu;
                 if (tid >= 7) fr[tid] = 0u;
                 if (tid >= 1) fr[(size_t)tid * 128] = fidx | ((unsigned)tid << 16);
diff --git a/sdrdaemon_amd/csrc/decim_mfma.hip b/sdrdaemon_amd/csrc/decim_mfma.hip
--- a/sdrdaemon_amd/csrc/decim_mfma.hip
+++ b/sdrdaemon_amd/csrc/decim_mfma.hip
@@ -1,4 +1,5 @@
 #include "decim_body.h"
+#include "decim_mfma_cursor.h"
 
 #include <type_traits>
 #include <utility>
@@ -89,15 +90,16 @@
     unsigned selB;
 };
 
-template <bool FR> struct MfOut {
+template <bool FR, bool FOLD = false> struct MfOut {
+    static constexpr bool frames = FR, folds = FOLD;
     unsigned *p;
     unsigned *dump;
     int store;
     int norm, trunk;
     unsigned sel_pack;
     __amdgpu_buffer_rsrc_t rsrc;
-    unsigned off, c, b, t0, t1;
-    unsigned gap;
+    MfCursor cur;
+    MfFold fold;
 };
 
 typedef unsigned uint2_t __attribute__((ext_vector_type(2)));
@@ -176,23 +178,13 @@
         const int r1 = __builtin_amdgcn_update_dpp(0, g1, 0xB1, 0xf, 0xf, true);
         const unsigned pk0 = perm((unsigned)((int)((unsigned)r0 << oc.norm) >> oc.trunk), (unsigned)((int)((unsigned)m0 << oc.norm) >> oc.trunk), oc.sel_pack);
         const unsigned pk1 = perm((unsigned)((int)((unsigned)r1 << oc.norm) >> oc.trunk), (unsigned)((int)((unsigned)m1 << oc.norm) >> oc.trunk), oc.sel_pack);
-        if constexpr (std::is_same<OC, MfOut<true>>::value) {
-            const unsigned extra = oc.b == 126u ? oc.gap : 4u;
-            const unsigned bias = oc.store ? 0u : 0x80000000u;
-            const unsigned a0 = oc.off + (oc.c >= oc.t0 ? extra : 0u) + bias;
-            const unsigned hi = a0 ^ 0x40000000u;
-            const bool split = oc.c == oc.t1;
-            const unsigned a8 = split ? hi : a0, a4 = split ? a0 : hi;
-            __builtin_amdgcn_raw_buffer_store_b64((uint2_t){pk0, pk1}, oc.rsrc, a8, 0, 0);
-            __builtin_amdgcn_raw_buffer_store_b32(pk0, oc.rsrc, a4, 0, 0);
-            __builtin_amdgcn_raw_buffer_store_b32(pk1, oc.rsrc, a4 + extra, 4, 0);
-            const unsigned inc = oc.store ? 16u : 0u;
-            oc.c += inc;
-            const bool wrap = oc.c >= 127u;
-            oc.off += 4u * inc + (wrap ? extra : 0u);
-            oc.c -= wrap ? 127u : 0u;
-            oc.b += wrap ? 1u : 0u;
-            oc.b = oc.b >= 127u ? 0u : oc.b;
+        if constexpr (OC::frames) {
+            const unsigned extra = mf_cursor_extra<OC::folds>(oc.cur, oc.fold);
+            const MfStoreAddr sa = mf_cursor_addr(oc.cur, oc.store != 0, extra);
+            __builtin_amdgcn_raw_buffer_store_b64((uint2_t){pk0, pk1}, oc.rsrc, sa.a8, 0, 0);
+            __builtin_amdgcn_raw_buffer_store_b32(pk0, oc.rsrc, sa.a4, 0, 0);
+            __builtin_amdgcn_raw_buffer_store_b32(pk1, oc.rsrc, sa.a4x, 4, 0);
+            mf_cursor_advance(oc.cur, oc.store != 0, extra);
         } else {
             unsigned *dst = oc.store ? oc.p : oc.dump;
             *reinterpret_cast<uint2_t *>(dst) = (uint2_t){pk0, pk1};
@@ -349,7 +341,7 @@
     mf_wait_vm<0>();
 }
 
-template <int NS, int NG = 0, bool FR = false> __device__ __forceinline__ void mf_wave(const DecimArgs &a, int gw, unsigned lds_addr)
+template <int NS, int NG = 0, bool FR = false, bool FOLD = false> __device__ __forceinline__ void mf_wave(const DecimArgs &a, int gw, unsigned lds_addr)
 {
     if (a.mf_prio) __builtin_amdgcn_s_setprio(3);
     constexpr int L = NS;
@@ -390,7 +382,7 @@
     k.selA = q == 0 ? 0x03020104u : 0x03020100u;
     k.selB = q == 0 ? 0x03020106u : 0x03020100u;
 
-    MfOut<FR> oc;
+    MfOut<FR, FOLD> oc;
     oc.store = 0;
     oc.dump = a.mf_dump + 4 * lane;
     oc.norm = a.norm; oc.trunk = a.trunk;
@@ -398,20 +390,18 @@
     {
         const size_t first = ((wave_start + (size_t)p * S) >> L) + 4u * (unsigned)q;
         if constexpr (FR) {
-            unsigned *obase = reinterpret_cast<unsigned *>(a.out) + (size_t)stream * a.out_stride;
-            oc.rsrc = __builtin_amdgcn_make_buffer_rsrc(obase, 0, 0x3fffffff, 0x00020000);
+            unsigned *obase = reinterpret_cast<unsigned *>(a.out) + (size_t)stream * a.out_stride - (FOLD ? (size_t)a.frame_blocks * 128u : 0u);
+            oc.fold = mf_cursor_fold(FOLD ? a.frame_fold : 0u, (unsigned)a.frame_blocks);
+            oc.rsrc = __builtin_amdgcn_make_buffer_rsrc(obase, 0, FOLD ? (int)mf_cursor_records(a.frame_fold, (unsigned)a.frame_blocks) : 0x3fffffff, 0x00020000);
             const unsigned long long g = a.frame_sample_base + first;
             const unsigned long long f = g / 16129u;
-            const unsigned w = (unsigned)(g - f * 16129u);
-            oc.b = w / 127u; oc.c = w - oc.b * 127u;
-            oc.off = 4u * (unsigned)(((size_t)f * (size_t)a.frame_blocks + 1u + oc.b) * 128u + 1u + oc.c + 2u * (unsigned)comp);
-            oc.t0 = 127u - 2u * (unsigned)comp; oc.t1 = 126u - 2u * (unsigned)comp;
-            oc.gap = 4u * ((unsigned)a.frame_blocks * 128u - 16255u);
+            mf_cursor_init(oc.cur, FOLD ? (a.frame_fold && f == a.frame_fold ? 0u : f + 1u) : f, (unsigned)(g - f * 16129u), (unsigned)a.frame_blocks, (unsigned)comp);
             oc.p = nullptr;
         } else {
             unsigned *obase = reinterpret_cast<unsigned *>(a.out) + (size_t)stream * a.out_stride;
             oc.p = obase + first + 2 * comp;
-            oc.off = oc.c = oc.b = oc.t0 = oc.t1 = oc.gap = 0u;
+            oc.cur = MfCursor{0u, 0u, 0u, 0u, 0u};
+            oc.fold = MfFold{~0u};
         }
     }
 
@@ -469,12 +459,12 @@
             if (lx >= nitems || (j < a.mf_piece_early && lx >= nearly)) break;
             const int stream = lx / a.mf_npieces, piece = lx - stream * a.mf_npieces;
             if (piece == 0) {
-                decim_piece<L, 2, PACK16>(a, lds, stream, 0, a.mf_head, true, false, piece, a.mf_npieces);
+                decim_piece<L, 2, PACK16, true, FR>(a, lds, stream, 0, a.mf_head, true, false, piece, a.mf_npieces);
             } else {
                 const size_t s0 = a.mf_tail_start + (size_t)(piece - 1) * a.mf_tail_seg;
                 size_t s1 = s0 + a.mf_tail_seg;
                 if (s1 > a.n_used || piece == a.mf_npieces - 1) s1 = a.n_used;
-                decim_piece<L, 2, PACK16>(a, lds, stream, s0, s1, false, piece == a.mf_npieces - 1, piece, a.mf_npieces);
+                decim_piece<L, 2, PACK16, true, FR>(a, lds, stream, s0, s1, false, piece == a.mf_npieces - 1, piece, a.mf_npieces);
             }
             __syncthreads();
         }
@@ -483,7 +473,7 @@
     const int gw = __builtin_amdgcn_readfirstlane(bx * 4 + (int)(threadIdx.x >> 6));
     if (gw >= a.nstreams * a.mf_wps) return;
     MF_STAMP(gw, 0);
-    mf_wave<L, NG, FR>(a, gw, (unsigned)(size_t)(__attribute__((address_space(3))) char *)lds);
+    mf_wave<L, NG, FR, FR>(a, gw, (unsigned)(size_t)(__attribute__((address_space(3))) char *)lds);
     MF_STAMP(gw, 7);
 }
 __device__ __forceinline__ int mf_ragged_find(const RaggedRow *rows, int nstreams, int x, bool waves)
diff --git a/sdrdaemon_amd/csrc/decim_mfma_cursor.h b/sdrdaemon_amd/csrc/decim_mfma_cursor.h
--- /dev/null
+++ b/sdrdaemon_amd/csrc/decim_mfma_cursor.h
@@ -0,0 +1,76 @@
+#pragma once
+
+#ifndef MF_CURSOR_FN
+#if defined(__HIPCC__)
+#define MF_CURSOR_FN __host__ __device__ __forceinline__
+#else
+#define MF_CURSOR_FN inline
+#endif
+#endif
+
+namespace sdrhip {
+
+struct MfCursor {
+    unsigned off, c, b, tw;
+    unsigned gap;
+};
+
+struct MfStoreAddr {
+    unsigned a8;
+    unsigned a4;
+    unsigned a4x;
+};
+
+MF_CURSOR_FN unsigned mf_cursor_records(unsigned fold, unsigned frame_blocks)
+{
+    return 0x3fffffffu - (fold ? (fold + 1u) * frame_blocks * 512u : 0u);
+}
+
+struct MfFold {
+    unsigned thr;
+};
+MF_CURSOR_FN MfFold mf_cursor_fold(unsigned fold, unsigned frame_blocks)
+{
+    MfFold f;
+    f.thr = fold ? fold * frame_blocks * 512u + 512u : ~0u;
+    return f;
+}
+
+MF_CURSOR_FN void mf_cursor_init(MfCursor &k, unsigned long long slot, unsigned w, unsigned frame_blocks, unsigned comp)
+{
+    k.b = w / 127u; k.c = w - k.b * 127u + 2u * comp;
+    k.off = 4u * (unsigned)((slot * (unsigned long long)frame_blocks + 1u + k.b) * 128u + 1u + k.c);
+    k.tw = 127u + 2u * comp;
+    k.gap = 4u * (frame_blocks * 128u - 16255u);
+}
+
+template <bool FOLD> MF_CURSOR_FN unsigned mf_cursor_extra(const MfCursor &k, const MfFold &f)
+{
+    const unsigned gap = FOLD && k.off >= f.thr ? 0u - (f.thr + (4u * 16255u - 512u)) : k.gap;
+    return k.b == 126u ? gap : 4u;
+}
+
+MF_CURSOR_FN MfStoreAddr mf_cursor_addr(const MfCursor &k, bool store, unsigned extra)
+{
+    const unsigned bias = store ? 0u : 0x80000000u;
+    const unsigned a0 = k.off + (k.c >= 127u ? extra : 0u) + bias;
+    const unsigned hi = a0 ^ 0x40000000u;
+    const bool split = k.c == 126u;
+    MfStoreAddr a;
+    a.a8 = split ? hi : a0; a.a4 = split ? a0 : hi;
+    a.a4x = a.a4 + extra;
+    return a;
+}
+
+MF_CURSOR_FN void mf_cursor_advance(MfCursor &k, bool store, unsigned extra)
+{
+    const unsigned inc = store ? 16u : 0u;
+    k.c += inc;
+    const bool wrap = k.c >= k.tw;
+    k.off += 4u * inc + (wrap ? extra : 0u);
+    k.c -= wrap ? 127u : 0u;
+    k.b += wrap ? 1u : 0u;
+    k.b = k.b >= 127u ? 0u : k.b;
+}
+
+}
diff --git a/sdrdaemon_amd/csrc/rx_frame_area.h b/sdrdaemon_amd/csrc/rx_frame_area.h
--- a/sdrdaemon_amd/csrc/rx_frame_area.h
+++ b/sdrdaemon_amd/csrc/rx_frame_area.h
@@ -20,6 +20,7 @@
     size_t new_cap = 0;
     bool keep_old = false;
     std::vector<uint8_t> to_slot0;
+    size_t dst_slot = 0;
     bool moves() const
     {
         for (size_t s = 0; s < to_slot0.size(); ++s)
@@ -86,6 +87,26 @@
         }
         return p;
     }
+    RxAreaPlan plan_slide(const size_t *done, size_t window_multiple, size_t *landing) const
+    {
+        RxAreaPlan p;
+        const size_t S = base_.size();
+        size_t need_max = 0;
+        for (size_t s = 0; s < S; ++s) need_max = done[s] + 1 > need_max ? done[s] + 1 : need_max;
+        p.to_slot0.assign(S, 0);
+        p.dst_slot = need_max;
+        if (2 * need_max > cap_) {
+            p.new_cap = (window_multiple < 2 ? 2 : window_multiple) * need_max;
+            p.to_slot0.assign(S, 1);
+        } else
+            for (size_t s = 0; s < S; ++s)
+                if (base_[s] + done[s] + (base_[s] ? 0 : 1) > cap_) p.to_slot0[s] = 1;
+        for (size_t s = 0; s < S; ++s) {
+            const size_t q = p.to_slot0[s] ? p.dst_slot : base_[s];
+            landing[s] = !done[s] ? q : q ? q - 1 : done[s];
+        }
+        return p;
+    }
     RxAreaPlan replan() const
     {
         RxAreaPlan p;
@@ -97,12 +118,12 @@
     {
         if (p.new_cap) cap_ = p.new_cap;
         for (size_t s = 0; s < base_.size(); ++s)
-            if (p.to_slot0[s]) base_[s] = 0;
+            if (p.to_slot0[s]) base_[s] = p.dst_slot;
     }
-    void commit(const size_t *done, const uint64_t *rest)
+    void commit(const size_t *done, const uint64_t *rest, const size_t *landing = nullptr)
     {
         for (size_t s = 0; s < base_.size(); ++s) {
-            base_[s] += done[s];
+            base_[s] = landing ? landing[s] : base_[s] + done[s];
             pending_[s] = rest[s];
             open_[s] = rest[s] > 0 ? 1 : 0;
             count_[s] = (uint16_t)(count_[s] + done[s]);
diff --git a/sdrdaemon_amd/csrc/sdrhip.cpp b/sdrdaemon_amd/csrc/sdrhip.cpp
--- a/sdrdaemon_amd/csrc/sdrhip.cpp
+++ b/sdrdaemon_amd/csrc/sdrhip.cpp
@@ -69,7 +69,7 @@
         if (hipGetDeviceProperties(&prop, device) == hipSuccess && prop.multiProcessorCount > 0) c->n_cu = prop.multiProcessorCount;
         static const char *const keys[][2] = {{"SDRHIP_DECIM_PATH", "decim_path"}, {"SDRHIP_MFMA_SPAN", "mfma_span"}, {"SDRHIP_MFMA_MIN", "mfma_min"},
                                               {"SDRHIP_INTERP_PATH", "interp_path"}, {"SDRHIP_INTERP_SPAN", "interp_span"}, {"SDRHIP_RX_FUSED", "rx_fused"}, {"SDRHIP_RX_DIRECT", "rx_direct"},
-                                              {"SDRHIP_DEC_PATH", "dec_path"}, {"SDRHIP_ENC_PATH", "enc_path"}, {"SDRHIP_ENC_MIN_ROWS", "enc_min_rows"}, {"SDRHIP_MFMA_RING", "mfma_ring"}, {"SDRHIP_TX_OVERLAP", "tx_overlap"}, {"SDRHIP_RX_WINDOW", "rx_window"}, {"SDRHIP_FEC_STAGGER", "fec_stagger"}, {"SDRHIP_FEC_STAGGER_MOD", "fec_stagger_mod"}, {"SDRHIP_DEC_PLAN", "dec_plan"}, {"SDRHIP_TX_GATHER", "tx_gather"}, {"SDRHIP_ENC_UNITS", "enc_units"}, {"SDRHIP_ENC_FORM", "enc_form"}};
+                                              {"SDRHIP_DEC_PATH", "dec_path"}, {"SDRHIP_ENC_PATH", "enc_path"}, {"SDRHIP_ENC_MIN_ROWS", "enc_min_rows"}, {"SDRHIP_MFMA_RING", "mfma_ring"}, {"SDRHIP_TX_OVERLAP", "tx_overlap"}, {"SDRHIP_RX_WINDOW", "rx_window"}, {"SDRHIP_RX_SLIDE", "rx_slide"}, {"SDRHIP_FEC_STAGGER", "fec_stagger"}, {"SDRHIP_FEC_STAGGER_MOD", "fec_stagger_mod"}, {"SDRHIP_DEC_PLAN", "dec_plan"}, {"SDRHIP_TX_GATHER", "tx_gather"}, {"SDRHIP_ENC_UNITS", "enc_units"}, {"SDRHIP_ENC_FORM", "enc_form"}};
         for (size_t i = 0; i < sizeof(keys) / sizeof(keys[0]); ++i)
             if (const char *v = getenv(keys[i][0])) (void)sdrhip_ctx_set_option(c, keys[i][1], v);
     }
@@ -161,6 +161,7 @@
     else if (k == "rx_fused" && v == "overlap") c->opt.rx_fused = 3;
     else if (k == "rx_direct" && isnum && num <= 1) c->opt.rx_direct = (int)num;
     else if (k == "rx_window" && isnum && num <= 8) c->opt.rx_window = (int)num;
+    else if (k == "rx_slide" && isnum && num <= 1) c->opt.rx_slide = (int)num;
     else if (k == "mfma_ring" && isnum && num >= 2 && num <= 4) c->opt.mfma_ring = (int)num;
     else if (k == "tx_overlap" && isnum && num <= 1) c->opt.tx_overlap = (int)num;
     else if (k == "fec_stagger" && isnum && num <= 64) c->opt.fec_stagger = (int)num;
@@ -201,6 +202,7 @@
     sdrhip::CtxLock lock_(c);
     if (std::string(key) == "h2d_bytes") { *value = c->h2d_bytes; return SDRHIP_OK; }
     if (std::string(key) == "d2h_bytes") { *value = c->d2h_bytes; return SDRHIP_OK; }
+    if (std::string(key) == "rx_open_frame_moves") { *value = c->rx_open_frame_moves; return SDRHIP_OK; }
     const bool shadow = std::string(key) == "fecbuf_shadow_mismatch";
     const bool deferred = std::string(key) == "dec_deferred";
     if (std::string(key) != "dec_rows_exceeded" && !shadow && !deferred) return fail(SDRHIP_EINVAL, "ctx_get_counter: unknown key: %s", key);
diff --git a/sdrdaemon_amd/csrc/sdrhip_decim.cpp b/sdrdaemon_amd/csrc/sdrhip_decim.cpp
--- a/sdrdaemon_amd/csrc/sdrhip_decim.cpp
+++ b/sdrdaemon_amd/csrc/sdrhip_decim.cpp
@@ -155,7 +155,7 @@
 namespace sdrhip {
 int decimate_device(sdrhip_decimators *d, int log2decim, int fcpos, unsigned *sampleSize, const int16_t *in, size_t n_in,
                     size_t in_stride, int16_t *out, size_t out_stride, size_t *n_out, int frame_mode, int frame_blocks,
-                    uint64_t frame_sample_base, const RxMeta *meta, const Enc128Args *fuse, bool *fused, bool coresident)
+                    uint64_t frame_sample_base, const RxMeta *meta, const Enc128Args *fuse, bool *fused, bool coresident, unsigned frame_fold)
 {
     if (fused) *fused = false;
     sdrhip_ctx *c = d->ctx;
@@ -174,16 +174,18 @@
             a.n_used = n_used;
             a.norm = (int)sh.norm; a.trunk = (int)sh.trunk;
             a.frame_sample_base = frame_sample_base;
+            a.frame_fold = frame_fold;
             if (meta) set_meta_args(a, *meta);
             plan_decimate(log2decim, fcpos, n_used, S, &a.nsub_per_seg, &a.nseg);
             const CtxOptions &env = c->opt;
-            const bool mfma_frames = env.rx_direct && out_stride * 4 < 0x3fffffffu;
+            const bool mfma_frames = env.rx_direct && out_stride * 4 + (size_t)frame_blocks * SDRHIP_UDPSIZE < 0x3fffffffu;
             a.mf_ring = coresident ? 3 : env.mfma_ring;
             a.mf_prio = coresident ? 1 : 0;
             MfPlan p;
             *mfma = (!frame_mode || mfma_frames) && mfma_admitted(env.decim_path, env.mfma_min, log2decim, n_used * (size_t)S) &&
                     plan_decimate_mfma(log2decim, fcpos, n_used, S, env.mfma_span, c->n_cu, a.mf_ring, &p);
             if (*mfma) set_mf_args(a, p);
+            if (frame_fold && !*mfma) return fail(SDRHIP_EINVAL, "internal: only the matrix-core launch folds a frame in front of its window");
             return SDRHIP_OK;
         },
         [&](const DecimArgs &a, bool pack16, bool mfma) -> hipError_t {
diff --git a/sdrdaemon_amd/csrc/sdrhip_host.h b/sdrdaemon_amd/csrc/sdrhip_host.h
--- a/sdrdaemon_amd/csrc/sdrhip_host.h
+++ b/sdrdaemon_amd/csrc/sdrhip_host.h
@@ -41,7 +41,8 @@
 int decimate_device(sdrhip_decimators *d, int log2decim, int fcpos, unsigned *sampleSize, const int16_t *in, size_t n_in,
                     size_t in_stride, int16_t *out, size_t out_stride, size_t *n_out, int frame_mode, int frame_blocks,
                     uint64_t frame_sample_base, const RxMeta *meta = nullptr, const Enc128Args *fuse = nullptr, bool *fused = nullptr,
-                    bool coresident = false);
+                    bool coresident = false,
+                    unsigned frame_fold = 0);
 int ragged_prepare(sdrhip_decimators *d, int log2decim, int fcpos, const size_t *n_in, RaggedRow *rows, const RaggedRow **rows_dev,
                    RaggedPlan *plan, PinnedBuf *pin = nullptr);
 int ragged_reserve(sdrhip_decimators *d, PinnedBuf *pin);
@@ -172,6 +173,7 @@
     int mfma_ring = 4;
     int rx_fused = 1;
     int rx_direct = 1;
+    int rx_slide = 1;
     int rx_window = 0;
     int tx_overlap = 1;
     int enc_fft = 1;
@@ -222,6 +224,7 @@
     int ktime_stride_cls[SDRHIP_KCLASSES] = {0, 0, 0, 0, 0};
     unsigned ktime_seen[SDRHIP_KCLASSES] = {0, 0, 0, 0, 0};
     std::vector<std::pair<hipEvent_t, hipEvent_t>> kev[SDRHIP_KCLASSES];
+    uint64_t rx_open_frame_moves = 0;
     uint64_t h2d_bytes = 0, d2h_bytes = 0;
 };
 
diff --git a/sdrdaemon_amd/csrc/sdrhip_internal.h b/sdrdaemon_amd/csrc/sdrhip_internal.h
--- a/sdrdaemon_amd/csrc/sdrhip_internal.h
+++ b/sdrdaemon_amd/csrc/sdrhip_internal.h
@@ -56,6 +56,7 @@
     int mf_ring;
     int mf_prio;
     const unsigned *meta_tab;
+    unsigned frame_fold;
 };
 template <class Args, class Meta> inline void set_meta_args(Args &a, const Meta &m)
 {
diff --git a/sdrdaemon_amd/csrc/sdrhip_rx.cpp b/sdrdaemon_amd/csrc/sdrhip_rx.cpp
--- a/sdrdaemon_amd/csrc/sdrhip_rx.cpp
+++ b/sdrdaemon_amd/csrc/sdrhip_rx.cpp
@@ -102,16 +102,19 @@
     const RxFrameArea &A = rx->area;
     const size_t S = A.streams(), dcap = fresh ? p.new_cap : A.cap();
     const uint8_t *src = rx->work.as<uint8_t>();
-    uint8_t *dst = fresh ? fresh->as<uint8_t>() : rx->work.as<uint8_t>();
+    uint8_t *dst = (fresh ? fresh->as<uint8_t>() : rx->work.as<uint8_t>()) + p.dst_slot * dst_pitch;
     bool together = true;
     for (size_t s = 0; s < S; ++s) together = together && p.to_slot0[s] && A.open(s) && A.slot(s) == A.slot(0);
     hipError_t e = hipSuccess;
-    if (together)
+    if (together) {
         e = hipMemcpy2DAsync(dst, dcap * dst_pitch, src + A.slot(0) * src_pitch, A.cap() * src_pitch, bytes, S, hipMemcpyDeviceToDevice, c->stream);
-    else
+        ++c->rx_open_frame_moves;
+    } else
         for (size_t s = 0; s < S && e == hipSuccess; ++s)
-            if (p.to_slot0[s] && A.open(s))
+            if (p.to_slot0[s] && A.open(s)) {
                 e = hipMemcpyAsync(dst + s * dcap * dst_pitch, src + A.index(s) * src_pitch, bytes, hipMemcpyDeviceToDevice, c->stream);
+                ++c->rx_open_frame_moves;
+            }
     if (e == hipSuccess && fresh) e = hipStreamSynchronize(c->stream);
     if (e != hipSuccess) {
         if (fresh) { (void)hipStreamSynchronize(c->stream); fresh->release(); }
@@ -126,11 +129,12 @@
     return SDRHIP_OK;
 }
 
-static int rx_make_room(sdrhip_rx *rx, const size_t *done, bool pipelined, const char *who, bool grow_only = false)
+static int rx_make_room(sdrhip_rx *rx, const size_t *done, bool pipelined, const char *who, bool grow_only = false, size_t *landing = nullptr)
 {
     sdrhip_ctx *c = rx->ctx;
     const size_t wmul = c->opt.rx_window ? (size_t)c->opt.rx_window : pipelined ? 4 : 2;
-    const RxAreaPlan p = rx->area.plan(done, rx->late.have && !rx->late.in_old ? rx->late.first : RX_NO_LATE, wmul);
+    const RxAreaPlan p = landing ? rx->area.plan_slide(done, wmul, landing)
+                                 : rx->area.plan(done, rx->late.have && !rx->late.in_old ? rx->late.first : RX_NO_LATE, wmul);
     if (!p.new_cap && (grow_only || !p.moves())) return SDRHIP_OK;
     const size_t fb = rx_frame_bytes(rx);
     DevBuf fresh;
@@ -459,8 +463,18 @@
 
     const std::vector<size_t> dones((size_t)S, done);
     if ((rc = rx_release_old(rx))) return rc;
-    if ((rc = rx_make_room(rx, dones.data(), rx->pipelined != 0, "rx_process"))) return rc;
+    const bool filterless = L == 0 || (rx->cfg.fcpos != SDRHIP_FC_CEN && L <= 2);
+    bool slide = c->opt.rx_slide && c->opt.rx_direct && !rx->pipelined && !filterless && (c->opt.rx_window == 0 || c->opt.rx_window >= 2) &&
+                 2 * (done + 1) * frame_bytes < 0x3fffffffu && decimate_mfma_applies(rx->dec, L, rx->cfg.fcpos, n_in);
+    if (slide) {
+        const size_t wm = c->opt.rx_window ? (size_t)c->opt.rx_window : 2;
+        const size_t cap_then = 2 * (done + 1) > rx->area.cap() ? wm * (done + 1) : rx->area.cap();
+        slide = (cap_then + 1) * frame_bytes < 0x3fffffffu;
+    }
+    std::vector<size_t> landing((size_t)S, 0);
+    if ((rc = rx_make_room(rx, dones.data(), rx->pipelined != 0, "rx_process", false, slide ? landing.data() : nullptr))) return rc;
     const size_t cap = rx->area.cap(), slot0 = rx->area.slot(0);
+    const unsigned fold = slide && landing[0] < slot0 ? (unsigned)done : 0u;
     const size_t stream_bytes = cap * frame_bytes;
     uint8_t *work = rx->work.as<uint8_t>() + slot0 * frame_bytes;
 
@@ -482,7 +496,6 @@
     FrameArgs fa;
     memset(&fa, 0, sizeof(fa));
     const bool structured = R >= enc128_min_rows(c) && frame_bytes % 4 == 0;
-    const bool filterless = L == 0 || (rx->cfg.fcpos != SDRHIP_FC_CEN && L <= 2);
     const Enc128Args *fuse = rx->late.encode && (c->opt.rx_fused == 1 || c->opt.rx_fused == 2) ? &rx->late.k : nullptr;
     const bool coresident = rx->late.encode && c->opt.rx_fused == 3 && rx->ev_framed;
     bool fused = false;
@@ -520,7 +533,7 @@
         }
     } else {
         rc = decimate_device(rx->dec, L, rx->cfg.fcpos, &ss, din, n_in, dstride, reinterpret_cast<int16_t *>(work), stream_bytes / 4, &n_out, 1,
-                             FB, pending, &meta);
+                             FB, pending, &meta, nullptr, nullptr, false, fold);
         if (rc) return rc;
         rx->consumed = true;
     }
@@ -583,7 +596,7 @@
     } else {
         if ((rc = rx_deliver(rx, rx->work.as<uint8_t>(), slot0, stream_bytes, done, frame_bytes, frames_out, frame_stride_bytes, n_frames, mem))) return rc;
     }
-    rx->area.commit(dones.data(), std::vector<uint64_t>((size_t)S, adv.rest).data());
+    rx->area.commit(dones.data(), std::vector<uint64_t>((size_t)S, adv.rest).data(), slide ? landing.data() : nullptr);
     if (mem == SDRHIP_MEM_HOST) HIP_TRY(hipStreamSynchronize(c->stream));
     return SDRHIP_OK;
 }
```

Result: no change. 1.013 million (-0.2%).
